# klasmodin/quflow

Hardware: AMD Instinct MI355X
Metric: isospectral timesteps/sec at N=1024 (1 GPU) + ensemble steps/sec at 1/2/4/8 GPUs (higher is better)
Workload: dtype f64

## Files before the change

### include/quflow_hip.h

```cpp
#ifndef QUFLOW_HIP_H
#define QUFLOW_HIP_H

#ifdef __cplusplus
extern "C" {
#endif

#define QF_OK 0
#define QF_ERR_INVALID 1
#define QF_ERR_NO_DEVICE 2
#define QF_ERR_HIP 3
#define QF_ERR_STATE 4
#define QF_ERR_CALLBACK 5
#define QF_ERR_UNSUPPORTED 6
#define QF_ERR_NONFINITE 7
#define QF_ERR_NOCONVERGE 8

#define QF_VERSION 100

typedef struct qf_ctx qf_ctx;

int qf_version(void);
const char *qf_last_error(void);
int qf_device_count(void);

int qf_ctx_create(int N, int device, qf_ctx **out);
int qf_ctx_destroy(qf_ctx *ctx);
int qf_ctx_size(const qf_ctx *ctx);
int qf_sync(qf_ctx *ctx);

double qf_hbar(int N);


int qf_laplacian_table(qf_ctx *ctx, int bc, double *lap_host);

int qf_solve_poisson(qf_ctx *ctx, const void *W_host, void *P_host, int skewh);

int qf_laplace(qf_ctx *ctx, const void *P_host, void *W_host);

int qf_solve_tridiagonal(qf_ctx *ctx, const double *lap_host, unsigned long long table_key,
                         const void *W_host, void *P_host, int skewh);
int qf_factor_cache_stats(qf_ctx *ctx, int *entries, unsigned long long *device_bytes);

int qf_set_hamiltonian(qf_ctx *ctx, const double *table_host, unsigned long long table_key, const void *offset_host,
                       unsigned long long offset_key);
int qf_clear_hamiltonian(qf_ctx *ctx);
int qf_hamiltonian(qf_ctx *ctx, const void *W_host, void *P_host);
int qf_hamiltonian_energy(qf_ctx *ctx, double *H);

int qf_set_forcing(qf_ctx *ctx, const void *F0_host, unsigned long long F0_key, double a_W, double a_P, double a_lap);
int qf_clear_forcing(qf_ctx *ctx);
int qf_forcing(qf_ctx *ctx, const void *P_host, const void *W_host, void *F_host);

int qf_set_stochastic_forcing(qf_ctx *ctx, int l_min, int l_max, const double *sigma, unsigned long long seed,
                              unsigned long long step, double a_W, double a_P, double a_lap, long long band_bytes_max);
int qf_stochastic_tell(qf_ctx *ctx, unsigned long long *step);
int qf_stochastic_seek(qf_ctx *ctx, unsigned long long step);
int qf_stochastic_pattern(qf_ctx *ctx, unsigned long long step, double dt, double *omega_host, void *F0_host);

int qf_upload_W(qf_ctx *ctx, const void *W_host);
int qf_download_W(qf_ctx *ctx, void *W_host);

typedef struct qf_isomp_stats {
    long long total_iterations;
    long long number_of_maxit;
    double tol_used;
    double last_resnorm;
} qf_isomp_stats;

int qf_isomp(qf_ctx *ctx, double dt, int steps, double tol, int minit, int maxit,
             int compsum, int reinitialize, qf_isomp_stats *stats_out);
int qf_isomp_continue(qf_ctx *ctx, double dt, int steps, double tol, int minit, int maxit,
                      int compsum, int reinitialize, qf_isomp_stats *stats_out);

int qf_isomp_multi(qf_ctx **ctxs, int k, double dt, int steps, double tol, int minit, int maxit,
                   qf_isomp_stats *stats_out);
int qf_c64_isomp_multi(qf_ctx **ctxs, int k, double dt, int steps, double tol, int minit, int maxit, qf_isomp_stats *stats_out);

#define QF_ERK_EULER 0
#define QF_ERK_HEUN 1
#define QF_ERK_RK4 2
int qf_erk(qf_ctx *ctx, int method, double dt, int steps, int skewh);
int qf_erk_states(qf_ctx *ctx, void *states_host, int k, int method, double dt, int steps, int skewh);

int qf_isomp_simple(qf_ctx *ctx, double dt, int steps);
int qf_isomp_quasinewton(qf_ctx *ctx, double dt, int steps, double tol, int maxit, qf_isomp_stats *stats_out);
struct qf_isomp_hooks;
int qf_isomp_simple_hooked(qf_ctx *ctx, double dt, int steps, const struct qf_isomp_hooks *hooks);
int qf_isomp_quasinewton_hooked(qf_ctx *ctx, double dt, int steps, double tol, int maxit, qf_isomp_stats *stats_out,
                                const struct qf_isomp_hooks *hooks);

int qf_isomp_states(qf_ctx *ctx, void *states_host, int k, double dt, int steps, double tol, int minit, int maxit,
                    int reinitialize, int magnetic, qf_isomp_stats *stats_out);

int qf_states_upload(qf_ctx *ctx, const void *states_host, int k);
int qf_states_download(qf_ctx *ctx, void *states_host, int k);
int qf_states_advance(qf_ctx *ctx, double dt, int steps, double tol, int minit, int maxit, int reinitialize, int magnetic,
                      qf_isomp_stats *stats_out);
int qf_states_select(qf_ctx *ctx, int j);
int qf_states_store(qf_ctx *ctx, int j);
int qf_states_inner(qf_ctx *ctx, double *out);
int qf_mhd_diagnostics(qf_ctx *ctx, double out[5]);
int qf_states_advance_diag(qf_ctx *ctx, double dt, int steps, double tol, int minit, int maxit, int reinitialize, int magnetic,
                           qf_isomp_stats *stats_out, double *mhd_out);

typedef struct qf_isomp_hooks {
    void *user;
    int (*hamiltonian)(void *user, const void *Whalf, void *P, double time);
    int (*forcing)(void *user, const void *P, const void *Whalf, void *F, double time);
    int (*strang)(void *user, double h, void *W);
    int (*callback)(void *user, const void *W, const void *dW2);
    int hamiltonian_takes_time, forcing_takes_time;
    int has_time;
    double time;
    int skewh;
    int solve_skewh;
    const double *strang_table;
    unsigned long long strang_key;
    int magnetic;
    int states_p;
} qf_isomp_hooks;
int qf_isomp_hooked(qf_ctx *ctx, void *states_host, int k, double dt, int steps, double tol, int minit, int maxit,
                    int compsum, int reinitialize, const qf_isomp_hooks *hooks, qf_isomp_stats *stats_out);
int qf_isomp_forced(qf_ctx *ctx, double dt, int steps, double tol, int minit, int maxit, int reinitialize,
                    const double *strang_table, unsigned long long strang_key, qf_isomp_stats *stats_out);
int qf_erk_hooked(qf_ctx *ctx, void *W_host, int method, double dt, int steps, const qf_isomp_hooks *hooks);
int qf_erk_states_hooked(qf_ctx *ctx, void *states_host, int k, int method, double dt, int steps, const qf_isomp_hooks *hooks);

int qf_basis_upload(qf_ctx *ctx, const double *basis_host, long long count);
int qf_basis_compute(qf_ctx *ctx);
int qf_basis_download(qf_ctx *ctx, double *basis_host, long long count);
int qf_basis_stream(qf_ctx *ctx, long long slab_bytes);
int qf_basis_slab_plan(int N, int Nmax, long long slab_bytes, int *first_block, int capacity);
int qf_shr2mat(qf_ctx *ctx, const double *omega_host, long long n_omega, void *W_host);
int qf_mat2shr(qf_ctx *ctx, const void *W_host, double *omega_host, long long n_omega);
int qf_shc2mat(qf_ctx *ctx, const void *omega_host, void *W_host);
int qf_mat2shc(qf_ctx *ctx, const void *W_host, void *omega_host);
int qf_shr2fun(qf_ctx *ctx, const double *omega_host, long long n_omega, int L, int berezin, double *f_host);
int qf_shc2fun(qf_ctx *ctx, const void *omega_host, long long n_omega, int L, int berezin, int isreal, void *f_host);
int qf_fun2shc(qf_ctx *ctx, const void *f_host, int L, int isreal, void *omega_host);
int qf_fun2shr(qf_ctx *ctx, const void *f_host, int L, int isreal, double *omega_host);

int qf_diagnostics(qf_ctx *ctx, double *energy_euler, double *enstrophy);
int qf_isomp_diag(qf_ctx *ctx, double dt, int steps, double tol, int minit, int maxit, int compsum,
                  int reinitialize, qf_isomp_stats *stats, double *energy_euler, double *enstrophy);
int qf_norm_inf_W(qf_ctx *ctx, double *out);

typedef struct qf_eigh_stats {
    int sweeps;
    long long rotations;
    double off;
} qf_eigh_stats;
int qf_eigh(qf_ctx *ctx, const void *H_host, double *lambda_host, void *V_host, qf_eigh_stats *stats);
int qf_eigh_skew(qf_ctx *ctx, const void *W_host, double *lambda_host, void *V_host, qf_eigh_stats *stats);
int qf_eigh_state(qf_ctx *ctx, double *lambda_host, qf_eigh_stats *stats);
int qf_scale_decomposition(qf_ctx *ctx, const void *W_host, const void *P_host, void *Ws_host, void *Wr_host);

int qf_so3_exp_plan(int N, const double xi[3], int *squarings, int *degree);
int qf_so3_exp(qf_ctx *ctx, const double xi[3], void *R_host);
// ... 68 lines not shown
```

### quflow_amd/_lib.py

```python
import ctypes
import os

_HERE = os.path.dirname(os.path.abspath(__file__))
LIB_PATH = os.environ.get("QUFLOW_HIP_LIB") or os.path.join(_HERE, "libquflow_hip.so")

QF_OK = 0
QF_ERR_NONFINITE = 7
QF_ERR_NOCONVERGE = 8
ERR_NAMES = {1: "QF_ERR_INVALID", 2: "QF_ERR_NO_DEVICE", 3: "QF_ERR_HIP", 4: "QF_ERR_STATE", 5: "QF_ERR_CALLBACK",
             6: "QF_ERR_UNSUPPORTED", 7: "QF_ERR_NONFINITE", 8: "QF_ERR_NOCONVERGE"}

KERNEL_IDS = {"poisson": 0, "gemm1": 1, "gemm2": 2, "norm": 3, "update": 4, "slice": 5}
ERK_METHODS = {"euler": 0, "heun": 1, "rk4": 2}
BUFFER_IDS = {"W": 0, "dW": 1, "Whalf": 2, "Phalf": 3, "PW": 4}


class QuflowHipError(RuntimeError):
    pass


HAMILTONIAN_CB = ctypes.CFUNCTYPE(ctypes.c_int, ctypes.c_void_p, ctypes.c_void_p, ctypes.c_void_p, ctypes.c_double)
FORCING_CB = ctypes.CFUNCTYPE(ctypes.c_int, ctypes.c_void_p, ctypes.c_void_p, ctypes.c_void_p, ctypes.c_void_p, ctypes.c_double)
STRANG_CB = ctypes.CFUNCTYPE(ctypes.c_int, ctypes.c_void_p, ctypes.c_double, ctypes.c_void_p)
CALLBACK_CB = ctypes.CFUNCTYPE(ctypes.c_int, ctypes.c_void_p, ctypes.c_void_p, ctypes.c_void_p)


class IsompHooks(ctypes.Structure):
    _fields_ = [("user", ctypes.c_void_p),
                ("hamiltonian", HAMILTONIAN_CB),
                ("forcing", FORCING_CB),
                ("strang", STRANG_CB),
                ("callback", CALLBACK_CB),
                ("hamiltonian_takes_time", ctypes.c_int),
                ("forcing_takes_time", ctypes.c_int),
                ("has_time", ctypes.c_int),
                ("time", ctypes.c_double),
                ("skewh", ctypes.c_int),
                ("solve_skewh", ctypes.c_int),
                ("strang_table", ctypes.c_void_p),
                ("strang_key", ctypes.c_ulonglong),
                ("magnetic", ctypes.c_int),
                ("states_p", ctypes.c_int)]


class IsompStats(ctypes.Structure):
    _fields_ = [("total_iterations", ctypes.c_longlong),
                ("number_of_maxit", ctypes.c_longlong),
                ("tol_used", ctypes.c_double),
                ("last_resnorm", ctypes.c_double)]


class EighStats(ctypes.Structure):
    _fields_ = [("sweeps", ctypes.c_int),
                ("rotations", ctypes.c_longlong),
                ("off", ctypes.c_double)]


_vp = ctypes.c_void_p
_dp = ctypes.POINTER(ctypes.c_double)
SIGNATURES = {
    "qf_version": (ctypes.c_int, []),
    "qf_last_error": (ctypes.c_char_p, []),
    "qf_device_count": (ctypes.c_int, []),
    "qf_ctx_create": (ctypes.c_int, [ctypes.c_int, ctypes.c_int, ctypes.POINTER(_vp)]),
    "qf_ctx_destroy": (ctypes.c_int, [_vp]),
    "qf_ctx_size": (ctypes.c_int, [_vp]),
    "qf_sync": (ctypes.c_int, [_vp]),
    "qf_hbar": (ctypes.c_double, [ctypes.c_int]),
    "qf_laplacian_table": (ctypes.c_int, [_vp, ctypes.c_int, _vp]),
    "qf_solve_poisson": (ctypes.c_int, [_vp, _vp, _vp, ctypes.c_int]),
    "qf_laplace": (ctypes.c_int, [_vp, _vp, _vp]),
    "qf_solve_tridiagonal": (ctypes.c_int, [_vp, _vp, ctypes.c_ulonglong, _vp, _vp, ctypes.c_int]),
    "qf_set_hamiltonian": (ctypes.c_int, [_vp, _vp, ctypes.c_ulonglong, _vp, ctypes.c_ulonglong]),
    "qf_clear_hamiltonian": (ctypes.c_int, [_vp]),
    "qf_hamiltonian": (ctypes.c_int, [_vp, _vp, _vp]),
    "qf_hamiltonian_energy": (ctypes.c_int, [_vp, _dp]),
    "qf_set_forcing": (ctypes.c_int, [_vp, _vp, ctypes.c_ulonglong, ctypes.c_double, ctypes.c_double, ctypes.c_double]),
    "qf_clear_forcing": (ctypes.c_int, [_vp]),
    "qf_forcing": (ctypes.c_int, [_vp, _vp, _vp, _vp]),
    "qf_set_stochastic_forcing": (ctypes.c_int, [_vp, ctypes.c_int, ctypes.c_int, _vp, ctypes.c_ulonglong, ctypes.c_ulonglong,
                                                 ctypes.c_double, ctypes.c_double, ctypes.c_double, ctypes.c_longlong]),
    "qf_stochastic_tell": (ctypes.c_int, [_vp, ctypes.POINTER(ctypes.c_ulonglong)]),
    "qf_stochastic_seek": (ctypes.c_int, [_vp, ctypes.c_ulonglong]),
    "qf_stochastic_pattern": (ctypes.c_int, [_vp, ctypes.c_ulonglong, ctypes.c_double, _vp, _vp]),
    "qf_isomp_forced": (ctypes.c_int, [_vp, ctypes.c_double, ctypes.c_int, ctypes.c_double, ctypes.c_int, ctypes.c_int,
                                       ctypes.c_int, _vp, ctypes.c_ulonglong, ctypes.POINTER(IsompStats)]),
    "qf_factor_cache_stats": (ctypes.c_int, [_vp, ctypes.POINTER(ctypes.c_int), ctypes.POINTER(ctypes.c_ulonglong)]),
    "qf_comm_unique_id": (ctypes.c_int, [_vp]),
    "qf_comm_create": (ctypes.c_int, [ctypes.POINTER(_vp), ctypes.c_int, ctypes.c_int, ctypes.c_int, _vp]),
    "qf_comm_allgather_f64": (ctypes.c_int, [_vp, _vp, ctypes.c_int, _vp]),
    "qf_comm_barrier": (ctypes.c_int, [_vp]),
    "qf_comm_destroy": (ctypes.c_int, [_vp]),
    "qf_upload_W": (ctypes.c_int, [_vp, _vp]),
    "qf_download_W": (ctypes.c_int, [_vp, _vp]),
    "qf_isomp": (ctypes.c_int, [_vp, ctypes.c_double, ctypes.c_int, ctypes.c_double, ctypes.c_int,
                                ctypes.c_int, ctypes.c_int, ctypes.c_int, ctypes.POINTER(IsompStats)]),
    "qf_isomp_diag": (ctypes.c_int, [_vp, ctypes.c_double, ctypes.c_int, ctypes.c_double, ctypes.c_int,
                                     ctypes.c_int, ctypes.c_int, ctypes.c_int, ctypes.POINTER(IsompStats),
                                     ctypes.POINTER(ctypes.c_double), ctypes.POINTER(ctypes.c_double)]),
    "qf_isomp_continue": (ctypes.c_int, [_vp, ctypes.c_double, ctypes.c_int, ctypes.c_double, ctypes.c_int,
                                         ctypes.c_int, ctypes.c_int, ctypes.c_int, ctypes.POINTER(IsompStats)]),
    "qf_isomp_multi": (ctypes.c_int, [ctypes.POINTER(_vp), ctypes.c_int, ctypes.c_double, ctypes.c_int, ctypes.c_double,
                                      ctypes.c_int, ctypes.c_int, ctypes.POINTER(IsompStats)]),
    "qf_c64_isomp_multi": (ctypes.c_int, [ctypes.POINTER(_vp), ctypes.c_int, ctypes.c_double, ctypes.c_int, ctypes.c_double,
                                          ctypes.c_int, ctypes.c_int, ctypes.POINTER(IsompStats)]),
    "qf_erk": (ctypes.c_int, [_vp, ctypes.c_int, ctypes.c_double, ctypes.c_int, ctypes.c_int]),
    "qf_erk_states": (ctypes.c_int, [_vp, _vp, ctypes.c_int, ctypes.c_int, ctypes.c_double, ctypes.c_int, ctypes.c_int]),
    "qf_isomp_simple_hooked": (ctypes.c_int, [_vp, ctypes.c_double, ctypes.c_int, ctypes.POINTER(IsompHooks)]),
    "qf_isomp_quasinewton_hooked": (ctypes.c_int, [_vp, ctypes.c_double, ctypes.c_int, ctypes.c_double, ctypes.c_int,
                                                   ctypes.POINTER(IsompStats), ctypes.POINTER(IsompHooks)]),
    "qf_isomp_simple": (ctypes.c_int, [_vp, ctypes.c_double, ctypes.c_int]),
    "qf_isomp_quasinewton": (ctypes.c_int, [_vp, ctypes.c_double, ctypes.c_int, ctypes.c_double, ctypes.c_int,
                                            ctypes.POINTER(IsompStats)]),
    "qf_isomp_states": (ctypes.c_int, [_vp, _vp, ctypes.c_int, ctypes.c_double, ctypes.c_int, ctypes.c_double,
                                       ctypes.c_int, ctypes.c_int, ctypes.c_int, ctypes.c_int,
                                       ctypes.POINTER(IsompStats)]),
    "qf_states_upload": (ctypes.c_int, [_vp, _vp, ctypes.c_int]),
    "qf_states_download": (ctypes.c_int, [_vp, _vp, ctypes.c_int]),
    "qf_states_advance": (ctypes.c_int, [_vp, ctypes.c_double, ctypes.c_int, ctypes.c_double, ctypes.c_int, ctypes.c_int,
                                         ctypes.c_int, ctypes.c_int, ctypes.POINTER(IsompStats)]),
    "qf_states_advance_diag": (ctypes.c_int, [_vp, ctypes.c_double, ctypes.c_int, ctypes.c_double, ctypes.c_int, ctypes.c_int,
                                              ctypes.c_int, ctypes.c_int, ctypes.POINTER(IsompStats), _dp]),
    "qf_states_select": (ctypes.c_int, [_vp, ctypes.c_int]),
    "qf_states_store": (ctypes.c_int, [_vp, ctypes.c_int]),
    "qf_mhd_diagnostics": (ctypes.c_int, [_vp, _dp]),
    "qf_states_inner": (ctypes.c_int, [_vp, _dp]),
    "qf_isomp_hooked": (ctypes.c_int, [_vp, _vp, ctypes.c_int, ctypes.c_double, ctypes.c_int, ctypes.c_double, ctypes.c_int,
                                       ctypes.c_int, ctypes.c_int, ctypes.c_int, ctypes.POINTER(IsompHooks),
                                       ctypes.POINTER(IsompStats)]),
    "qf_erk_hooked": (ctypes.c_int, [_vp, _vp, ctypes.c_int, ctypes.c_double, ctypes.c_int, ctypes.POINTER(IsompHooks)]),
    "qf_erk_states_hooked": (ctypes.c_int, [_vp, _vp, ctypes.c_int, ctypes.c_int, ctypes.c_double, ctypes.c_int,
                                            ctypes.POINTER(IsompHooks)]),
    "qf_basis_upload": (ctypes.c_int, [_vp, _vp, ctypes.c_longlong]),
    "qf_basis_compute": (ctypes.c_int, [_vp]),
    "qf_basis_download": (ctypes.c_int, [_vp, _vp, ctypes.c_longlong]),
    "qf_basis_stream": (ctypes.c_int, [_vp, ctypes.c_longlong]),
    "qf_basis_slab_plan": (ctypes.c_int, [ctypes.c_int, ctypes.c_int, ctypes.c_longlong, ctypes.POINTER(ctypes.c_int),
                                          ctypes.c_int]),
    "qf_shr2mat": (ctypes.c_int, [_vp, _vp, ctypes.c_longlong, _vp]),
    "qf_mat2shr": (ctypes.c_int, [_vp, _vp, _vp, ctypes.c_longlong]),
    "qf_shc2mat": (ctypes.c_int, [_vp, _vp, _vp]),
    "qf_mat2shc": (ctypes.c_int, [_vp, _vp, _vp]),
    "qf_shr2fun": (ctypes.c_int, [_vp, _vp, ctypes.c_longlong, ctypes.c_int, ctypes.c_int, _vp]),
    "qf_shc2fun": (ctypes.c_int, [_vp, _vp, ctypes.c_longlong, ctypes.c_int, ctypes.c_int, ctypes.c_int, _vp]),
    "qf_fun2shc": (ctypes.c_int, [_vp, _vp, ctypes.c_int, ctypes.c_int, _vp]),
    "qf_fun2shr": (ctypes.c_int, [_vp, _vp, ctypes.c_int, ctypes.c_int, _vp]),
    "qf_diagnostics": (ctypes.c_int, [_vp, _dp, _dp]),
    "qf_norm_inf_W": (ctypes.c_int, [_vp, _dp]),
    "qf_eigh": (ctypes.c_int, [_vp, _vp, _vp, _vp, ctypes.POINTER(EighStats)]),
    "qf_eigh_skew": (ctypes.c_int, [_vp, _vp, _vp, _vp, ctypes.POINTER(EighStats)]),
    "qf_eigh_state": (ctypes.c_int, [_vp, _vp, ctypes.POINTER(EighStats)]),
    "qf_scale_decomposition": (ctypes.c_int, [_vp, _vp, _vp, _vp, _vp]),
    "qf_so3_exp_plan": (ctypes.c_int, [ctypes.c_int, _dp, ctypes.POINTER(ctypes.c_int), ctypes.POINTER(ctypes.c_int)]),
    "qf_so3_exp": (ctypes.c_int, [_vp, _dp, _vp]),
    "qf_so3_exp_times": (ctypes.c_int, [_vp, _dp, _dp]),
    "qf_rotate": (ctypes.c_int, [_vp, _dp, _vp, _vp]),
    "qf_grad": (ctypes.c_int, [_vp, _vp, _vp]),
    "qf_profile_enable": (ctypes.c_int, [_vp, ctypes.c_int]),
    "qf_profile_reset": (ctypes.c_int, [_vp]),
    "qf_profile_read": (ctypes.c_int, [_vp, ctypes.c_int, ctypes.POINTER(ctypes.c_longlong), _dp]),
    "qf_plan_describe": (ctypes.c_int, [_vp, ctypes.c_char_p, ctypes.c_int]),
    "qf_device_info": (ctypes.c_int, [ctypes.c_int, ctypes.c_char_p, ctypes.c_int]),
    "qf_debug_modulus": (ctypes.c_int, [_vp, ctypes.c_int, _dp, _dp, _dp, _dp]),
    "qf_profile_stride": (ctypes.c_int, [_vp, ctypes.c_int]),
    "qf_profile_seen": (ctypes.c_int, [_vp, ctypes.c_int, ctypes.POINTER(ctypes.c_longlong)]),
    "qf_timer_start": (ctypes.c_int, [_vp]),
    "qf_timer_stop": (ctypes.c_int, [_vp, _dp]),
    "qf_download_buffer": (ctypes.c_int, [_vp, ctypes.c_int, _vp]),
    "qf_debug_guard_check": (ctypes.c_int, [ctypes.POINTER(ctypes.c_longlong), ctypes.POINTER(ctypes.c_longlong), ctypes.c_char_p, ctypes.c_int]),
    "qf_zgemm": (ctypes.c_int, [_vp, _vp, _vp, _vp]),
    "qf_commutator": (ctypes.c_int, [_vp, _vp, _vp, _vp, ctypes.c_int]),
    "qf_zgemm_i8": (ctypes.c_int, [_vp, _vp, _vp, _vp]),
    "qf_fixedpoint_products": (ctypes.c_int, [_vp, _vp, _vp, _vp, _vp, ctypes.c_int, _vp, _vp, _vp]),
    "qf_c64_laplacian_table": (ctypes.c_int, [_vp, ctypes.c_int, _vp]),
    "qf_c64_solve_poisson": (ctypes.c_int, [_vp, _vp, _vp, ctypes.c_int]),
    "qf_c64_laplace": (ctypes.c_int, [_vp, _vp, _vp]),
    "qf_c64_solve_tridiagonal": (ctypes.c_int, [_vp, _vp, _vp, _vp, ctypes.c_int]),
    "qf_c64_upload_W": (ctypes.c_int, [_vp, _vp]),
    "qf_c64_download_W": (ctypes.c_int, [_vp, _vp]),
    "qf_c64_isomp": (ctypes.c_int, [_vp, ctypes.c_double, ctypes.c_int, ctypes.c_double, ctypes.c_int,
                                    ctypes.c_int, ctypes.c_int, ctypes.c_int, ctypes.POINTER(IsompStats)]),
    "qf_c64_isomp_continue": (ctypes.c_int, [_vp, ctypes.c_double, ctypes.c_int, ctypes.c_double, ctypes.c_int,
                                             ctypes.c_int, ctypes.c_int, ctypes.c_int, ctypes.POINTER(IsompStats)]),
    "qf_c64_diagnostics": (ctypes.c_int, [_vp, _dp, _dp]),
    "qf_cgemm": (ctypes.c_int, [_vp, _vp, _vp, _vp]),
    "qf_c64_fixedpoint_products": (ctypes.c_int, [_vp, _vp, _vp, _vp, _vp, _vp, _vp, _vp]),
    "qf_c64_fixedpoint_products_tri": (ctypes.c_int, [_vp, _vp, _vp, _vp, _vp, _vp, _vp, _vp]),
}
# ... 50 lines not shown
```

### quflow_amd/csrc/api_context.hip

```cpp
#include <cmath>
#include <cstdarg>
#include <cstdio>
#include <cstdlib>
#include <cstring>
#include <limits>
#include <chrono>

#include "qf_api.h"

static thread_local char g_err[512] = "";

void qf_set_error(const char *fmt, ...)
{
    va_list ap;
    va_start(ap, fmt);
    vsnprintf(g_err, sizeof(g_err), fmt, ap);
    va_end(ap);
}

extern "C" {

int qf_version(void) { return QF_VERSION; }

int qf_device_info(int device, char *buf, int n)
// ... 35 lines not shown
        return -QF_ERR_INVALID;
    }
    static const char *const role[QF_KERNEL_COUNT] = {"laplacian_inverse", "first_product", "second_product", "residual_norm",
                                                      "step_update", "slicing"};
    std::string out = "{\"N\": " + std::to_string(ctx->N);
    for (int r = 0; r < QF_KERNEL_COUNT; ++r) {
        out += ", \"";
        out += role[r];
        out += "\": ";
        out += ctx->plan[r].text[0] ? ctx->plan[r].text : "null";
    }
    if (ctx->ham_table || ctx->ham_offset_on) {
        char h[160];
        if (ctx->ham_table) snprintf(h, sizeof(h), ", \"hamiltonian\": {\"table_key\": %llu, \"offset\": %s}", ctx->ham_key, ctx->ham_offset_on ? "true" : "false");
        else snprintf(h, sizeof(h), ", \"hamiltonian\": {\"table_key\": null, \"offset\": true}");
        out += h;
    } else {
        out += ", \"hamiltonian\": \"poisson\"";
    }
    out += "}";
    if (n > 0) {
        const size_t m = out.size() < (size_t)(n - 1) ? out.size() : (size_t)(n - 1);
        memcpy(buf, out.data(), m);
        buf[m] = 0;
    }
    return (int)out.size();
}

const char *qf_last_error(void) { return g_err; }

int qf_device_count(void)
{
    int n = 0;
    if (hipGetDeviceCount(&n) != hipSuccess) return 0;
    return n;
}

double qf_hbar(int N) { return 2.0 / std::sqrt((double)N * (double)N - 1.0); }

int qf_ctx_create(int N, int device, qf_ctx **out)
{
    if (!out) {
        qf_set_error("qf_ctx_create: out is null");
        return QF_ERR_INVALID;
    }
    *out = nullptr;
    if (N < 2 || N > 8192) {
        qf_set_error("qf_ctx_create: N=%d out of range [2, 8192]", N);
        return QF_ERR_INVALID;
    }
    int ndev = qf_device_count();
    if (ndev <= 0) {
        qf_set_error("qf_ctx_create: no HIP device visible (this library has no CPU fallback)");
        return QF_ERR_NO_DEVICE;
    }
    if (device < 0 || device >= ndev) {
        qf_set_error("qf_ctx_create: device %d out of range (0..%d)", device, ndev - 1);
        return QF_ERR_NO_DEVICE;
    }
    QF_HIP(hipSetDevice(device));
    qf_ctx *ctx = new qf_ctx();
    ctx->N = N;
    ctx->device = device;
    if (const char *g = getenv("QUFLOW_HIP_GEMM")) {
        ctx->gemm_i8_allowed = (g[0] == 'i');
        if (g[0] == 'i' && strstr(g, "x6")) ctx->oz_digits = 6;
        if (g[0] == 'i' && strstr(g, "x65")) ctx->oz_digits2 = 5;
        if (g[0] == 'i' && strchr(g, 'h')) ctx->gemm_i8_hybrid = true;
        if (g[0] == 'i' && strchr(g, 'f') && !ctx->gemm_i8_hybrid) ctx->gemm_i8_first = true;
        if (g[0] == 'a') {
            ctx->gemm_i8_allowed = true;
            ctx->oz_digits = 6;
            ctx->oz_digits2 = 5;
            ctx->gemm_i8_min_n = 1024;
        }
    }
    if (const char *g = getenv("QUFLOW_HIP_GEMM2")) ctx->gemm_tri_allowed = !(g[0] == 'f');
    if (const char *g = getenv("QUFLOW_HIP_FUSED")) ctx->fused_allowed = !(g[0] == '0');
    if (const char *g = getenv("QUFLOW_HIP_I8_MIN_N")) ctx->gemm_i8_min_n = atoi(g);
    if (const char *g = getenv("QUFLOW_HIP_TRI_MIN_N")) ctx->gemm_tri_min_n = atoi(g);
    if (const char *g = getenv("QUFLOW_HIP_DEFER")) ctx->defer_allowed = !(g[0] == '0');
    if (getenv("QUFLOW_HIP_DEBUG"))
        if (const char *g = getenv("QUFLOW_HIP_DEBUG_DROP_FLAG")) ctx->debug_drop = atoi(g);
    if (const char *g = getenv("QUFLOW_HIP_FACTOR_CACHE_MB")) ctx->factor_budget_bytes = (size_t)(atoi(g) > 0 ? atoi(g) : 1) << 20;
    const size_t NN = (size_t)N * N;
    const size_t mbytes = NN * sizeof(cplx);
    int rc = QF_OK;
    auto fail = [&](int code) {
        qf_ctx_destroy(ctx);
        return code;
    };
#define QF_CREATE_HIP(call)                                                                   \
    do {                                                                                      \
        hipError_t _e = (call);                                                               \
        if (_e != hipSuccess) {                                                               \
            qf_set_error("%s failed: %s", #call, hipGetErrorString(_e));                     \
            return fail(QF_ERR_HIP);                                                          \
        }                                                                                     \
    } while (0)
    QF_CREATE_HIP(hipStreamCreateWithFlags(&ctx->stream, hipStreamNonBlocking));
    cplx **mats[] = {&ctx->W, &ctx->dW[0], &ctx->dW[1], &ctx->Whalf, &ctx->Phalf, &ctx->PW, &ctx->stage};
    for (cplx **m : mats) {
        QF_CREATE_HIP(hipMalloc((void **)m, mbytes));
        QF_CREATE_HIP(hipMemsetAsync(*m, 0, mbytes, ctx->stream));
    }
    QF_CREATE_HIP(hipMalloc((void **)&ctx->lap, 2 * NN * sizeof(double)));
    ctx->rowpart_tiles = qf_gemm_tiles_n(N);
    {
        const int slots32 = (N + 31) / 32;
        QF_CREATE_HIP(hipMalloc((void **)&ctx->rowpart, (size_t)(ctx->rowpart_tiles > slots32 ? ctx->rowpart_tiles : slots32) * N * sizeof(double)));
    }
    QF_CREATE_HIP(hipMalloc((void **)&ctx->rowsum, (size_t)N * sizeof(double)));
    QF_CREATE_HIP(hipMalloc((void **)&ctx->scalars, 4096 * sizeof(double)));
    QF_CREATE_HIP(hipHostMalloc((void **)&ctx->host_scalars, 64 * sizeof(double), hipHostMallocDefault));
    QF_CREATE_HIP(hipMalloc((void **)&ctx->state, sizeof(qf_dev_state)));
    QF_CREATE_HIP(hipMemsetAsync(ctx->state, 0, sizeof(qf_dev_state), ctx->stream));
    QF_CREATE_HIP(hipMalloc((void **)&ctx->ticket, 704 * sizeof(unsigned)));
    QF_CREATE_HIP(hipMemsetAsync(ctx->ticket, 0, 704 * sizeof(unsigned), ctx->stream));
    QF_CREATE_HIP(hipHostMalloc((void **)&ctx->host_rec, sizeof(qf_host_record), hipHostMallocCoherent));
    memset(ctx->host_rec, 0, sizeof(qf_host_record));
    {
        hipDeviceProp_t prop;
        QF_CREATE_HIP(hipGetDeviceProperties(&prop, device));
        ctx->num_cus = prop.multiProcessorCount;
        if (N % 64 == 0 && ctx->num_cus > 0) {
            ctx->sk_slots = ctx->num_cus;
            QF_CREATE_HIP(hipMalloc((void **)&ctx->sk_partial, (size_t)ctx->sk_slots * 64 * 64 * sizeof(cplx)));
            QF_CREATE_HIP(hipMalloc((void **)&ctx->sk_flags, (size_t)(ctx->sk_slots + 16) * sizeof(unsigned)));
            QF_CREATE_HIP(hipMemsetAsync(ctx->sk_flags, 0, (size_t)(ctx->sk_slots + 16) * sizeof(unsigned), ctx->stream));
        }
    }
    QF_CREATE_HIP(hipEventCreate(&ctx->timer_start));
    QF_CREATE_HIP(hipEventCreate(&ctx->timer_stop));
#undef QF_CREATE_HIP
    if ((rc = alloc_factors(ctx, &ctx->poisson)) != QF_OK) return fail(rc);
    if ((rc = qf_launch_lap_table(ctx, 1, ctx->lap)) != QF_OK) return fail(rc);
    if ((rc = qf_launch_build_factors(ctx, ctx->lap, ctx->poisson)) != QF_OK) return fail(rc);
    if (hipStreamSynchronize(ctx->stream) != hipSuccess) {
        qf_set_error("qf_ctx_create: table construction failed");
        return fail(QF_ERR_HIP);
    }
    *out = ctx;
    return QF_OK;
}

int qf_ctx_destroy(qf_ctx *ctx)
{
    if (!ctx) return QF_OK;
    (void)hipSetDevice(ctx->device);
    if (ctx->stream) (void)hipStreamSynchronize(ctx->stream);
    void *ptrs[] = {ctx->W, ctx->dW[0], ctx->dW[1], ctx->Whalf, ctx->Phalf, ctx->PW, ctx->kahan_c, ctx->stage,
                    ctx->lap, ctx->lap_user, ctx->poisson.tab, ctx->ham.tab, ctx->ham_offset, ctx->forcing_f0, ctx->stoch.basis, ctx->stoch.omega,
                    ctx->stoch.stage, ctx->stoch.sigma, ctx->rowpart, ctx->rowsum,
                    ctx->t32_partial, ctx->t32_arrive, ctx->W2, ctx->Whalf2, ctx->ns_inv, ctx->ns_tmp, ctx->multi_rowpart, ctx->scalars, ctx->sk_partial, ctx->sk_flags, ctx->basis, ctx->sh_stage, ctx->sh_omega, ctx->slab};
    for (void *p : ptrs)
        if (p) (void)hipFree(p);
    void *sht[] = {ctx->sht.omega, ctx->sht.tab, ctx->sht.col, ctx->sht.At, ctx->sht.tw, ctx->sht.f, ctx->sht.H, ctx->sht.Q};
    for (void *p : sht)
        if (p) (void)hipFree(p);
    void *eigh[] = {ctx->eigh.H, ctx->eigh.G, ctx->eigh.V, ctx->eigh.ray, ctx->eigh.sig, ctx->eigh.perm, ctx->eigh.word};
    for (void *p : eigh)
        if (p) (void)hipFree(p);
    void *geom[] = {ctx->geom.R[0], ctx->geom.R[1], ctx->geom.grad};
    for (void *p : geom)
        if (p) (void)hipFree(p);
    for (hipEvent_t e : ctx->geom.ev)
        if (e) (void)hipEventDestroy(e);
    for (cplx *p : ctx->multi)
        if (p) (void)hipFree(p);
    for (cplx *p : ctx->stack)
        if (p) (void)hipFree(p);
    if (ctx->mhd_part) (void)hipFree(ctx->mhd_part);
    for (int q = 0; q < 4; ++q) {
        if (ctx->oz_planes[q]) (void)hipFree(ctx->oz_planes[q]);
        if (ctx->oz_scale[q]) (void)hipFree(ctx->oz_scale[q]);
        if (q == 0 && ctx->oz_tbuf) (void)hipFree(ctx->oz_tbuf);
        if (q == 0 && ctx->oz_tflags) (void)hipFree(ctx->oz_tflags);
        if (q == 0 && ctx->oz_diag) (void)hipFree(ctx->oz_diag);
    }
    for (auto &kv : ctx->user_factors) {
        if (kv.second.f.tab) (void)hipFree(kv.second.f.tab);
    }
    for (int q = 0; q < 3; ++q)
        if (ctx->hook_host[q]) (void)hipHostFree(ctx->hook_host[q]);
    qf_c64_free(ctx->c64);
    ctx->c64 = nullptr;
    if (ctx->host_scalars) (void)hipHostFree(ctx->host_scalars);
    if (ctx->host_rec) (void)hipHostFree(ctx->host_rec);
    if (ctx->state) (void)hipFree(ctx->state);
    if (ctx->ticket) (void)hipFree(ctx->ticket);
    for (auto &ev : ctx->events_busy) {
        (void)hipEventDestroy(ev.start);
        (void)hipEventDestroy(ev.stop);
    }
    for (auto &ev : ctx->events_free) {
        (void)hipEventDestroy(ev.start);
        (void)hipEventDestroy(ev.stop);
    }
    if (ctx->timer_start) (void)hipEventDestroy(ctx->timer_start);
    if (ctx->timer_stop) (void)hipEventDestroy(ctx->timer_stop);
    if (ctx->stream) (void)hipStreamDestroy(ctx->stream);
    delete ctx;
    return QF_OK;
}

int qf_ctx_size(const qf_ctx *ctx) { return ctx ? ctx->N : -1; }

int qf_sync(qf_ctx *ctx)
{
    QF_TRY(check_ctx(ctx));
    QF_HIP(hipStreamSynchronize(ctx->stream));
    return QF_OK;
}


int qf_upload_W(qf_ctx *ctx, const void *W_host)
{
    QF_TRY(check_ctx(ctx));
    if (!W_host) {
        qf_set_error("qf_upload_W: null buffer");
        return QF_ERR_INVALID;
    }
    QF_HIP(hipMemcpyAsync(ctx->W, W_host, (size_t)ctx->N * ctx->N * sizeof(cplx), hipMemcpyHostToDevice, ctx->stream));
    QF_HIP(hipStreamSynchronize(ctx->stream));
    ctx->w_skew_known = false;
    return QF_OK;
}

int qf_download_W(qf_ctx *ctx, void *W_host)
{
    QF_TRY(check_ctx(ctx));
    if (!W_host) {
        qf_set_error("qf_download_W: null buffer");
        return QF_ERR_INVALID;
    }
    QF_HIP(hipMemcpyAsync(W_host, ctx->W, (size_t)ctx->N * ctx->N * sizeof(cplx), hipMemcpyDeviceToHost, ctx->stream));
    QF_HIP(hipStreamSynchronize(ctx->stream));
    return QF_OK;
}

int qf_norm_inf_W(qf_ctx *ctx, double *out)
{
    QF_TRY(check_ctx(ctx));
    QF_TRY(qf_launch_norm_inf(ctx, ctx->W, ctx->scalars));
    return read_scalar(ctx, ctx->scalars, out);
}


int qf_c64_upload_W(qf_ctx *ctx, const void *W_host)
{
    QF_TRY(qf_need_c64(ctx));
    if (!W_host) {
        qf_set_error("qf_c64_upload_W: null buffer");
        return QF_ERR_INVALID;
    }
    QF_HIP(hipMemcpyAsync(ctx->c64->W, W_host, (size_t)ctx->N * ctx->N * sizeof(float2), hipMemcpyHostToDevice, ctx->stream));
    QF_HIP(hipStreamSynchronize(ctx->stream));
    ctx->c64->increment_valid = false;
    ctx->c64->w_skew_known = false;
    return QF_OK;
}

int qf_c64_download_W(qf_ctx *ctx, void *W_host)
{
    QF_TRY(qf_need_c64(ctx));
    if (!W_host) {
        qf_set_error("qf_c64_download_W: null buffer");
        return QF_ERR_INVALID;
    }
    QF_HIP(hipMemcpyAsync(W_host, ctx->c64->W, (size_t)ctx->N * ctx->N * sizeof(float2), hipMemcpyDeviceToHost, ctx->stream));
    QF_HIP(hipStreamSynchronize(ctx->stream));
    return QF_OK;
}


int qf_profile_enable(qf_ctx *ctx, int mask)
{
    QF_TRY(check_ctx(ctx));
    if (!mask) QF_TRY(drain_events(ctx));
    ctx->profile_mask = mask;
    return QF_OK;
}

// ... 109 lines not shown
```

### quflow_amd/csrc/api_isomp.hip

```cpp
#include <cmath>
#include <cstdarg>
#include <cstdio>
#include <cstdlib>
#include <cstring>
#include <limits>
#include <chrono>
#include <type_traits>
#include <utility>

#include "qf_api.h"

namespace {

#ifndef QF_RUN_AHEAD
#define QF_RUN_AHEAD 3
#endif

template <class S> constexpr bool is_c64 = std::is_same<S, qf_c64>::value;

template <class S> S *ws(qf_ctx *ctx)
{
    if constexpr (is_c64<S>) return ctx->c64;
    else return ctx;
}

template <class S> double mach_eps(bool root)
{
    using R = std::conditional_t<is_c64<S>, float, double>;
    const R e = std::numeric_limits<R>::epsilon();
    return root ? std::sqrt(e) : e;
}

int launch_solve(qf_ctx *ctx, const cplx *W, cplx *P, double vareps, qf_guard g, const qf_decide *dec = nullptr)
{
    return qf_launch_hamiltonian(ctx, W, P, vareps, g, dec);
}
int launch_solve(qf_ctx *ctx, const float2 *W, float2 *P, double vareps, qf_guard g)
{
    return qf_launch_solve(ctx, ctx->c64->tab, W, P, (float)vareps, 1, g);
}
int launch_gemm(qf_ctx *ctx, const cplx *A, const cplx *B, cplx *C, const qf_epilogue *ep, qf_guard g)
{
    return qf_launch_zgemm(ctx, A, B, C, ep, g);
}
int launch_gemm(qf_ctx *ctx, const float2 *A, const float2 *B, float2 *C, const qf_epilogue_f *ep, qf_guard g)
{
    return qf_launch_cgemm(ctx, A, B, C, ep, g);
}

template <class S> auto epilogue_of(S *w, bool fused)
{
    std::conditional_t<is_c64<S>, qf_epilogue_f, qf_epilogue> ep;
    ep.PW = w->PW;
    ep.W = w->W;
    ep.dW[0] = w->dW[0];
    ep.dW[1] = w->dW[1];
    ep.Whalf = w->Whalf;
    ep.rowpart = w->rowpart;
    if (fused) {
        ep.fused = 1;
        ep.Wpair[0] = w->W;
        ep.Wpair[1] = w->W2;
        ep.Whalf_step = w->Whalf2;
    }
    return ep;
}

template <class S> int check_skew(qf_ctx *ctx, S *w)
{
    if (w->w_skew_known) return QF_OK;
    double defect = 0.0;
    QF_TRY(qf_launch_skew_defect(ctx, w->W, ctx->scalars + 4));
    QF_TRY(read_scalar(ctx, ctx->scalars + 4, &defect));
    w->w_skew_known = (defect == 0.0);
    return QF_OK;
}

int tri32_alloc(qf_ctx *ctx)
{
    const int nt = (ctx->N + 31) / 32;
    const int n_tiles = nt * (nt + 1) / 2;
    if (!ctx->t32_partial) {
        QF_HIP(hipMalloc((void **)&ctx->t32_partial, (size_t)n_tiles * 4 * 32 * 32 * sizeof(cplx)));
        QF_HIP(hipMalloc((void **)&ctx->t32_arrive, (size_t)n_tiles * sizeof(unsigned)));
        QF_HIP(hipMemsetAsync(ctx->t32_arrive, 0, (size_t)n_tiles * sizeof(unsigned), ctx->stream));
        int so = 2, sd = 1;
        {
            const int cus = ctx->num_cus > 0 ? ctx->num_cus : 256;
            if (nt * (nt - 1) + 2 * nt <= cus) sd = 2;
            else if (nt * (nt - 1) + nt > cus) so = 1;
        }
        ctx->tri32_split = so;
        ctx->tri32_split_diag = sd;
    }
    return QF_OK;
}

int select_second_product(qf_ctx *ctx)
{
// ... 6 lines not shown
    const bool want_tri32 = ctx->gemm_tri_allowed && !want_tri && ctx->N >= 64 && tri32_fits;
    const bool want_i8 = ctx->gemm_i8_allowed && ctx->N % 64 == 0 && ctx->N >= ctx->gemm_i8_min_n && ctx->N <= 4096;
    if (!want_tri && !want_i8 && !want_tri32) return QF_OK;
    QF_TRY(check_skew(ctx, ctx));
    const bool skew = ctx->w_skew_known;
    ctx->gemm_tri = want_tri && skew;
    ctx->gemm_i8 = want_i8 && skew;
    ctx->gemm_tri32 = want_tri32 && skew && (!ctx->gemm_i8 || ctx->gemm_i8_first);
    if (ctx->gemm_tri32) QF_TRY(tri32_alloc(ctx));
    return QF_OK;
}

int select_second_product_c64(qf_ctx *ctx)
{
    qf_c64 *f = ctx->c64;
    f->tri = false;
    if (f->tri_allowed && ctx->gemm_tri_allowed && (qf_c64_tile(ctx) == 32 || ctx->N % 64 == 0) && ctx->N >= 64) {
        QF_TRY(check_skew(ctx, f));
        if (f->w_skew_known) {
            QF_TRY(qf_c64_tri_alloc(ctx));
            f->tri = true;
        }
    }
    return QF_OK;
}

bool triangle_product(const qf_ctx *ctx) { return (ctx->gemm_tri || ctx->gemm_tri32) && (!ctx->gemm_i8 || ctx->gemm_i8_first); }
bool triangle_product(const qf_c64 *f) { return f->tri; }

template <class S> int begin_increment(qf_ctx *ctx, S *w, bool carry)
{
    const size_t mbytes = (size_t)ctx->N * ctx->N * sizeof(*w->W);
    if (carry) {
        if (w->dw_cur != 0)
            QF_HIP(hipMemcpyAsync(w->dW[0], w->dW[w->dw_cur], mbytes, hipMemcpyDeviceToDevice, ctx->stream));
        QF_TRY(qf_launch_lincomb(ctx, 1, w->W, 1, w->dW[0], 0, w->Whalf));
    } else {
        QF_HIP(hipMemsetAsync(w->dW[0], 0, mbytes, ctx->stream));
        QF_HIP(hipMemcpyAsync(w->Whalf, w->W, mbytes, hipMemcpyDeviceToDevice, ctx->stream));
    }
    return QF_OK;
}

template <class S> int enqueue_iterations(qf_ctx *ctx, int step, int first, int count, double vareps)
{
    S *w = ws<S>(ctx);
    for (int i = first; i < first + count; ++i) {
        qf_guard g;
        g.state = ctx->state;
        g.step = step;
        g.iter = i;
        {
            prof_scope p(ctx, QF_KERNEL_POISSON);
            QF_TRY(launch_solve(ctx, w->Whalf, w->Phalf, vareps, g));
        }
        {
            prof_scope p(ctx, QF_KERNEL_GEMM1);
            QF_TRY(launch_gemm(ctx, w->Phalf, w->Whalf, w->PW, nullptr, g));
        }
        {
            prof_scope p(ctx, QF_KERNEL_GEMM2);
            const auto ep = epilogue_of(w, false);
            QF_TRY(launch_gemm(ctx, w->PW, w->Phalf, nullptr, &ep, g));
        }
        {
            prof_scope p(ctx, QF_KERNEL_NORM);
            QF_TRY(qf_launch_norm_decide(ctx, w->rowpart, is_c64<S> ? w->rowpart_tiles : qf_rowpart_slots(ctx), g));
        }
    }
    return QF_OK;
}

qf_decide deferred_decision(qf_ctx *ctx)
{
    qf_decide d;
    d.rowpart = ctx->rowpart;
    d.slots = ctx->gemm_tri32 ? (ctx->N + 31) / 32 : ctx->N / 64;
    d.state_rw = ctx->state;
    d.rec = ctx->host_rec;
    d.ticket = ctx->ticket + 402;
    return d;
}

template <class S> int enqueue_iterations_fused(qf_ctx *ctx, int step, int first, int count, double vareps, bool last_step)
{
    S *w = ws<S>(ctx);
    const bool defer = !is_c64<S> && ctx->defer;
    const qf_decide dec = defer ? deferred_decision(ctx) : qf_decide();
    for (int i = first; i < first + count; ++i) {
        qf_guard g;
        g.state = ctx->state;
        g.step = step;
        g.iter = i;
        g.alt = w->Whalf2;
        {
            prof_scope p(ctx, QF_KERNEL_POISSON);
            if constexpr (is_c64<S>) QF_TRY(launch_solve(ctx, w->Whalf, w->Phalf, vareps, g));
            else QF_TRY(launch_solve(ctx, w->Whalf, w->Phalf, vareps, g, defer ? &dec : nullptr));
        }
        {
            prof_scope p(ctx, QF_KERNEL_GEMM1);
            QF_TRY(launch_gemm(ctx, w->Phalf, w->Whalf, w->PW, nullptr, g));
        }
        {
            prof_scope p(ctx, QF_KERNEL_GEMM2);
            const auto ep = epilogue_of(w, true);
            g.alt = nullptr;
            if constexpr (is_c64<S>) {
                if (w->tri) QF_TRY(qf_launch_cgemm_tri(ctx, w->PW, w->Phalf, &ep, g));
                else QF_TRY(qf_launch_cgemm(ctx, w->PW, w->Phalf, nullptr, &ep, g));
            } else {
                QF_TRY(qf_launch_zgemm(ctx, w->PW, w->Phalf, nullptr, &ep, g));
            }
        }
    }
    if (defer && last_step && count > 0) QF_TRY(qf_launch_decide(ctx, dec));
    return QF_OK;
}

int enqueue_iterations_fused_i8(qf_ctx *ctx, int step, int first, int count, double vareps)
{
    for (int i = first; i < first + count; ++i) {
        qf_guard g;
        g.state = ctx->state;
        g.step = step;
        g.iter = i;
        g.alt = ctx->Whalf2;
        {
            prof_scope p(ctx, QF_KERNEL_POISSON);
            QF_TRY(qf_launch_hamiltonian(ctx, ctx->Whalf, ctx->Phalf, vareps, g));
        }
        if (ctx->gemm_i8_hybrid) {
            {
                prof_scope p(ctx, QF_KERNEL_GEMM1);
                QF_TRY(qf_launch_zgemm(ctx, ctx->Phalf, ctx->Whalf, ctx->PW, nullptr, g));
            }
            g.alt = nullptr;
            {
                prof_scope p(ctx, QF_KERNEL_SLICE);
                qf_oz_jobs jobs;
                jobs.n = 2;
                jobs.j[0].X = ctx->PW;
                jobs.j[0].planes = ctx->oz_planes[3];
                jobs.j[0].scale = ctx->oz_scale[3];
                jobs.j[1].X = ctx->Phalf;
                jobs.j[1].planes = ctx->oz_planes[0];
                jobs.j[1].scale = ctx->oz_scale[0];
                QF_TRY(qf_launch_oz_slice(ctx, jobs, g));
            }
            {
                prof_scope p(ctx, QF_KERNEL_GEMM2);
                const qf_epilogue ep = epilogue_of(ctx, true);
                QF_TRY(qf_launch_oz_gemm(ctx, ctx->oz_planes[3], ctx->oz_scale[3], ctx->oz_planes[0], ctx->oz_scale[0], nullptr,
                                         &ep, g));
            }
            continue;
        }
        g.alt = nullptr;
        {
            prof_scope p(ctx, QF_KERNEL_SLICE);
            qf_oz_jobs jobs;
            jobs.n = 2;
            jobs.j[0].X = ctx->Phalf;
            jobs.j[0].planes = ctx->oz_planes[0];
            jobs.j[0].scale = ctx->oz_scale[0];
            jobs.j[1].X = ctx->Whalf;
            jobs.j[1].X_alt = ctx->Whalf2;
            jobs.j[1].planes = ctx->oz_planes[2];
            jobs.j[1].scale = ctx->oz_scale[2];
            jobs.diag = ctx->oz_diag;
            QF_TRY(qf_launch_oz_slice(ctx, jobs, g));
        }
        {
            prof_scope p(ctx, QF_KERNEL_GEMM1);
            QF_TRY(qf_launch_oz_gemm(ctx, ctx->oz_planes[0], ctx->oz_scale[0], ctx->oz_planes[2], ctx->oz_scale[2],
                                     ctx->PW, nullptr, g, 0, 0, ctx->oz_diag));
        }
        if (ctx->gemm_i8_first) {
            prof_scope p(ctx, QF_KERNEL_GEMM2);
            const qf_epilogue ep = epilogue_of(ctx, true);
            QF_TRY(qf_launch_zgemm(ctx, ctx->PW, ctx->Phalf, nullptr, &ep, g));
            continue;
        }
        {
            prof_scope p(ctx, QF_KERNEL_SLICE);
            qf_oz_jobs jobs;
            jobs.n = 1;
            jobs.j[0].X = ctx->PW;
            jobs.j[0].planes = ctx->oz_planes[3];
            jobs.j[0].scale = ctx->oz_scale[3];
            QF_TRY(qf_launch_oz_slice(ctx, jobs, g, ctx->oz_digits2));
        }
        {
            prof_scope p(ctx, QF_KERNEL_GEMM2);
            const qf_epilogue ep = epilogue_of(ctx, true);
            QF_TRY(qf_launch_oz_gemm(ctx, ctx->oz_planes[3], ctx->oz_scale[3], ctx->oz_planes[0], ctx->oz_scale[0], nullptr,
                                     &ep, g, ctx->oz_digits2, ctx->oz_digits2 ? ctx->oz_digits : 0));
        }
    }
    return QF_OK;
}

template <class S> struct fused_run {
    qf_ctx *ctx = nullptr;
    int steps = 0, minit = 1, maxit = 1;
    double vareps = 0.0;
    int pred = 1, pred0 = 1;
    std::vector<int> enq_iters;
    int known = 0, enq = 0;
    bool first_seen = false;
    bool aborted = false;
    unsigned long long idle_polls = 0;

    int enqueue(int step, int first, int count)
    {
        if constexpr (!is_c64<S>)
            if (ctx->gemm_i8) return enqueue_iterations_fused_i8(ctx, step, first, count, vareps);
        return enqueue_iterations_fused<S>(ctx, step, first, count, vareps, step == steps - 1);
    }
    bool cold_start = true;
    void begin(qf_ctx *c, int steps_, int minit_, int maxit_, double vareps_)
    {
        ctx = c;
        cold_start = ws<S>(c)->increment_is_zero;
        steps = steps_;
        minit = minit_;
        maxit = maxit_;
        vareps = vareps_;
        pred = ctx->pred_iters;
        if (pred < minit) pred = minit;
        if (pred > maxit) pred = maxit;
        pred0 = ctx->pred_first_iters > 0 ? ctx->pred_first_iters : pred + 1;
        if (pred0 < pred) pred0 = pred;
        if (pred0 > maxit) pred0 = maxit;
        enq_iters.assign((size_t)steps + 1, 0);
        known = enq = 0;
        first_seen = false;
        aborted = false;
        idle_polls = 0;
    }
    bool done() const { return known >= steps; }
    int pump()
    {
        if (done()) return QF_OK;
        while (enq < steps && enq - known < QF_RUN_AHEAD) {
            const int n = (enq == 0 && cold_start) ? pred0 : pred;
            QF_TRY(enqueue(enq, 0, n));
            enq_iters[enq] = n;
            ++enq;
        }
        volatile qf_host_record *rec = ctx->host_rec;
        unsigned long long p = __atomic_load_n(&rec->progress, __ATOMIC_ACQUIRE);
        int ps = (int)(p >> 32), pi = (int)(p & 0xffffffffull);
        if (ps >= QF_STEP_ABORTED) {
            aborted = true;
            known = steps;
            return QF_OK;
        }
        if (!(ps > known || (ps == known && pi >= enq_iters[known]))) {
            if (++idle_polls > (1ull << 22)) {
                QF_HIP(hipStreamSynchronize(ctx->stream));
                p = __atomic_load_n(&rec->progress, __ATOMIC_ACQUIRE);
                ps = (int)(p >> 32);
                pi = (int)(p & 0xffffffffull);
                if (ps >= QF_STEP_ABORTED) {
                    aborted = true;
                    known = steps;
                    return QF_OK;
                }
                if (!(ps > known || (ps == known && pi >= enq_iters[known]))) {
                    qf_set_error("qf_isomp: device progress stuck at step %d iteration %d (waiting for step %d)", ps, pi, known);
                    return QF_ERR_STATE;
                }
            } else {
                return QF_OK;
            }
        }
        idle_polls = 0;
        if (ps > known) {
            const int it = rec->last_step_iters;
            if (known == 0 && ps == 1 && !first_seen && cold_start) {
                first_seen = true;
                if (it >= minit && it <= maxit) ctx->pred_first_iters = it;
            } else if (it >= minit && it <= maxit) {
                pred = it;
            }
            known = ps < enq ? ps : enq;
            if (done()) ctx->pred_iters = pred;
            return QF_OK;
        }
        const int have = enq_iters[known];
        if (have >= maxit) {
            qf_set_error("qf_isomp: step %d did not close after maxit=%d iterations (internal error)", known, maxit);
            return QF_ERR_STATE;
        }
        QF_TRY(enqueue(known, have, maxit - have));
        enq_iters[known] = maxit;
        enq = known + 1;
        if (pred < maxit) pred += 1;
        return QF_OK;
    }
};

bool poll_yields()
{
    static const int mode = [] {
        const char *e = getenv("QUFLOW_HIP_POLL");
        return (e && strcmp(e, "yield") == 0) ? 1 : 0;
    }();
    return mode == 1;
}

inline void poll_relax()
{
    if (poll_yields()) {
        sched_yield();
        return;
    }
#if defined(__x86_64__)
    __builtin_ia32_pause();
#endif
}

template <class S> int run_fused(qf_ctx *ctx, int steps, int minit, int maxit, double vareps)
{
    fused_run<S> run;
    run.begin(ctx, steps, minit, maxit, vareps);
    while (!run.done()) {
        QF_TRY(run.pump());
        poll_relax();
    }
    ctx->pred_iters = run.pred;
    return QF_OK;
}

template <class S> int enqueue_step_end(qf_ctx *ctx, int step, int compsum, int reinitialize)
{
    S *w = ws<S>(ctx);
    qf_guard g;
    g.state = ctx->state;
    g.step = step;
    prof_scope p(ctx, QF_KERNEL_UPDATE);
    return qf_launch_update(ctx, w->PW, w->W, w->dW[0], w->dW[1], w->Whalf, compsum ? w->kahan_c : nullptr, reinitialize, g);
}

int wait_for_advance(qf_ctx *ctx, unsigned long long seq)
{
    volatile qf_host_record *rec = ctx->host_rec;
    unsigned long long spins = 0;
    while (__atomic_load_n(&rec->seq, __ATOMIC_ACQUIRE) < seq) {
        if (++spins > (1ull << 22)) {
            const unsigned long long before = __atomic_load_n(&rec->seq, __ATOMIC_ACQUIRE);
            const hipError_t q = hipStreamQuery(ctx->stream);
            QF_HIP(hipStreamSynchronize(ctx->stream));
            if (getenv("QUFLOW_HIP_DEBUG"))
                fprintf(stderr, "[quflow_hip] wait_for_advance: spin limit; want seq %llu, saw %llu before sync (stream %s), %llu after; step_index %d incomplete %d\n",
                        seq, before, q == hipSuccess ? "idle" : "busy", (unsigned long long)rec->seq, rec->step_index, rec->incomplete);
            if (__atomic_load_n(&rec->seq, __ATOMIC_ACQUIRE) < seq) {
                qf_set_error("qf_isomp: device progress record stuck at %llu (< %llu)",
                             (unsigned long long)rec->seq, seq);
                return QF_ERR_STATE;
            }
            break;
        }
#if defined(__x86_64__)
        __builtin_ia32_pause();
#endif
    }
    return QF_OK;
}

int reset_after_abort(qf_ctx *ctx)
{
    if (!ctx->needs_reset) return QF_OK;
    QF_HIP(hipMemsetAsync(ctx->ticket, 0, 704 * sizeof(unsigned), ctx->stream));
    if (ctx->sk_flags) QF_HIP(hipMemsetAsync(ctx->sk_flags + (ctx->sk_slots > 0 ? ctx->sk_slots : ctx->num_cus), 0, 16 * sizeof(unsigned), ctx->stream));
    if (ctx->t32_arrive) {
        const size_t nt = (size_t)(ctx->N + 31) / 32;
        QF_HIP(hipMemsetAsync(ctx->t32_arrive, 0, nt * (nt + 1) / 2 * sizeof(unsigned), ctx->stream));
    }
    if (ctx->c64 && ctx->c64->tri_arrive)
        QF_HIP(hipMemsetAsync(ctx->c64->tri_arrive, 0, ctx->c64->tri_arrive_count * sizeof(unsigned), ctx->stream));
    ctx->needs_reset = false;
    return QF_OK;
}

template <class S> int fused_enter(qf_ctx *ctx, double dt, double tol, int minit, int maxit, bool carry)
{
    S *w = ws<S>(ctx);
    const size_t mbytes = (size_t)ctx->N * ctx->N * sizeof(*w->W);
    const bool tol_on_device = tol < 0;
    const double tol_factor = tol_on_device ? mach_eps<S>(true) * dt / qf_hbar(ctx->N) : 0.0;
    QF_TRY(reset_after_abort(ctx));
    if constexpr (is_c64<S>) {
        QF_TRY(select_second_product_c64(ctx));
    } else {
        QF_TRY(select_second_product(ctx));
        ctx->defer = ctx->defer_allowed && !ctx->gemm_i8 && ctx->gemm_tri32 && ctx->N <= 512;
    }
    w->increment_is_zero = !carry;
    w->increment_valid = true;
    volatile qf_host_record *rec = ctx->host_rec;
    rec->progress = 0ull;
    rec->step_index = 0;
    rec->fault = 0;
    rec->nonfinite = 0;
    __atomic_thread_fence(__ATOMIC_SEQ_CST);
    if (is_c64<S> || carry) {
        if (tol_on_device) QF_TRY(qf_launch_norm_inf(ctx, w->W, ctx->scalars));
        QF_TRY(begin_increment(ctx, w, carry));
        QF_TRY(qf_launch_state_init(ctx, tol, minit, maxit, tol_on_device ? ctx->scalars : nullptr, tol_factor));
    } else {
        QF_TRY(qf_launch_call_begin(ctx, tol, minit, maxit, tol_on_device ? 1 : 0, tol_factor));
    }
    if (!w->W2) QF_HIP(hipMalloc((void **)&w->W2, mbytes));
    if (!w->Whalf2) QF_HIP(hipMalloc((void **)&w->Whalf2, mbytes));
    if constexpr (!is_c64<S>)
        if (ctx->gemm_i8) QF_TRY(qf_oz_alloc(ctx));
    return QF_OK;
}

template <class S> int fused_leave(qf_ctx *ctx, int steps, qf_isomp_stats *stats_out)
{
    S *w = ws<S>(ctx);
    volatile qf_host_record *rec = ctx->host_rec;
    const int w_parity = steps > 0 ? rec->w_parity : 0, wh_sel = steps > 0 ? rec->wh_sel : 0;
    w->dw_cur = steps > 0 ? rec->dw_parity : 0;
    if (w_parity) std::swap(w->W, w->W2);
    if (wh_sel) std::swap(w->Whalf, w->Whalf2);
    if (triangle_product(w) && steps > 0) {
        QF_TRY(qf_launch_mirror_lower(ctx, w->W));
        QF_TRY(qf_launch_mirror_lower(ctx, w->dW[w->dw_cur]));
    }
    if constexpr (!is_c64<S>)
        if (ctx->diag_at_exit) {
            QF_TRY(qf_enqueue_diagnostics(ctx));
            ctx->diag_valid = true;
        }
    QF_HIP(hipStreamSynchronize(ctx->stream));
    if (rec->nonfinite) {
        qf_set_error("array must not contain infs or NaNs");
        ctx->needs_reset = true;
        w->increment_valid = false;
        ctx->diag_valid = false;
        rec->nonfinite = 0;
        return QF_ERR_NONFINITE;
    }
    if (steps > 0 && rec->step_index != steps) {
        qf_set_error("qf_isomp: device completed %d of %d steps (internal error)", rec->step_index, steps);
        return QF_ERR_STATE;
    }
    if (rec->fault) {
        qf_set_error("qf_isomp: a device-side wait of the second product ran out (a parked partial tile or a mirrored result tile was never published)");
        return QF_ERR_STATE;
    }
    if (stats_out) {
        stats_out->total_iterations = steps > 0 ? rec->total_iterations : 0;
        stats_out->number_of_maxit = steps > 0 ? rec->number_of_maxit : 0;
        stats_out->tol_used = rec->tol;
        stats_out->last_resnorm = rec->resnorm;
    }
    return QF_OK;
}

void fused_abort(qf_ctx *ctx)
{
    (void)hipStreamSynchronize(ctx->stream);
// ... 142 lines not shown
                steps, t_tol, t_sel, t_init, t_loop, t_sync, ms_since(t_entry), t_waitmax, waitstep, t_waitat, t_enqmax, enqstep, t_enqat);
    if (st.fault == QF_FAULT_NONFINITE || rec->nonfinite) {
        qf_set_error("array must not contain infs or NaNs");
        ctx->needs_reset = true;
        w->increment_valid = false;
        rec->nonfinite = 0;
        return QF_ERR_NONFINITE;
    }
    if (st.step_index != steps) {
        qf_set_error("qf_isomp: device completed %d of %d steps (internal error)", st.step_index, steps);
        return QF_ERR_STATE;
    }
    w->dw_cur = st.dw_parity;
    if (rec->fault) {
        qf_set_error("qf_isomp: a device-side wait of the second product ran out (a parked partial tile or a mirrored result tile was never published)");
        return QF_ERR_STATE;
    }
    if (stats_out) {
        stats_out->total_iterations = st.total_iterations;
        stats_out->number_of_maxit = st.number_of_maxit;
        stats_out->tol_used = tol;
        stats_out->last_resnorm = rec->resnorm;
    }
    return QF_OK;
}

template <class S>
int isomp_multi(qf_ctx **ctxs, int k, double dt, int steps, double tol, int minit, int maxit, qf_isomp_stats *stats_out)
{
    const char *name = is_c64<S> ? "qf_c64_isomp_multi" : "qf_isomp_multi";
    if (!ctxs || k < 1) {
        qf_set_error("%s: bad arguments (k=%d)", name, k);
        return QF_ERR_INVALID;
    }
    if (minit < 1) {
        qf_set_error("minit must be at least 1.");
        return QF_ERR_INVALID;
    }
    if (maxit < minit) {
        qf_set_error("maxit must be at minit.");
        return QF_ERR_INVALID;
    }
    if (steps < 0) {
        qf_set_error("%s: steps must be >= 0", name);
        return QF_ERR_INVALID;
    }
    bool together = true;
    for (int r = 0; r < k; ++r) {
        QF_TRY(check_ctx(ctxs[r]));
        QF_TRY(qf_refuse_forcing(ctxs[r], name));
        if (is_c64<S> && !ctxs[r]->c64) {
            qf_set_error("%s: context %d holds no complex64 state (qf_c64_upload_W)", name, r);
            return QF_ERR_STATE;
        }
        for (int q = 0; q < r; ++q)
            if (ctxs[q] == ctxs[r]) {
                qf_set_error("%s: context %d is listed twice", name, r);
                return QF_ERR_INVALID;
            }
        if (ctxs[r]->device != ctxs[0]->device) {
            qf_set_error("%s: the contexts live on different devices", name);
            return QF_ERR_INVALID;
        }
        together = together && ctxs[r]->fused_allowed;
    }
    auto mark_failed = [&](int r) {
        if (!stats_out) return;
        stats_out[r].total_iterations = -1;
        stats_out[r].number_of_maxit = -1;
        stats_out[r].last_resnorm = std::numeric_limits<double>::quiet_NaN();
    };
    if (!together) {
        int first_rc = QF_OK;
        for (int q = 0; q < k; ++q) {
            const int rc = isomp_impl<S>(ctxs[q], dt, steps, tol, minit, maxit, 0, 0, stats_out ? stats_out + q : nullptr, false);
            if (rc != QF_OK) {
                mark_failed(q);
                if (first_rc == QF_OK) first_rc = rc;
            }
        }
        return first_rc;
    }
    auto abort_all = [&](int rc) {
        for (int q = 0; q < k; ++q) fused_abort(ctxs[q]);
        return rc;
    };
    std::vector<fused_run<S>> runs((size_t)k);
    for (int r = 0; r < k; ++r) {
        const int rc = fused_enter<S>(ctxs[r], dt, tol, minit, maxit, false);
        if (rc != QF_OK) return abort_all(rc);
        runs[r].begin(ctxs[r], steps, minit, maxit, dt / (2 * qf_hbar(ctxs[r]->N)));
    }
    for (;;) {
        bool all = true;
        for (int r = 0; r < k; ++r) {
            if (runs[r].done()) continue;
            const int rc = runs[r].pump();
            if (rc != QF_OK) return abort_all(rc);
            all = all && runs[r].done();
        }
        if (all) break;
        poll_relax();
    }
    int first_rc = QF_OK;
    for (int r = 0; r < k; ++r) {
        ctxs[r]->pred_iters = runs[r].pred;
        const int rc = fused_leave<S>(ctxs[r], steps, stats_out ? stats_out + r : nullptr);
        if (rc != QF_OK) {
            mark_failed(r);
            if (first_rc == QF_OK) first_rc = rc;
        }
    }
    return first_rc == QF_OK ? QF_OK : abort_all(first_rc);
}

int c64_fixedpoint_products(const char *name, bool tri, qf_ctx *ctx, const void *Phalf_host, const void *Whalf_host,
                            const void *W_host, const void *dW_old_host, void *dW_new_host, void *Whalf_new_host,
                            double *rowsum_host)
{
    QF_TRY(qf_need_c64(ctx));
    if (!Phalf_host || !Whalf_host || !W_host || !dW_old_host || !dW_new_host || !Whalf_new_host || !rowsum_host) {
        qf_set_error("%s: null buffer", name);
        return QF_ERR_INVALID;
    }
    if (tri) QF_TRY(qf_c64_tri_alloc(ctx));
    qf_c64 *f = ctx->c64;
    const int N = ctx->N;
    const size_t bytes = (size_t)N * N * sizeof(float2);
    QF_HIP(hipMemcpyAsync(f->Phalf, Phalf_host, bytes, hipMemcpyHostToDevice, ctx->stream));
    QF_HIP(hipMemcpyAsync(f->Whalf, Whalf_host, bytes, hipMemcpyHostToDevice, ctx->stream));
    QF_HIP(hipMemcpyAsync(f->stage, W_host, bytes, hipMemcpyHostToDevice, ctx->stream));
    QF_HIP(hipMemcpyAsync(f->dW[0], dW_old_host, bytes, hipMemcpyHostToDevice, ctx->stream));
    QF_TRY(qf_launch_cgemm(ctx, f->Phalf, f->Whalf, f->PW, nullptr));
    qf_epilogue_f ep = epilogue_of(f, false);
    ep.W = f->stage;
    if (tri) {
        QF_TRY(qf_launch_cgemm_tri(ctx, f->PW, f->Phalf, &ep));
        QF_TRY(qf_launch_mirror_lower(ctx, f->dW[1]));
        QF_TRY(qf_launch_sum_rowpart(ctx, f->rowpart, (N + qf_c64_tile(ctx) - 1) / qf_c64_tile(ctx), ctx->rowsum));
    } else {
        QF_TRY(qf_launch_cgemm(ctx, f->PW, f->Phalf, nullptr, &ep));
        QF_TRY(qf_launch_sum_rowpart(ctx, f->rowpart, f->rowpart_tiles, ctx->rowsum));
    }
    QF_HIP(hipMemcpyAsync(dW_new_host, f->dW[1], bytes, hipMemcpyDeviceToHost, ctx->stream));
    QF_HIP(hipMemcpyAsync(Whalf_new_host, f->Whalf, bytes, hipMemcpyDeviceToHost, ctx->stream));
    QF_HIP(hipMemcpyAsync(rowsum_host, ctx->rowsum, (size_t)N * sizeof(double), hipMemcpyDeviceToHost, ctx->stream));
    QF_HIP(hipStreamSynchronize(ctx->stream));
    return QF_OK;
}

}

int qf_rowpart_slots(const qf_ctx *ctx) { return ctx->gemm_tri ? ctx->N / 64 : ctx->gemm_tri32 ? (ctx->N + 31) / 32 : ctx->rowpart_tiles; }

int qf_enqueue_diagnostics(qf_ctx *ctx)
{
    QF_TRY(qf_launch_solve(ctx, ctx->poisson, ctx->W, ctx->stage, 1.0, 1));
    QF_TRY(qf_launch_inner2(ctx, ctx->W, ctx->stage, ctx->scalars + 2));
    QF_HIP(hipMemcpyAsync(ctx->host_scalars, ctx->scalars + 2, 2 * sizeof(double), hipMemcpyDeviceToHost, ctx->stream));
    return QF_OK;
}

int qf_isomp_multi(qf_ctx **ctxs, int k, double dt, int steps, double tol, int minit, int maxit, qf_isomp_stats *stats_out)
{
    return isomp_multi<qf_ctx>(ctxs, k, dt, steps, tol, minit, maxit, stats_out);
}

int qf_c64_isomp_multi(qf_ctx **ctxs, int k, double dt, int steps, double tol, int minit, int maxit, qf_isomp_stats *stats_out)
{
    return isomp_multi<qf_c64>(ctxs, k, dt, steps, tol, minit, maxit, stats_out);
}

int qf_isomp(qf_ctx *ctx, double dt, int steps, double tol, int minit, int maxit, int compsum,
             int reinitialize, qf_isomp_stats *stats_out)
{
    return isomp_impl<qf_ctx>(ctx, dt, steps, tol, minit, maxit, compsum, reinitialize, stats_out, false);
}

int qf_isomp_continue(qf_ctx *ctx, double dt, int steps, double tol, int minit, int maxit, int compsum,
                      int reinitialize, qf_isomp_stats *stats_out)
{
    return isomp_impl<qf_ctx>(ctx, dt, steps, tol, minit, maxit, compsum, reinitialize, stats_out, true);
}

int qf_isomp_diag(qf_ctx *ctx, double dt, int steps, double tol, int minit, int maxit, int compsum, int reinitialize,
                  qf_isomp_stats *stats_out, double *energy_euler, double *enstrophy)
{
    QF_TRY(check_ctx(ctx));
    ctx->diag_at_exit = true;
    ctx->diag_valid = false;
    const int rc = isomp_impl<qf_ctx>(ctx, dt, steps, tol, minit, maxit, compsum, reinitialize, stats_out, false);
    ctx->diag_at_exit = false;
    if (rc != QF_OK) return rc;
    if (!ctx->diag_valid) return qf_diagnostics(ctx, energy_euler, enstrophy);
    ctx->diag_valid = false;
    const double wp = ctx->host_scalars[0], ww = ctx->host_scalars[1];
    if (energy_euler) *energy_euler = -(wp / ctx->N) / 2.0;
    if (enstrophy) *enstrophy = (ww / ctx->N) / 2.0;
    return QF_OK;
}


int qf_fixedpoint_products(qf_ctx *ctx, const void *Phalf_host, const void *Whalf_host, const void *W_host,
                           const void *dW_old_host, int variant, void *dW_new_host, void *Whalf_new_host,
                           double *rowsum_host)
{
    QF_TRY(check_ctx(ctx));
    if (!Phalf_host || !Whalf_host || !W_host || !dW_old_host || !dW_new_host || !Whalf_new_host || !rowsum_host) {
        qf_set_error("qf_fixedpoint_products: null buffer");
        return QF_ERR_INVALID;
    }
    const int variant_arg = variant;
    variant &= 15;
    if (variant == 1 && !ctx->sk_partial) {
        qf_set_error("qf_fixedpoint_products: the upper-triangle product needs N %% 64 == 0 (N=%d)", ctx->N);
        return QF_ERR_INVALID;
    }
    if (variant == 2) {
        if (ctx->N < 64) {
            qf_set_error("qf_fixedpoint_products: the 32x32 upper-triangle product needs N >= 64 (N=%d)", ctx->N);
            return QF_ERR_INVALID;
        }
        QF_TRY(tri32_alloc(ctx));
    }
    const int N = ctx->N;
    const size_t bytes = (size_t)N * N * sizeof(cplx);
    QF_HIP(hipMemcpyAsync(ctx->Phalf, Phalf_host, bytes, hipMemcpyHostToDevice, ctx->stream));
    QF_HIP(hipMemcpyAsync(ctx->Whalf, Whalf_host, bytes, hipMemcpyHostToDevice, ctx->stream));
    QF_HIP(hipMemcpyAsync(ctx->stage, W_host, bytes, hipMemcpyHostToDevice, ctx->stream));
    QF_HIP(hipMemcpyAsync(ctx->dW[0], dW_old_host, bytes, hipMemcpyHostToDevice, ctx->stream));
    QF_TRY(qf_launch_zgemm(ctx, ctx->Phalf, ctx->Whalf, ctx->PW, nullptr));
    qf_epilogue ep = epilogue_of(ctx, false);
    ep.W = ctx->stage;
    const bool saved = ctx->gemm_tri, saved32 = ctx->gemm_tri32;
    const int s_min = ctx->sk_min_units, s_epi = ctx->sk_epi_units, s_so = ctx->tri32_split, s_sd = ctx->tri32_split_diag;
    ctx->gemm_tri = (variant == 1);
    ctx->gemm_tri32 = (variant == 2);
    if (variant == 1) {
        if ((variant_arg >> 8) & 0xff) ctx->sk_min_units = (variant_arg >> 8) & 0xff;
        if ((variant_arg >> 16) & 0xff) ctx->sk_epi_units = ((variant_arg >> 16) & 0xff) - 64;
    } else if (variant == 2) {
        const int so = (variant_arg >> 8) & 15, sd = (variant_arg >> 12) & 15;
        if (so == 1 || so == 2 || so == 4) ctx->tri32_split = so;
// ... 65 lines not shown
```

### quflow_amd/csrc/poisson.hip

```cpp
#include "qf_internal.h"
#include "qf_step_end.h"

#pragma clang fp contract(off)

#ifdef QF_PROBE
__device__ int qf_probe_flags = 0;
__device__ unsigned long long *qf_probe_stamps = nullptr;
#define QF_PROBE_SKIP(bit_) (qf_probe_flags & (1 << (bit_)))
#define QF_PROBE_STAMP(slot_)                                                                     \
    if (qf_probe_stamps && (threadIdx.x & 63) == 0)                                               \
        qf_probe_stamps[((size_t)blockIdx.x * (blockDim.x >> 6) + (threadIdx.x >> 6)) * 16 + (slot_)] = __builtin_amdgcn_s_memtime();
#else
#define QF_PROBE_SKIP(bit_) 0
#define QF_PROBE_STAMP(slot_)
#endif

namespace {

template <typename R>
__global__ void k_lap_table(int N, int bc, R *__restrict__ lap)
{
    size_t e = (size_t)blockIdx.x * blockDim.x + threadIdx.x;
    if (e >= (size_t)N * N) return;
    int i = (int)(e / N), j = (int)(e % N);
// ... 126 lines not shown
    const int l = lane & (width - 1);
#define QF_SCAN_STEP(D_)                                                               \
    if (width > (D_)) {                                                                \
        const R ap = dpp_mov<0x110 + (D_), 0xf>(a);                                    \
        const R bx = dpp_mov<0x110 + (D_), 0xf>(b.x);                                  \
        const R by = dpp_mov<0x110 + (D_), 0xf>(b.y);                                  \
        if (l >= (D_) && (lane & 15) >= (D_)) {                                        \
            b.x = fma_r(a, bx, b.x);                                                   \
            b.y = fma_r(a, by, b.y);                                                   \
            a *= ap;                                                                   \
        }                                                                              \
    }
    QF_SCAN_STEP(1)
    QF_SCAN_STEP(2)
    QF_SCAN_STEP(4)
    QF_SCAN_STEP(8)
#undef QF_SCAN_STEP
    if (width > 16) {
        const R ap = dpp_mov<0x142, 0xa>(a);
        const R bx = dpp_mov<0x142, 0xa>(b.x);
        const R by = dpp_mov<0x142, 0xa>(b.y);
        if (lane & 16) {
            b.x = fma_r(a, bx, b.x);
            b.y = fma_r(a, by, b.y);
            a *= ap;
        }
    }
    if (width > 32) {
        const R ap = dpp_mov<0x143, 0xc>(a);
        const R bx = dpp_mov<0x143, 0xc>(b.x);
        const R by = dpp_mov<0x143, 0xc>(b.y);
        if (lane & 32) {
            b.x = fma_r(a, bx, b.x);
            b.y = fma_r(a, by, b.y);
            a *= ap;
        }
    }
}

template <typename R> __device__ __forceinline__ R lane_before(R v) { return dpp_mov<0x138, 0xf>(v); }

template <typename R, int CPW, bool REVERSE>
__device__ __forceinline__ void scan_chunks(int C, int G, int CE, int CR, int GP, const R *endc, const typename rt<R>::C *endv,
                                            typename rt<R>::C *carry, int lane, int wave, int nwaves)
{
    typedef typename rt<R>::C cplx;
    int Cp = CPW;
    if (!CPW) {
        Cp = 1;
        while (Cp < C) Cp <<= 1;
    }
    const int dpw = 64 / Cp;
    const int l = lane & (Cp - 1);
    const int q = REVERSE ? C - 1 - l : l;
    for (int gd = wave * dpw + (CPW == 64 ? 0 : lane / Cp); gd < G; gd += nwaves * dpw) {
        R a = R(0);
        cplx b = mkc<R>(R(0), R(0));
        if (l < C) {
            a = endc[gd * CR + q];
            b = endv[gd * CE + q];
        }
        scan_affine(a, b, lane, Cp);
        const R cx = lane_before(b.x), cy = lane_before(b.y);
        if (l < C) carry[q * GP + gd] = (l == 0) ? mkc<R>(R(0), R(0)) : mkc<R>(cx, cy);
    }
}

template <typename R, int L, int SKEWH, int FOLD = 0>
__global__ __launch_bounds__(L <= 17 ? 512 : 256) void k_solve(int N, int G, int C, const typename rt<R>::C *__restrict__ W,
                        typename rt<R>::C *__restrict__ P, const typename rt<R>::C *__restrict__ tab, R scale,
                        qf_guard guard, qf_decide dec, int tail_off)
#define QF_SOLVE_OFFSET 0
#include "poisson_solve_body.h"
#undef QF_SOLVE_OFFSET

template <int L, int FOLD>
__global__ __launch_bounds__(L <= 17 ? 512 : 256) void k_solve_off(int N, int G, int C, const double2 *__restrict__ W,
                        double2 *__restrict__ P, const double2 *__restrict__ tab, const double2 *__restrict__ F, double scale,
                        qf_guard guard, qf_decide dec, int tail_off)
#define QF_SOLVE_OFFSET 1
#include "poisson_solve_body.h"
#undef QF_SOLVE_OFFSET

__global__ __launch_bounds__(256) void k_decide(int N, qf_decide dec)
{
    __shared__ double scratch[40];
    if (!dec.state_rw->pending) return;
    const qf_new_state ns = qf_decide_compute(N, dec.slots, dec.rowpart, dec.state_rw, scratch);
    if (threadIdx.x == 0) qf_decide_apply(dec.state_rw, dec.rec, dec.ticket, ns);
}

struct solve_cfg {
    int L, G, C, threads, fold, T;
    size_t smem;
};

bool fold_wanted(int N, int skewh)
{
    const char *e = getenv("QUFLOW_HIP_SOLVE_FOLD");
    const int forced = e ? atoi(e) : -1;
    if (!skewh || N + 1 > 17 * 128) return false;
    if (forced == 0) return false;
    if (forced == 1) return N >= 256;
    return N >= 768;
}

solve_cfg pick_cfg(int N, size_t csize = sizeof(cplx), bool fold = false)
{
    solve_cfg c;
    c.fold = fold ? 1 : 0;
    c.T = N;
    if (fold) {
        c.L = (N + 1 <= 9 * 128) ? 9 : 17;
        c.C = (N + 1 + c.L - 1) / c.L;
        c.T = (N + 1) / 2;
        int G = 64;
        while (G > 1 && G * c.C > 512) G >>= 1;
        while (G > 2 && (c.T + G - 1) / G < 256) G >>= 1;
        c.G = G;
        c.threads = ((G * c.C + 63) / 64) * 64;
        const size_t scan_bytes = (size_t)(c.C + 2) * G * csize + (size_t)c.C * (G + 1) * csize + (size_t)c.threads * csize +
                                  (size_t)(c.C + 4) * G * (csize / 2);
        const size_t tile_bytes = (size_t)c.C * c.L * G * csize;
        c.smem = (((scan_bytes > tile_bytes ? scan_bytes : tile_bytes) + 15) & ~(size_t)15) + 8 * csize;
        return c;
    }
    c.L = 16;
    c.C = (N + c.L - 1) / c.L;
    if (c.C > 64) {
        c.L = 32;
        c.C = (N + c.L - 1) / c.L;
    } else if ((N + 3) / 4 <= 64) {
        c.L = 4;
        c.C = (N + 3) / 4;
    } else if ((N + 7) / 8 <= 64) {
        c.L = 8;
        c.C = (N + 7) / 8;
    }
    const int max_threads = c.L <= 16 ? 512 : 256;
    int G = 64;
    while (G > 1 && G * c.C > max_threads) G >>= 1;
    while (G > 4 && (N + G - 1) / G < 256) G >>= 1;
    c.G = G;
    c.threads = ((G * c.C + 63) / 64) * 64;
    const size_t scan_bytes = (size_t)(c.C + 2) * G * csize + (size_t)c.C * (G + 1) * csize + (size_t)c.threads * csize +
                              (size_t)(c.C + 4) * G * (csize / 2);
    const size_t tile_bytes = (size_t)c.C * (c.L + 1) * G * csize;
    c.smem = (((scan_bytes > tile_bytes ? scan_bytes : tile_bytes) + 15) & ~(size_t)15) + 8 * csize;
    return c;
}

template <typename R>
int launch_solve(qf_ctx *ctx, const typename rt<R>::C *tab, const typename rt<R>::C *W, typename rt<R>::C *P, R scale, int skewh,
                 const qf_guard &guard, const qf_decide *decp = nullptr, const typename rt<R>::C *F = nullptr)
{
    if (F && (sizeof(R) != sizeof(double) || !skewh)) {
        qf_set_error("qf_launch_solve: the offset form exists for the double-precision skew-Hermitian solve only");
        return QF_ERR_UNSUPPORTED;
    }
    qf_decide dec;
    if (decp) dec = *decp;
    const int N = ctx->N;
    solve_cfg c = pick_cfg(N, sizeof(typename rt<R>::C), fold_wanted(N, skewh));
    if (c.G * c.C > (c.L <= 17 ? 512 : 256)) {
        qf_set_error("qf_launch_solve: N=%d too large for the chunked solver", N);
        return QF_ERR_INVALID;
    }
    const int T = c.fold ? c.T : (skewh ? N : N + 1);
    unsigned blocks = (unsigned)((T + c.G - 1) / c.G);
    dim3 grid(blocks), block(c.threads);
    if (c.smem > 160 * 1024) {
        qf_set_error("qf_launch_solve: N=%d needs %zu bytes of LDS", N, c.smem);
// ... 9 lines not shown
#define QF_SOLVE(LL, SK) QF_SOLVE_F(LL, SK, 0)
    qf_plan_note(ctx, 0x4000000ull | (unsigned long long)(c.L << 16 | c.G << 8 | (F ? 8 : 0) | c.fold << 2 | (skewh ? 2 : 0) | (sizeof(R) == 4 ? 1 : 0)),
                 "{\"kernel\": \"k_solve%s<%s, L=%d, %s%s>\", \"chunk\": %d, \"chunks_per_walk\": %d, \"walks_per_workgroup\": %d, "
                 "\"workgroups\": %u, \"threads\": %d, \"lds_bytes\": %zu, \"step_end\": \"%s\"}",
                 F ? "_off" : "", sizeof(R) == 4 ? "float" : "double", c.L, skewh ? "skew-Hermitian" : "general", c.fold ? ", folded walk slots" : "", c.L, c.C,
                 c.G, blocks, c.threads, c.smem, dec.state_rw ? "takes the deferred decision of the previous iteration" : "none");
    if constexpr (sizeof(R) == sizeof(double)) {
        if (F) {
#define QF_SOLVE_OFF(LL, FO)                                                                        \
    {                                                                                               \
        static qf_smem_attr attr;                                                                   \
        QF_TRY(qf_smem_attr_set(attr, (const void *)k_solve_off<LL, FO>, ctx->device, c.smem));     \
        hipLaunchKernelGGL((k_solve_off<LL, FO>), grid, block, c.smem, ctx->stream, N, c.G, c.C, W, P, tab, F,  \
                           scale, guard, dec, (int)c.smem - 8 * (int)sizeof(typename rt<R>::C)); \
    }
            if (c.fold) {
                if (c.L == 9) QF_SOLVE_OFF(9, 1) else QF_SOLVE_OFF(17, 1)
            } else if (c.L == 4) QF_SOLVE_OFF(4, 0)
            else if (c.L == 8) QF_SOLVE_OFF(8, 0)
            else if (c.L == 16) QF_SOLVE_OFF(16, 0)
            else QF_SOLVE_OFF(32, 0)
#undef QF_SOLVE_OFF
            QF_HIP(hipGetLastError());
            return QF_OK;
        }
    }
    if (c.fold) {
        if (c.L == 9) QF_SOLVE_F(9, 1, 1) else QF_SOLVE_F(17, 1, 1)
    } else if (c.L == 4) {
        if (skewh) QF_SOLVE(4, 1) else QF_SOLVE(4, 0)
    } else if (c.L == 8) {
        if (skewh) QF_SOLVE(8, 1) else QF_SOLVE(8, 0)
    } else if (c.L == 16) {
        if (skewh) QF_SOLVE(16, 1) else QF_SOLVE(16, 0)
    } else {
        if (skewh) QF_SOLVE(32, 1) else QF_SOLVE(32, 0)
    }
#undef QF_SOLVE
#undef QF_SOLVE_F
    QF_HIP(hipGetLastError());
    return QF_OK;
}

}

int qf_launch_lap_table(qf_ctx *ctx, int bc, double *lap_dev)
{
    size_t NN = (size_t)ctx->N * ctx->N;
    int threads = 256;
    unsigned blocks = (unsigned)((NN + threads - 1) / threads);
    hipLaunchKernelGGL(k_lap_table<double>, dim3(blocks), dim3(threads), 0, ctx->stream, ctx->N, bc, lap_dev);
    QF_HIP(hipGetLastError());
    return QF_OK;
}

int qf_launch_build_factors(qf_ctx *ctx, const double *lap_dev, qf_factors f)
{
    int threads = 64;
    unsigned blocks = (unsigned)((ctx->N + 1 + threads - 1) / threads);
    hipLaunchKernelGGL((k_build_factors<double, double2>), dim3(blocks), dim3(threads), 0, ctx->stream, ctx->N, lap_dev, f.tab);
    QF_HIP(hipGetLastError());
    return QF_OK;
}

int qf_launch_solve(qf_ctx *ctx, const qf_factors &f, const cplx *W, cplx *P, double scale, int skewh,
                    qf_guard guard, const qf_decide *dec)
{
    return launch_solve<double>(ctx, f.tab, W, P, scale, skewh, guard, dec);
}

int qf_launch_hamiltonian(qf_ctx *ctx, const cplx *W, cplx *P, double scale, qf_guard guard, const qf_decide *dec)
{
    const qf_factors &f = ctx->ham_table ? ctx->ham : ctx->poisson;
    return launch_solve<double>(ctx, f.tab, W, P, scale, 1, guard, dec, ctx->ham_offset_on ? ctx->ham_offset : nullptr);
}

int qf_launch_decide(qf_ctx *ctx, const qf_decide &dec)
{
    hipLaunchKernelGGL(k_decide, dim3(1), dim3(256), 0, ctx->stream, ctx->N, dec);
    QF_HIP(hipGetLastError());
    return QF_OK;
}

int qf_launch_laplace(qf_ctx *ctx, const cplx *P, cplx *W)
{
    const int N = ctx->N;
    dim3 block(256), grid((N + 255) / 256, N);
    hipLaunchKernelGGL((k_laplace<double, double2>), grid, block, 0, ctx->stream, N, P, W);
    QF_HIP(hipGetLastError());
    return QF_OK;
}

int qf_launch_laplace_scaled(qf_ctx *ctx, const cplx *P, cplx *W, double scale)
{
    const int N = ctx->N;
    dim3 block(256), grid((N + 255) / 256, N);
    hipLaunchKernelGGL(k_laplace_scaled, grid, block, 0, ctx->stream, N, P, W, scale);
    QF_HIP(hipGetLastError());
    return QF_OK;
}

int qf_launch_lap_table(qf_ctx *ctx, int bc, float *lap_dev)
{
    size_t NN = (size_t)ctx->N * ctx->N;
    int threads = 256;
    unsigned blocks = (unsigned)((NN + threads - 1) / threads);
    hipLaunchKernelGGL(k_lap_table<float>, dim3(blocks), dim3(threads), 0, ctx->stream, ctx->N, bc, lap_dev);
    QF_HIP(hipGetLastError());
    return QF_OK;
}

int qf_launch_build_factors(qf_ctx *ctx, const float *lap_dev, float2 *tab)
{
    int threads = 64;
    unsigned blocks = (unsigned)((ctx->N + 1 + threads - 1) / threads);
    hipLaunchKernelGGL((k_build_factors<float, float2>), dim3(blocks), dim3(threads), 0, ctx->stream, ctx->N, lap_dev, tab);
    QF_HIP(hipGetLastError());
    return QF_OK;
}

int qf_launch_solve(qf_ctx *ctx, const float2 *tab, const float2 *W, float2 *P, float scale, int skewh, qf_guard guard)
{
    return launch_solve<float>(ctx, tab, W, P, scale, skewh, guard, nullptr);
}

int qf_launch_laplace(qf_ctx *ctx, const float2 *P, float2 *W)
{
    const int N = ctx->N;
    dim3 block(256), grid((N + 255) / 256, N);
    hipLaunchKernelGGL((k_laplace<float, float2>), grid, block, 0, ctx->stream, N, P, W);
    QF_HIP(hipGetLastError());
    return QF_OK;
}
```

### quflow_amd/csrc/qf_internal.h

```cpp
#pragma once

#include <hip/hip_runtime.h>

#include <atomic>
#include <cstdarg>
#include <cstdio>
#include <map>
#include <mutex>
#include <string>
#include <vector>

#include "../../include/quflow_hip.h"

typedef double2 cplx;

hipError_t qf_guard_malloc(void **p, size_t bytes);
hipError_t qf_guard_free(void *p);
#define hipMalloc(p, n) qf_guard_malloc((void **)(p), (n))
#define hipFree(p) qf_guard_free((void *)(p))

void qf_set_error(const char *fmt, ...);
struct qf_ctx;
inline void qf_plan_note(qf_ctx *ctx, unsigned long long key, const char *fmt, ...) __attribute__((format(printf, 3, 4)));

#define QF_HIP(call)                                                                   \
    do {                                                                               \
        hipError_t _e = (call);                                                        \
        if (_e != hipSuccess) {                                                        \
            qf_set_error("%s failed: %s (%s:%d)", #call, hipGetErrorString(_e), __FILE__, __LINE__); \
            return QF_ERR_HIP;                                                         \
        }                                                                              \
    } while (0)

#define QF_TRY(call)              \
    do {                          \
        int _r = (call);          \
        if (_r != QF_OK) return _r; \
    } while (0)

struct qf_factors {
    double2 *tab = nullptr;
};

#define QF_FAULT_WAIT 1
#define QF_FAULT_NONFINITE 2
#define QF_STEP_ABORTED 0x40000000
#define QF_FINITE(x_) ((x_) <= 1.7976931348623157e308 && (x_) >= -1.7976931348623157e308)

struct qf_dev_state {
    double resnorm;
    double tol;
    long long total_iterations;
    long long number_of_maxit;
    int step_index;
    int iters_this_step;
    int step_done;
    int minit, maxit;
    int dw_parity;
    int fault;
    int w_parity;
    int wh_sel;
    int pending;
    int pending_iter;
};


struct qf_host_record {
    unsigned long long seq;
    long long total_iterations;
    long long number_of_maxit;
    double resnorm;
    int step_index;
    int last_step_iters;
    int incomplete;
    int nonfinite;
    unsigned long long progress;
    double tol;
    int w_parity, wh_sel, dw_parity;
    int fault;
};

struct qf_decide {
    const double *rowpart = nullptr;
    int slots = 0;
    qf_dev_state *state_rw = nullptr;
    qf_host_record *rec = nullptr;
    unsigned *ticket = nullptr;
};

struct qf_guard {
    const qf_dev_state *state = nullptr;
    int step = 0;
    int iter = 0;
    const void *alt = nullptr;
};

#ifdef __HIPCC__
__device__ __forceinline__ bool qf_guard_iter(const qf_guard &g)
{
    if (!g.state) return true;
    return g.state->step_index == g.step && g.state->step_done == 0 && g.state->iters_this_step == g.iter;
}
__device__ __forceinline__ bool qf_guard_step_end(const qf_guard &g)
{
    if (!g.state) return true;
    return g.state->step_index == g.step && (g.state->step_done != 0 || g.state->iters_this_step >= g.state->maxit);
}
template <int CTRL> __device__ __forceinline__ double qf_dpp_f64(double v)
{
    const int lo = __builtin_amdgcn_update_dpp(0, __double2loint(v), CTRL, 0xf, 0xf, true);
    const int hi = __builtin_amdgcn_update_dpp(0, __double2hiint(v), CTRL, 0xf, 0xf, true);
    return __hiloint2double(hi, lo);
}
__device__ __forceinline__ double qf_row16_sum(double v)
{
    v += qf_dpp_f64<0xB1>(v);
    v += qf_dpp_f64<0x4E>(v);
    v += qf_dpp_f64<0x141>(v);
    v += qf_dpp_f64<0x140>(v);
    return v;
}

__device__ __forceinline__ double qf_modulus(double er, double ei)
{
    const double x = er * er + ei * ei;
    const double y = __builtin_amdgcn_rsq(x);
    double g = x * y, h = 0.5 * y;
    const double r = __builtin_fma(-h, g, 0.5);
    g = __builtin_fma(g, r, g);
    h = __builtin_fma(h, r, h);
    double d = __builtin_fma(-g, g, x);
    g = __builtin_fma(d, h, g);
    d = __builtin_fma(-g, g, x);
    g = __builtin_fma(d, h, g);
    return (x > 0.0 && x < __builtin_inf()) ? g : x;
}

__device__ __forceinline__ double qf_lap_b(int N, int i, int j)
{
    long long k = i < j ? i : j;
    long long am = i < j ? j - i : i - j;
    long long NN = N;
    return -(double)((NN - 1) * (2 * k + 1 + am) - 2 * k * (k + am));
}
__device__ __forceinline__ double qf_lap_a(int N, int i, int j)
{
    long long k = i < j ? i : j;
    long long am = i < j ? j - i : i - j;
    long long NN = N;
    return sqrt((double)(((k + am) * (NN - k - am)) * (k * (NN - k))));
}
template <typename R, typename C2>
__device__ __forceinline__ C2 qf_laplace_entry(int N, const C2 *__restrict__ P, int i, int j)
{
#pragma clang fp contract(off)
    const size_t e = (size_t)i * N + j;
    R b = (R)qf_lap_b(N, i, j);
    C2 p = P[e];
    R wr = b * p.x, wi = b * p.y;
    if (i < N - 1 && j < N - 1) {
        R a = (R)qf_lap_a(N, i + 1, j + 1);
        C2 q = P[e + N + 1];
        wr += a * q.x;
        wi += a * q.y;
    }
    if (i > 0 && j > 0) {
        R a = (R)qf_lap_a(N, i, j);
        C2 q = P[e - N - 1];
        wr += a * q.x;
        wi += a * q.y;
    }
// ... 127 lines not shown
    cplx *W2 = nullptr;
    cplx *Whalf2 = nullptr;
    bool fused_allowed = true;
    cplx *Whalf = nullptr;
    cplx *Phalf = nullptr;
    cplx *PW = nullptr;
    cplx *kahan_c = nullptr;
    cplx *stage = nullptr;
    signed char *oz_planes[4] = {nullptr, nullptr, nullptr, nullptr};
    double *oz_scale[4] = {nullptr, nullptr, nullptr, nullptr};
    bool gemm_i8 = false;
    bool gemm_i8_allowed = false;
    bool gemm_i8_hybrid = false;
    bool gemm_i8_first = false;
    int gemm_i8_min_n = 768;
    int oz_digits = 5;
    int oz_digits2 = 0;
    cplx *oz_tbuf = nullptr;
    unsigned *oz_tflags = nullptr;
    unsigned oz_epoch = 0;
    double *oz_diag = nullptr;
    std::vector<cplx *> multi;
    double *multi_rowpart = nullptr;
    std::vector<cplx *> stack;
    int stack_k = 0;
    double *mhd_part = nullptr;
    cplx *hook_host[3] = {nullptr, nullptr, nullptr};
    size_t hook_host_bytes = 0;
    cplx *ns_inv = nullptr;
    cplx *ns_tmp = nullptr;

    double *lap = nullptr;
    qf_factors poisson;
    struct factor_entry {
        qf_factors f;
        unsigned long long fingerprint = 0;
        unsigned long long last_used = 0;
    };
    std::map<unsigned long long, factor_entry> user_factors;
    unsigned long long factor_clock = 0;
    size_t factor_budget_bytes = (size_t)512 << 20;
    double *lap_user = nullptr;
    qf_factors ham;
    unsigned long long ham_key = 0, ham_fp = 0;
    cplx *ham_offset = nullptr;
    unsigned long long ham_offset_key = 0, ham_offset_fp = 0;
    bool ham_table = false, ham_offset_on = false;
    cplx *forcing_f0 = nullptr;
    unsigned long long forcing_key = 0, forcing_fp = 0;
    bool forcing_on = false, forcing_f0_on = false;
    double forcing_aW = 0.0, forcing_aP = 0.0, forcing_alap = 0.0;
    qf_stoch stoch;

    double *basis = nullptr;
    cplx *sh_stage = nullptr;
    double *sh_omega = nullptr;
    long long sh_shr_count = 0;
    long long slab_budget = 0;
    double *slab = nullptr;
    size_t slab_cap = 0;
    qf_sht sht;
    qf_eigh_ws eigh;
    qf_geom_ws geom;

    double *rowpart = nullptr;
    int rowpart_tiles = 0;
    double *rowsum = nullptr;
    double *scalars = nullptr;
    double *host_scalars = nullptr;
    qf_dev_state *state = nullptr;
    qf_host_record *host_rec = nullptr;
    bool diag_at_exit = false, diag_valid = false;
    unsigned *ticket = nullptr;
    int pred_iters = 3;
    bool gemm_tri_allowed = true;
    bool gemm_tri = false;
    int gemm_tri_min_n = 960;
    bool gemm_tri32 = false;
    int tri32_split = 2, tri32_split_diag = 1;
    cplx *t32_partial = nullptr;
    unsigned *t32_arrive = nullptr;
    bool defer_allowed = true;
    bool defer = false;
    int num_cus = 0;
    cplx *sk_partial = nullptr;
    unsigned *sk_flags = nullptr;
    int sk_slots = 0;
    unsigned sk_epoch = 0;
    int sk_epi_units = 0;
    int sk_epi_units_fused = 2;
    int sk_min_units = 8;
    int debug_drop = 0;
    bool needs_reset = false;

    qf_c64 *c64 = nullptr;

    int profile_mask = 0;
    std::vector<qf_event_pair> events_busy;
    std::vector<qf_event_pair> events_free;
    int profile_stride = 1;
    struct plan_slot {
        unsigned long long key = 0;
        char text[384] = {0};
    } plan[QF_KERNEL_COUNT];
    int plan_role = -1;
    long long prof_seen[QF_KERNEL_COUNT] = {0};
    long long prof_launches[QF_KERNEL_COUNT] = {0};
    double prof_ms[QF_KERNEL_COUNT] = {0};
    hipEvent_t timer_start = nullptr, timer_stop = nullptr;
};

inline void qf_plan_note(qf_ctx *ctx, unsigned long long key, const char *fmt, ...)
{
    if (!ctx || ctx->plan_role < 0 || ctx->plan_role >= QF_KERNEL_COUNT) return;
    qf_ctx::plan_slot &s = ctx->plan[ctx->plan_role];
    if (key != 0 && s.key == key) return;
    va_list ap;
    va_start(ap, fmt);
    vsnprintf(s.text, sizeof(s.text), fmt, ap);
    va_end(ap);
    s.key = key;
}

inline int qf_refuse_forcing(const qf_ctx *ctx, const char *who)
{
    if (ctx && ctx->forcing_on) {
        qf_set_error("%s: a forcing is installed on this context (qf_set_forcing) and this entry point cannot apply it; "
                     "qf_isomp_forced, qf_isomp_hooked (k = 1) and qf_erk_hooked follow an installed forcing", who);
        return QF_ERR_UNSUPPORTED;
    }
    return QF_OK;
}

int qf_launch_forcing_affine(qf_ctx *ctx, const cplx *Ph, const cplx *X, cplx *out, double pscale, double s);

int qf_launch_stoch_pattern(qf_ctx *ctx, unsigned long long step, double dt);

int qf_launch_lap_table(qf_ctx *ctx, int bc, double *lap_dev);
int qf_launch_build_factors(qf_ctx *ctx, const double *lap_dev, qf_factors f);
int qf_launch_solve(qf_ctx *ctx, const qf_factors &f, const cplx *W, cplx *P, double scale, int skewh,
                    qf_guard guard = qf_guard(), const qf_decide *dec = nullptr);
int qf_launch_decide(qf_ctx *ctx, const qf_decide &dec);
int qf_launch_hamiltonian(qf_ctx *ctx, const cplx *W, cplx *P, double scale, qf_guard guard = qf_guard(),
                          const qf_decide *dec = nullptr);
int qf_launch_laplace(qf_ctx *ctx, const cplx *P, cplx *W);
int qf_launch_laplace_scaled(qf_ctx *ctx, const cplx *P, cplx *W, double scale);

int qf_launch_lap_table(qf_ctx *ctx, int bc, float *lap_dev);
int qf_launch_build_factors(qf_ctx *ctx, const float *lap_dev, float2 *tab);
int qf_launch_solve(qf_ctx *ctx, const float2 *tab, const float2 *W, float2 *P, float scale, int skewh,
                    qf_guard guard = qf_guard());
int qf_launch_laplace(qf_ctx *ctx, const float2 *P, float2 *W);

int qf_c64_alloc(qf_ctx *ctx);
void qf_c64_free(qf_c64 *f);
int qf_launch_cgemm(qf_ctx *ctx, const float2 *A, const float2 *B, float2 *C, const qf_epilogue_f *ep, qf_guard guard = qf_guard());
int qf_c64_tile(const qf_ctx *ctx);
int qf_c64_tile_first(const qf_ctx *ctx);
int qf_c64_tri_alloc(qf_ctx *ctx);
int qf_launch_cgemm_tri(qf_ctx *ctx, const float2 *A, const float2 *B, const qf_epilogue_f *ep, qf_guard guard = qf_guard());

struct qf_epilogue {
    const cplx *PW = nullptr;
    const cplx *W = nullptr;
    cplx *dW[2] = {nullptr, nullptr};
    cplx *Whalf = nullptr;
    double *rowpart = nullptr;
    int fused = 0;
    cplx *Wpair[2] = {nullptr, nullptr};
    cplx *Whalf_step = nullptr;
    unsigned *ticket = nullptr;
    int n_tiles = 0;
    qf_dev_state *state_rw = nullptr;
    qf_host_record *rec = nullptr;
    int debug_drop = 0;
};
struct qf_streamk {
    cplx *partial = nullptr;
    unsigned *flags = nullptr;
    unsigned epoch = 0;
    int *fault = nullptr;
    unsigned *ticket = nullptr;
    int n_tiles = 0;
    qf_dev_state *state_rw = nullptr;
    qf_host_record *rec = nullptr;
    unsigned spin_limit = 1u << 22;
    int debug_drop = 0;
    int slots = 0;
};
struct qf_tri32 {
    cplx *partial = nullptr;
    unsigned *arrive = nullptr;
    int split = 1;
    int split_diag = 1;
    unsigned *ticket = nullptr;
    int n_tiles = 0;
    qf_dev_state *state_rw = nullptr;
    qf_host_record *rec = nullptr;
    int debug_drop = 0;
    int deferred = 0;
};
int qf_gemm_tiles_n(int N);
int qf_launch_zgemm_tri32(qf_ctx *ctx, const cplx *A, const cplx *B, const qf_epilogue *ep, qf_guard guard = qf_guard());
int qf_launch_zgemm_tri(qf_ctx *ctx, const cplx *A, const cplx *B, const qf_epilogue *ep, qf_guard guard = qf_guard());
int qf_launch_zgemm(qf_ctx *ctx, const cplx *A, const cplx *B, cplx *C, const qf_epilogue *ep,
                    qf_guard guard = qf_guard());

int qf_launch_basis(qf_ctx *ctx, double *basis_dev);
__host__ __device__ inline long long qf_slab_prefix(int N, int Nmax, int m)
{
    const long long a = m, n = N, k = Nmax;
    return a * n * k - (n + k) * (a * (a - 1) / 2) + (a - 1) * a * (2 * a - 1) / 6;
}
int qf_slab_plan(int N, int Nmax, long long slab_bytes, std::vector<int> &first, long long *max_bytes);
int qf_launch_shr2mat(qf_ctx *ctx, int Nmax, const double *omega_dev, cplx *W_dev);
int qf_launch_band_basis(qf_ctx *ctx, int Nmax, double *band_dev);
int qf_launch_band_shr2mat(qf_ctx *ctx, int Nmax, const double *band_dev, const double *omega_dev, cplx *stage, cplx *W_dev);
int qf_launch_mat2shr(qf_ctx *ctx, int Nmax, const cplx *W_dev, double *omega_dev);
int qf_launch_shc2mat(qf_ctx *ctx, const double *omega_dev, cplx *W_dev);
int qf_launch_mat2shc(qf_ctx *ctx, const cplx *W_dev, double *omega_dev);

int qf_launch_sht_synth(qf_ctx *ctx, int L, int shr, int isreal, const double *omega_dev, long long n_valid);
void qf_sht_sizes(int L, int isreal, size_t bytes[6]);
int qf_launch_sht_analysis(qf_ctx *ctx, int L, int shr, int isreal, double *omega_dev);
int qf_launch_sht_qbuild(qf_ctx *ctx, int L);
void qf_sht_analysis_sizes(int L, int isreal, size_t bytes[8]);

int qf_launch_eigh_round(qf_ctx *ctx, cplx *G, int round, double tol, unsigned long long *word);
int qf_launch_eigh_normalise(qf_ctx *ctx, cplx *G, double *sig);
int qf_launch_eigh_rowdot(qf_ctx *ctx, const cplx *T, const cplx *U, cplx *out);
int qf_launch_eigh_conj_transpose(qf_ctx *ctx, const cplx *U, const int *perm, const cplx *scale, cplx *out);
int qf_launch_eigh_neg_i(qf_ctx *ctx, const cplx *X, cplx *out);

#define QF_SO3_STRIP 32
#define QF_SO3_MAX_DEGREE 16
int qf_so3_plan(int N, const double xi[3], int *squarings, int *degree, double *b_scaled);
int qf_launch_so3_taylor(qf_ctx *ctx, const double xi[3], int squarings, int degree, cplx *T);
int qf_launch_so3_grad(qf_ctx *ctx, const cplx *P, cplx *out);

struct qf_oz_job {
    const cplx *X = nullptr;
    const cplx *X_alt = nullptr;
    signed char *planes = nullptr;
    double *scale = nullptr;
};
struct qf_oz_mirror {
    cplx *tbuf = nullptr;
    unsigned *flags = nullptr;
    unsigned epoch = 0;
    int *fault = nullptr;
    const double *diag = nullptr;
    int debug_drop = 0;
};
struct qf_oz_jobs {
    qf_oz_job j[3];
    int n = 0;
    double *diag = nullptr;
};
size_t qf_oz_operand_bytes(int N, int digits);
size_t qf_oz_record_bytes(int N, int digits);
int qf_launch_oz_slice(qf_ctx *ctx, const qf_oz_jobs &jobs, qf_guard guard = qf_guard(), int digits = 0);
int qf_launch_oz_gemm(qf_ctx *ctx, const signed char *pa, const double *sa, const signed char *pm, const double *sm,
                      cplx *C, const qf_epilogue *ep = nullptr, qf_guard guard = qf_guard(), int digits = 0, int digits_m = 0,
                      const double *diag = nullptr);

template <class T> struct qf_same_type { typedef T type; };
template <class T> using qf_same = typename qf_same_type<T>::type;
template <class C>
int qf_launch_update(qf_ctx *ctx, const C *PW, C *W, const C *dW_a, const C *dW_b, C *Whalf, qf_same<C> *kahan_c,
                     int reinitialize, qf_guard guard = qf_guard());
int qf_launch_debug_modulus(qf_ctx *ctx, int n, const double *er, const double *ei, double *out_mod, double *out_sqrt);
int qf_launch_norm_from_rowpart(qf_ctx *ctx, const double *rowpart, int tiles, double *out_dev);
int qf_launch_fold_nonfinite(qf_ctx *ctx, const double *in_dev, double *acc_dev);
int qf_launch_norm_decide(qf_ctx *ctx, const double *rowpart, int tiles, qf_guard guard);
int qf_launch_state_init(qf_ctx *ctx, double tol, int minit, int maxit, const double *norm_dev = nullptr, double tol_factor = 0.0);
template <class C> int qf_launch_norm_inf(qf_ctx *ctx, const C *A, double *out_dev);
int qf_launch_call_begin(qf_ctx *ctx, double tol, int minit, int maxit, int auto_tol, double tol_factor);
template <class C> int qf_launch_inner2(qf_ctx *ctx, const C *A, const C *B, double *out_dev);
int qf_launch_inner(qf_ctx *ctx, const cplx *A, const cplx *B, double *out_dev);
int qf_launch_mhd_sums(qf_ctx *ctx, const cplx *W, const cplx *P, const cplx *Theta, double *part, double *out_dev);
int qf_launch_erk_stage(qf_ctx *ctx, const cplx *A, const cplx *B, double inv_hb, const cplx *W, cplx *acc,
                        double c_acc, cplx *Wp, double c_wp, cplx *Wout, double c_fin);
int qf_launch_magnetic_fix(qf_ctx *ctx, const cplx *BTP, const cplx *BT, cplx *dW, const cplx *dW_old, const cplx *W,
                           cplx *Whalf, double *rowpart);
int qf_launch_magnetic_update(qf_ctx *ctx, const cplx *BT, cplx *W, const cplx *dW, cplx *Whalf);
template <class C>
int qf_launch_lincomb(qf_ctx *ctx, double a, const C *X, double b, const qf_same<C> *Y, double c, C *out);
int qf_launch_neg_conj_transpose(qf_ctx *ctx, const cplx *X, cplx *out);
template <class C> int qf_launch_mirror_lower(qf_ctx *ctx, C *X);
// ... 3 lines not shown
```

### quflow_amd/csrc/zgemm.hip

```cpp
#include "qf_internal.h"
#include "qf_step_end.h"

#include <cstring>

typedef double v4d __attribute__((ext_vector_type(4)));

#ifdef QF_STAMP
__device__ unsigned long long *qf_stamp_buf = nullptr;
#define QF_STAMP_SLOTS 80
#ifdef QF_STAMP_LIGHT
#define QF_STAMP_AT(slot_)
#define QF_STAMP_PH(kt_, ph_)
__device__ unsigned long long *qf_phase_buf = nullptr;
#else
#define QF_STAMP_AT(slot_)                                                              \
    if (qf_stamp_buf && lane == 0 && (slot_) < QF_STAMP_SLOTS)                          \
        qf_stamp_buf[((size_t)blockIdx.x * (T / 64) + wave) * QF_STAMP_SLOTS + (slot_)] = __builtin_amdgcn_s_memtime();
__device__ unsigned long long *qf_phase_buf = nullptr;
#define QF_STAMP_PH(kt_, ph_)                                                           \
    if (qf_phase_buf && tid == 0 && (kt_) >= 20 && (kt_) < 28)                          \
        qf_phase_buf[((size_t)blockIdx.x * 8 + ((kt_) - 20)) * 5 + (ph_)] = __builtin_amdgcn_s_memtime();
#endif
__device__ unsigned long long *qf_tri_buf = nullptr;
#define QF_TRI_STAMP(seg_, k_)                                                          \
    if (qf_tri_buf && tid == 0 && (seg_) < 4)                                           \
        qf_tri_buf[((size_t)blockIdx.x * 4 + (seg_)) * 8 + (k_)] = __builtin_amdgcn_s_memtime();
#define QF_TRI_NOTE(seg_, k_, v_)                                                       \
    if (qf_tri_buf && tid == 0 && (seg_) < 4) qf_tri_buf[((size_t)blockIdx.x * 4 + (seg_)) * 8 + (k_)] = (unsigned long long)(v_);
#else
#define QF_STAMP_AT(slot_)
#define QF_STAMP_PH(kt_, ph_)
#define QF_TRI_STAMP(seg_, k_)
#define QF_TRI_NOTE(seg_, k_, v_)
#endif
#ifndef QF_ABL_NOSTORE
#define QF_ABL_NOSTORE 0
#endif
#ifndef QF_ABL_NOSUMS
#define QF_ABL_NOSUMS 0
#endif
#ifndef QF_ABL_NOADD
#define QF_ABL_NOADD 0
#endif
#define QF_SUM3M(c_) (QF_ABL_NOADD ? (c_).x : (c_).x + (c_).y)
#ifndef QF_ABL_NOGLOAD
#define QF_ABL_NOGLOAD 0
#endif
#ifndef QF_ABL_NOBARRIER
#define QF_ABL_NOBARRIER 0
#endif
#ifndef QF_SK_AUX_ST
#define QF_SK_AUX_ST 16
#endif
#ifndef QF_SK_AUX_LD
#define QF_SK_AUX_LD 16
#endif
#ifndef QF_XCD_BLOCK
#define QF_XCD_BLOCK 1
#endif
#ifndef QF_POLL_SLEEP
#define QF_POLL_SLEEP 8
#endif
#ifndef QF_TAIL_LITERAL
#define QF_TAIL_LITERAL 1
#endif
#ifndef QF_TAIL_LITERAL32
#define QF_TAIL_LITERAL32 1
#endif
#ifndef QF_STAGE_SPREAD
#define QF_STAGE_SPREAD 1
#endif

#ifndef QF_WT_PW
#define QF_WT_PW 1
#endif

namespace {

constexpr int BK = 16;

template <int BM, int BN, bool PAIR = false>
struct tile_smem {
    static constexpr int A_STRIDE = BM;
    static constexpr int B_STRIDE = BN;
    static constexpr int A_BUF_BYTES = BK * A_STRIDE * (int)sizeof(cplx);
    static constexpr int B_BUF_BYTES = BK * B_STRIDE * (int)sizeof(cplx);
    static constexpr int B_OFFSET = 2 * A_BUF_BYTES;
    static constexpr int A3_STRIDE = PAIR ? BM : BM + 2;
    static constexpr int B3_STRIDE = BN;
    static constexpr int A3_BUF_BYTES = BK * A3_STRIDE * (int)sizeof(double);
    static constexpr int B3_BUF_BYTES = BK * B3_STRIDE * (int)sizeof(double);
    static constexpr int A3_OFFSET = 2 * (A_BUF_BYTES + B_BUF_BYTES);
    static constexpr int B3_OFFSET = A3_OFFSET + 2 * A3_BUF_BYTES;
    static constexpr size_t main_bytes = (size_t)2 * (A_BUF_BYTES + B_BUF_BYTES) + (size_t)2 * (A3_BUF_BYTES + B3_BUF_BYTES);
    static constexpr size_t epi_bytes = (size_t)4 * BM * sizeof(double);
    static constexpr size_t bytes = main_bytes > epi_bytes ? main_bytes : epi_bytes;
};

__device__ __forceinline__ int xcd_remap(int bid, int nwg)
{
    const int q = nwg / 8, r = nwg % 8, xcd = bid % 8;
    return (xcd < r ? xcd * (q + 1) : r * (q + 1) + (xcd - r) * q) + bid / 8;
}

template <int BM, int BN, int WM, int WN, bool EPI, bool EXACT, bool FUSED = false>
__global__ __launch_bounds__(WM *WN * 64) void k_zgemm(int N, int tiles_m, int tiles_n,
                                                        const cplx *__restrict__ A,
                                                        const cplx *__restrict__ B, cplx *__restrict__ C,
                                                        qf_epilogue ep, qf_guard guard)
{
    constexpr int T = WM * WN * 64;
    constexpr bool FAST = EXACT && BM == 64 && BN == 64 && T == 256;
    using SM = tile_smem<BM, BN, FAST>;
    constexpr int WTM = BM / WM, WTN = BN / WN;
    constexpr int MT = WTM / 16, NT = WTN / 16;
    constexpr int A_STRIDE = SM::A_STRIDE, B_STRIDE = SM::B_STRIDE;
    constexpr int A_PER = (BM * BK) / T;
    constexpr int B_PER = (BN * BK) / T;
    constexpr int A_ROWS_PER = T / BK;
    constexpr int B_ROWS_PER = T / BN;
    static_assert((BM * BK) % T == 0 && (BN * BK) % T == 0 && T % BK == 0 && T % BN == 0, "tile/threads mismatch");
    constexpr int A3_STRIDE = SM::A3_STRIDE, B3_STRIDE = SM::B3_STRIDE;

    extern __shared__ __attribute__((aligned(16))) unsigned char smem_raw[];

    const int tid = (int)threadIdx.x;
    const int lane = tid & 63, wave = tid >> 6;
    const int wm = wave / WN, wn = wave % WN;
    const int r16 = lane & 15, q4 = lane >> 4;

    int tm, tn;
    if (QF_XCD_BLOCK && tiles_m % 4 == 0 && tiles_n % 2 == 0) {
        const int x = blockIdx.x & 7, l = blockIdx.x >> 3;
        const int R = tiles_m / 4, C = tiles_n / 2;
        int lr, lc;
        if (R % 4 == 0 && C % 8 == 0) {
            const int blk = l >> 5, in = l & 31;
            const int bpr = C / 8;
            lr = (blk / bpr) * 4 + (in >> 3);
            lc = (blk % bpr) * 8 + (in & 7);
        } else {
            lr = l / C;
            lc = l % C;
        }
        tm = (x >> 1) * R + lr;
        tn = (x & 1) * C + lc;
    } else {
        const int lid0 = xcd_remap(blockIdx.x, tiles_m * tiles_n);
        tm = lid0 / tiles_n;
        tn = lid0 % tiles_n;
    }
    const int lid = tm * tiles_n + tn;
    const int i0 = tm * BM, j0 = tn * BN;
    const cplx zero = make_double2(0.0, 0.0);
    const int parity = (EPI && guard.state) ? guard.state->dw_parity : 0;
    const cplx *__restrict__ ep_dW_old = ep.dW[parity];
    cplx *__restrict__ ep_dW_new = ep.dW[parity ^ 1];
    const int wpar = (FUSED && guard.state) ? guard.state->w_parity : 0;
    const cplx *__restrict__ ep_W = FUSED ? (wpar ? ep.Wpair[1] : ep.Wpair[0]) : ep.W;
    cplx *__restrict__ ep_Wnext = FUSED ? (wpar ? ep.Wpair[0] : ep.Wpair[1]) : nullptr;

    const unsigned char *lds_fa[2] = {
        smem_raw + (size_t)(q4 * A_STRIDE + wm * WTM + (r16 ^ q4)) * sizeof(cplx),
        smem_raw + (size_t)(q4 * A_STRIDE + wm * WTM + (r16 ^ q4 ^ 4)) * sizeof(cplx)};
    const unsigned char *lds_fb = smem_raw + SM::B_OFFSET + (size_t)(q4 * B_STRIDE + wn * WTN + r16) * sizeof(cplx);
    unsigned char *lds_sa = smem_raw + (size_t)((tid % BK) * A_STRIDE + ((tid / BK) ^ (tid % BK & 7))) * sizeof(cplx);
    unsigned char *lds_sb = smem_raw + SM::B_OFFSET + (size_t)tid * sizeof(cplx);
    const unsigned char *lds_fa3[2] = {
        smem_raw + SM::A3_OFFSET + (size_t)(q4 * A3_STRIDE + (FAST ? wm * WTM + 2 * (r16 ^ q4) : wm * WTM + r16)) * sizeof(double),
        smem_raw + SM::A3_OFFSET + (size_t)(q4 * A3_STRIDE + (FAST ? wm * WTM + 2 * (r16 ^ q4 ^ 4) : wm * WTM + r16)) * sizeof(double)};
    const unsigned char *lds_fb3 = smem_raw + SM::B3_OFFSET +
        (size_t)(q4 * B3_STRIDE + (FAST ? wn * WTN + 2 * r16 : wn * WTN + r16)) * sizeof(double);
    unsigned char *lds_sa3 = smem_raw + SM::A3_OFFSET +
        (size_t)((tid % BK) * A3_STRIDE + (FAST ? 2 * ((tid / BK) ^ (tid % BK & 7)) : tid / BK)) * sizeof(double);
    const int b_jA = ((tid % 32) / 16) * 32 + (tid % 16);
    unsigned char *lds_sb3 = smem_raw + SM::B3_OFFSET +
        (size_t)(FAST ? (tid / 32) * B3_STRIDE + 32 * ((tid % 32) / 16) + 2 * (tid % 16) : tid) * sizeof(double);
    if (FAST) lds_sb = smem_raw + SM::B_OFFSET + (size_t)((tid / 32) * B_STRIDE + b_jA) * sizeof(cplx);

    const unsigned a_voff = (unsigned)(((size_t)(tid / BK) * N + (tid % BK)) * sizeof(cplx));
    const unsigned b_voff = (unsigned)(((size_t)(tid / BN) * N + (tid % BN)) * sizeof(cplx));
    const int kt_off = 0;
    const unsigned char *a_row = reinterpret_cast<const unsigned char *>(A) + (size_t)i0 * N * sizeof(cplx);
    const size_t a_pass = (size_t)A_ROWS_PER * N * sizeof(cplx);
    const size_t b_pass = (size_t)B_ROWS_PER * N * sizeof(cplx);
    const size_t b_ktile = (size_t)BK * N * sizeof(cplx);
    const __amdgpu_buffer_rsrc_t rsrcA = __builtin_amdgcn_make_buffer_rsrc(
        const_cast<cplx *>(A), 0, FAST ? (int)((size_t)N * N * sizeof(cplx)) : 0, 0x00020000);
    const unsigned fa_voff = (unsigned)(((size_t)(tid / BK) * N + (tid % BK)) * sizeof(cplx));
    const unsigned fb_voff = (unsigned)(((size_t)(tid / 32) * N + b_jA) * sizeof(cplx));
    const unsigned fa_soff0 = (unsigned)((size_t)i0 * N * sizeof(cplx));
    const unsigned fb_soff0 = (unsigned)((size_t)j0 * sizeof(cplx));
// ... 352 lines not shown
#pragma unroll
        for (int mi = 0; mi < MT; ++mi)
#pragma unroll
            for (int ni = 0; ni < NT; ++ni)
#pragma unroll
                for (int reg = 0; reg < 4; ++reg) {
                    int gi = i0 + wm * WTM + mi * 16 + q4 + 4 * reg;
                    int gj = j0 + wn * WTN + ni * 16 + r16;
                    const double cre = accR[mi][ni][reg] - accI[mi][ni][reg];
                    const double cim = (accS[mi][ni][reg] - accR[mi][ni][reg]) - accI[mi][ni][reg];
                    if (EXACT || (gi < N && gj < N)) {
#if QF_WT_PW
                        const cplx v = make_double2(cre, cim);
                        __builtin_amdgcn_raw_buffer_store_b128(*reinterpret_cast<const v4u *>(&v), rsrcC,
                                                               (unsigned)(((size_t)gi * N + gj) * sizeof(cplx)), 0, 16);
#else
                        C[(size_t)gi * N + gj] = make_double2(cre, cim);
#endif
                    }
                }
    } else {
        double *rs = reinterpret_cast<double *>(smem_raw);
        __syncthreads();
#pragma unroll
        for (int mi = 0; mi < MT; ++mi) {
#pragma unroll
            for (int reg = 0; reg < 4; ++reg) {
                const int li = wm * WTM + mi * 16 + q4 + 4 * reg;
                const int gi = i0 + li;
                double rsum = 0.0;
#pragma unroll
                for (int ni = 0; ni < NT; ++ni) {
                    const int gj = j0 + wn * WTN + ni * 16 + r16;
                    if (EXACT || (gi < N && gj < N)) {
                        const size_t e = (size_t)gi * N + gj;
                        const double cr = e_c[mi][ni][reg].x;
                        const double ci = e_c[mi][ni][reg].y;
                        const double tre = accR[mi][ni][reg] - accI[mi][ni][reg];
                        const double tim = (accS[mi][ni][reg] - accR[mi][ni][reg]) - accI[mi][ni][reg];
                        const double dr = tre + cr;
                        const double di = tim + ci;
                        ep_dW_new[e] = make_double2(dr, di);
                        const cplx w = e_w[mi][ni][reg];
                        ep.Whalf[e] = make_double2(w.x + dr, w.y + di);
                        if (FUSED) {
                            const double wr = w.x + 2.0 * cr, wi = w.y + 2.0 * ci;
                            ep_Wnext[e] = make_double2(wr, wi);
                            ep.Whalf_step[e] = make_double2(wr + dr, wi + di);
                        }
                        const cplx o = e_old[mi][ni][reg];
                        const double er = o.x - dr, ei = o.y - di;
                        rsum += qf_modulus(er, ei);
                    }
                }
                rsum = qf_row16_sum(rsum);
                if (r16 == 0) rs[wn * BM + li] = rsum;
            }
        }
        __syncthreads();
        for (int li = tid; li < BM; li += T) {
            double s = 0.0;
#pragma unroll
            for (int c = 0; c < WN; ++c) s += rs[c * BM + li];
            if (EXACT || i0 + li < N) {
                if (FUSED) __hip_atomic_store(ep.rowpart + (size_t)tn * N + i0 + li, s, __ATOMIC_RELAXED, __HIP_MEMORY_SCOPE_AGENT);
                else ep.rowpart[(size_t)tn * N + i0 + li] = s;
            }
        }
        if (FUSED) {
            asm volatile("s_waitcnt vmcnt(0)" ::: "memory");
            __syncthreads();
            unsigned *last_flag = reinterpret_cast<unsigned *>(rs + WN * BM);
            if (tid == 0) {
                unsigned old = 0u;
                if (!((ep.debug_drop & 2) && lid == 0)) old = __hip_atomic_fetch_add(ep.ticket, 1u, __ATOMIC_RELAXED, __HIP_MEMORY_SCOPE_AGENT);
                *last_flag = (old == (unsigned)(ep.n_tiles - 1)) ? 1u : 0u;
            }
            __syncthreads();
            if (*last_flag != 0u)
                qf_fused_step_end(N, tiles_n, ep.rowpart, ep.ticket, ep.state_rw, ep.rec, guard.iter, tid, rs + WN * BM + 2);
        }
    }
    QF_STAMP_AT(KT + 2)
}

constexpr size_t TRI_SMEM_BYTES = 2 * 64 * 65 * sizeof(cplx) + 4 * 64 * sizeof(double) + 64;

__global__ __launch_bounds__(256) void k_zgemm_tri(int N, int nt, int U, int E, const cplx *__restrict__ A,
                                                    const cplx *__restrict__ B, qf_epilogue ep, qf_guard guard,
                                                    qf_streamk sk)
{
    constexpr int BM = 64, BN = 64, WM = 2, WN = 2;
    constexpr bool EPI = true, EXACT = true, FAST = true;
    using SM = tile_smem<BM, BN, true>;
    constexpr int T = WM * WN * 64;
    constexpr int WTM = BM / WM, WTN = BN / WN;
    constexpr int MT = WTM / 16, NT = WTN / 16;
    constexpr int A_STRIDE = SM::A_STRIDE, B_STRIDE = SM::B_STRIDE;
    constexpr int A_PER = (BM * BK) / T, B_PER = (BN * BK) / T;
    constexpr int A_ROWS_PER = T / BK, B_ROWS_PER = T / BN;
    constexpr int A3_STRIDE = SM::A3_STRIDE, B3_STRIDE = SM::B3_STRIDE;
    constexpr int TS = BN + 1;
    constexpr int TT_BYTES = BM * TS * (int)sizeof(cplx);
    static_assert((size_t)2 * TT_BYTES + (WN * BM + WM * BN) * sizeof(double) + 16 <= TRI_SMEM_BYTES, "epilogue scratch exceeds the LDS request");
    static_assert(TRI_SMEM_BYTES >= SM::main_bytes, "K-loop buffers exceed the LDS request");
    typedef unsigned v4u __attribute__((ext_vector_type(4)));
    constexpr int SG_MFMA = 0x008, SG_VMEM_RD = 0x020, SG_DS_WR = 0x200;

    extern __shared__ __attribute__((aligned(16))) unsigned char smem_raw[];

    const int tid = threadIdx.x;
    const int lane = tid & 63, wave = tid >> 6;
    const int wm = wave / WN, wn = wave % WN;
    const int r16_c = lane & 15, q4_c = lane >> 4;
    const int G = gridDim.x;
    const int c = xcd_remap(blockIdx.x, G);
    const int KTN = N / BK;
    const int S = KTN + E;
    int u = (int)((long long)c * U / G);
    const int u_end = (int)((long long)(c + 1) * U / G);
    const cplx zero = make_double2(0.0, 0.0);

    const unsigned char *lds_fa[2] = {
        smem_raw + (size_t)(q4_c * A_STRIDE + wm * WTM + (r16_c ^ q4_c)) * sizeof(cplx),
        smem_raw + (size_t)(q4_c * A_STRIDE + wm * WTM + (r16_c ^ q4_c ^ 4)) * sizeof(cplx)};
    const unsigned char *lds_fb = smem_raw + SM::B_OFFSET + (size_t)(q4_c * B_STRIDE + wn * WTN + r16_c) * sizeof(cplx);
    unsigned char *lds_sa = smem_raw + (size_t)((tid % BK) * A_STRIDE + ((tid / BK) ^ (tid % BK & 7))) * sizeof(cplx);
    const unsigned char *lds_fa3[2] = {
        smem_raw + SM::A3_OFFSET + (size_t)(q4_c * A3_STRIDE + wm * WTM + 2 * (r16_c ^ q4_c)) * sizeof(double),
        smem_raw + SM::A3_OFFSET + (size_t)(q4_c * A3_STRIDE + wm * WTM + 2 * (r16_c ^ q4_c ^ 4)) * sizeof(double)};
    const unsigned char *lds_fb3 = smem_raw + SM::B3_OFFSET + (size_t)(q4_c * B3_STRIDE + wn * WTN + 2 * r16_c) * sizeof(double);
    unsigned char *lds_sa3 = smem_raw + SM::A3_OFFSET + (size_t)((tid % BK) * A3_STRIDE + 2 * ((tid / BK) ^ (tid % BK & 7))) * sizeof(double);
    const int b_jA = ((tid % 32) / 16) * 32 + (tid % 16);
    unsigned char *lds_sb3 = smem_raw + SM::B3_OFFSET + (size_t)((tid / 32) * B3_STRIDE + 32 * ((tid % 32) / 16) + 2 * (tid % 16)) * sizeof(double);
    unsigned char *lds_sb = smem_raw + SM::B_OFFSET + (size_t)((tid / 32) * B_STRIDE + b_jA) * sizeof(cplx);
    const __amdgpu_buffer_rsrc_t rsrcA = __builtin_amdgcn_make_buffer_rsrc(const_cast<cplx *>(A), 0, (int)((size_t)N * N * sizeof(cplx)), 0x00020000);
    const __amdgpu_buffer_rsrc_t rsrcB = __builtin_amdgcn_make_buffer_rsrc(const_cast<cplx *>(B), 0, (int)((size_t)N * N * sizeof(cplx)), 0x00020000);
    const unsigned fa_voff = (unsigned)(((size_t)(tid / BK) * N + (tid % BK)) * sizeof(cplx));
    const unsigned fb_voff = (unsigned)(((size_t)(tid / 32) * N + b_jA) * sizeof(cplx));
    const unsigned f_rows16 = (unsigned)((size_t)16 * N * sizeof(cplx));
    const __amdgpu_buffer_rsrc_t rsrcP = __builtin_amdgcn_make_buffer_rsrc(sk.partial, 0, (int)((size_t)sk.slots * (BM * BN) * sizeof(cplx)), 0x00020000);
    const unsigned p_voff = (unsigned)(tid * sizeof(cplx));
    const unsigned char *a_row = nullptr, *b_col = nullptr;
    const size_t a_pass = 0, b_pass = 0, b_ktile = 0;
    const unsigned a_voff = 0, b_voff = 0;
    const int kt_off = 0;
    const int i0 = 0, j0 = 0;

    cplx e_c[MT][NT][4], e_t[MT][NT][4], e_w[MT][NT][4], e_old[MT][NT][4];
    v4d accR[MT][NT], accI[MT][NT], accS[MT][NT];
    cplx ra[2][A_PER], rb[2][B_PER];
    cplx fa[2][MT], fb[2][NT];
    double fas[2][MT], fbs[2][NT];
#pragma unroll
    for (int r = 0; r < A_PER; ++r) ra[1][r] = rb[1][r] = zero;

#define QF_TRI_KOF(p_) ((p_) <= 0 ? 0 : ((p_) <= E + 1 ? 1 : ((p_) - E > KTN ? KTN : (int)((p_) - E))))
#define QF_TRI_NEXT(u_, found_, t_, k0_, KT_, tm_, tn_)                                \
    {                                                                                  \
        found_ = false;                                                                \
        while (!(found_) && (u_) < u_end) {                                            \
            t_ = (int)((u_) / S);                                                      \
            const int pa_ = (u_) - (t_) * S;                                           \
            int pb_ = u_end - (t_) * S;                                                \
            if (pb_ > S) pb_ = S;                                                      \
            const int klo_ = QF_TRI_KOF(pa_), khi_ = QF_TRI_KOF(pb_);                  \
// ... 220 lines not shown
                for (int cc = 0; cc < WN; ++cc) s2 += rs[cc * BM + tid];
                __hip_atomic_store(ep.rowpart + (size_t)tn * N + i0 + tid, s2, __ATOMIC_RELAXED, __HIP_MEMORY_SCOPE_AGENT);
                if (open_if_large && s2 > tol_now) *open_flag = 1u;
            } else if (offdiag && tid < BM + BN) {
                const int lj = tid - BM;
                double s2 = 0.0;
#pragma unroll
                for (int cc = 0; cc < WM; ++cc) s2 += cs[cc * BN + lj];
                __hip_atomic_store(ep.rowpart + (size_t)tm * N + j0 + lj, s2, __ATOMIC_RELAXED, __HIP_MEMORY_SCOPE_AGENT);
                if (open_if_large && s2 > tol_now) *open_flag = 1u;
            }
            unsigned ticket_old = 0u;
            if (ep.fused) {
                asm volatile("s_waitcnt vmcnt(0) lgkmcnt(0)\n\ts_barrier" ::: "memory");
                if (tid == 0 && !((sk.debug_drop & 2) && t == 0))
                    ticket_old = __hip_atomic_fetch_add(sk.ticket, 1u, __ATOMIC_RELAXED, __HIP_MEMORY_SCOPE_AGENT);
            } else {
                asm volatile("s_waitcnt lgkmcnt(0)\n\ts_barrier" ::: "memory");
            }
            QF_TRI_STAMP(seg, 7)
            const bool speculate = ep.fused && !(open_for_sure || (open_if_large && *open_flag != 0u));

            if (speculate) {
#pragma unroll
                for (int mi = 0; mi < MT; ++mi)
#pragma unroll
                    for (int reg = 0; reg < 4; ++reg) {
                        const int li = wm * WTM + mi * 16 + q4 + 4 * reg;
#pragma unroll
                        for (int ni = 0; ni < NT; ++ni) {
                            const int lj = wn * WTN + ni * 16 + r16;
                            const size_t e = (size_t)(i0 + li) * N + (j0 + lj);
                            const cplx w = e_w[mi][ni][reg];
                            const cplx wc = make_double2(w.x + 2.0 * e_c[mi][ni][reg].x, w.y + 2.0 * e_c[mi][ni][reg].y);
                            const cplx whs = make_double2(wc.x + tre[mi][ni][reg], wc.y + tim[mi][ni][reg]);
                            ep_Wnext[e] = wc;
                            ep.Whalf_step[e] = whs;
                            Ts[li * TS + lj] = whs;
                        }
                    }
            }
            asm volatile("s_waitcnt lgkmcnt(0)\n\ts_barrier" ::: "memory");
            if (offdiag) {
#pragma unroll
                for (int r = 0; r < 16; ++r) {
                    const int jl = wave * 16 + r;
                    const cplx wv = Th[lane_v * TS + jl];
                    const size_t e2 = (size_t)(j0 + jl) * N + (i0 + lane_v);
                    ep.Whalf[e2] = make_double2(-wv.x, wv.y);
                    if (speculate || !ep.fused) {
                        const cplx ws = Ts[lane_v * TS + jl];
                        if (ep.fused) ep.Whalf_step[e2] = make_double2(-ws.x, ws.y);
                        else ep_dW_new[e2] = make_double2(-ws.x, ws.y);
                    }
                }
            }
            if (have_next) QF_TRI_START_LOADS(n_k0, n_KT, n_tm, n_tn)
            if (ep.fused) {
                unsigned *last_flag = reinterpret_cast<unsigned *>(rs);
                if (tid == 0) *last_flag = (ticket_old == (unsigned)(sk.n_tiles - 1)) ? 1u : 0u;
                asm volatile("s_waitcnt lgkmcnt(0)\n\ts_barrier" ::: "memory");
                if (*last_flag != 0u) run_finale = true;
            }
        }
        QF_TRI_STAMP(seg, 3)
        ++seg;
        have = have_next;
        t = n_t;
        k0 = n_k0;
        KT = n_KT;
        tm = n_tm;
        tn = n_tn;
        asm volatile("s_waitcnt lgkmcnt(0)\n\ts_barrier" ::: "memory");
    }
    if (run_finale)
        qf_fused_step_end(N, nt, ep.rowpart, sk.ticket, sk.state_rw, sk.rec, guard.iter, tid, reinterpret_cast<double *>(smem_raw));
#undef QF_TRI_NEXT
#undef QF_TRI_KOF
#undef QF_TRI_HAS_PIECE
#undef QF_TRI_START_LOADS
}

template <bool EXACT>
__global__ __launch_bounds__(256) void k_zgemm_tri32(int N, int nt, const cplx *__restrict__ A, const cplx *__restrict__ B,
                                                      qf_epilogue ep, qf_guard guard, qf_tri32 sx)
{
    if (!qf_guard_iter(guard)) return;
    constexpr int BM = 32, BN = 32, WM = 2, WN = 2;
    constexpr bool EPI = true, FAST = false;
    using SM = tile_smem<BM, BN, false>;
    constexpr int T = WM * WN * 64;
    constexpr int WTM = BM / WM, WTN = BN / WN;
    constexpr int MT = WTM / 16, NT = WTN / 16;
    static_assert(MT == 1 && NT == 1, "one MFMA tile per wave");
    constexpr int A_STRIDE = SM::A_STRIDE, B_STRIDE = SM::B_STRIDE;
    constexpr int A_PER = (BM * BK) / T, B_PER = (BN * BK) / T;
    constexpr int A_ROWS_PER = T / BK, B_ROWS_PER = T / BN;
    constexpr int A3_STRIDE = SM::A3_STRIDE, B3_STRIDE = SM::B3_STRIDE;
    constexpr int TS = BN + 1;
    constexpr int TT_BYTES = BM * TS * (int)sizeof(cplx);
    static_assert((size_t)2 * TT_BYTES + (WN * BM + WM * BN) * sizeof(double) + 16 <= SM::bytes, "epilogue scratch exceeds the K-loop buffers");
    typedef unsigned v4u __attribute__((ext_vector_type(4)));
    constexpr int SG_MFMA = 0x008, SG_VMEM_RD = 0x020, SG_DS_WR = 0x200;

    extern __shared__ __attribute__((aligned(16))) unsigned char smem_raw[];

    const int tid = threadIdx.x;
    const int lane = tid & 63, wave = tid >> 6;
    const int wm = wave / WN, wn = wave % WN;
    const int r16 = lane & 15, q4 = lane >> 4;

    const int n_diag_w = nt * sx.split_diag;
    const int n_off = nt * (nt - 1) / 2;
    int tm, tn, h, nh, t;
    if ((int)blockIdx.x < n_diag_w) {
        nh = sx.split_diag;
        tm = tn = (int)blockIdx.x % nt;
        h = (int)blockIdx.x / nt;
        t = tm;
    } else {
        const int nw = (int)gridDim.x - n_diag_w;
        const int w = (n_diag_w % 8 == 0) ? xcd_remap((int)blockIdx.x - n_diag_w, nw) : (int)blockIdx.x - n_diag_w;
        nh = sx.split;
        const int o = w % n_off;
        h = w / n_off;
        tm = 0;
        int rem = o;
        while (rem >= nt - 1 - tm) {
            rem -= nt - 1 - tm;
            ++tm;
        }
        tn = tm + 1 + rem;
        t = nt + o;
    }
    const int i0 = tm * BM, j0 = tn * BN;
    const int KTN = (N + BK - 1) / BK;
    const int kt_begin = (int)((long long)h * KTN / nh);
    const int KT = (int)((long long)(h + 1) * KTN / nh) - kt_begin;

    const cplx zero = make_double2(0.0, 0.0);
    const int parity = guard.state ? guard.state->dw_parity : 0;
    const cplx *__restrict__ ep_dW_old = ep.dW[parity];
    cplx *__restrict__ ep_dW_new = ep.dW[parity ^ 1];
    const int wpar = (ep.fused && guard.state) ? guard.state->w_parity : 0;
    const cplx *__restrict__ ep_W = ep.fused ? ep.Wpair[wpar] : ep.W;
    cplx *__restrict__ ep_Wnext = ep.fused ? ep.Wpair[wpar ^ 1] : nullptr;
    const bool below_maxit = ep.fused && sx.state_rw && (guard.iter + 1 < sx.state_rw->maxit);
    const bool open_for_sure = below_maxit && (guard.iter + 1 < sx.state_rw->minit);
    const bool open_if_large = below_maxit && guard.iter == 0;
    const double tol_now = (ep.fused && sx.state_rw) ? sx.state_rw->tol : 0.0;

    const unsigned char *lds_fa[2] = {
        smem_raw + (size_t)(q4 * A_STRIDE + wm * WTM + (r16 ^ q4)) * sizeof(cplx),
        smem_raw + (size_t)(q4 * A_STRIDE + wm * WTM + (r16 ^ q4 ^ 4)) * sizeof(cplx)};
    const unsigned char *lds_fb = smem_raw + SM::B_OFFSET + (size_t)(q4 * B_STRIDE + wn * WTN + r16) * sizeof(cplx);
    unsigned char *lds_sa = smem_raw + (size_t)((tid % BK) * A_STRIDE + ((tid / BK) ^ (tid % BK & 7))) * sizeof(cplx);
    unsigned char *lds_sb = smem_raw + SM::B_OFFSET + (size_t)tid * sizeof(cplx);
    const unsigned char *lds_fa3[2] = {
        smem_raw + SM::A3_OFFSET + (size_t)(q4 * A3_STRIDE + wm * WTM + r16) * sizeof(double),
        smem_raw + SM::A3_OFFSET + (size_t)(q4 * A3_STRIDE + wm * WTM + r16) * sizeof(double)};
    const unsigned char *lds_fb3 = smem_raw + SM::B3_OFFSET + (size_t)(q4 * B3_STRIDE + wn * WTN + r16) * sizeof(double);
    unsigned char *lds_sa3 = smem_raw + SM::A3_OFFSET + (size_t)((tid % BK) * A3_STRIDE + tid / BK) * sizeof(double);
    unsigned char *lds_sb3 = smem_raw + SM::B3_OFFSET + (size_t)tid * sizeof(double);
    const unsigned a_voff = (unsigned)(((size_t)(tid / BK) * N + (tid % BK)) * sizeof(cplx));
    const unsigned b_voff = (unsigned)(((size_t)(tid / BN) * N + (tid % BN)) * sizeof(cplx));
    const int kt_off = kt_begin;
    const unsigned char *a_row = reinterpret_cast<const unsigned char *>(A) + ((size_t)i0 * N + (size_t)kt_begin * BK) * sizeof(cplx);
    const unsigned char *b_col = reinterpret_cast<const unsigned char *>(B) + ((size_t)kt_begin * BK * N + (size_t)j0) * sizeof(cplx);
// ... 122 lines not shown
    if (tid < BM) {
        double s2 = 0.0;
#pragma unroll
        for (int cc = 0; cc < WN; ++cc) s2 += rs[cc * BM + tid];
        if (EXACT || i0 + tid < N)
            __hip_atomic_store(ep.rowpart + (size_t)tn * N + i0 + tid, s2, __ATOMIC_RELAXED, __HIP_MEMORY_SCOPE_AGENT);
        if (open_if_large && s2 > tol_now) *open_flag = 1u;
    } else if (offdiag && tid >= 64 && tid < 64 + BN) {
        const int lj = tid - 64;
        double s2 = 0.0;
#pragma unroll
        for (int cc = 0; cc < WM; ++cc) s2 += cs[cc * BN + lj];
        if (EXACT || j0 + lj < N)
            __hip_atomic_store(ep.rowpart + (size_t)tm * N + j0 + lj, s2, __ATOMIC_RELAXED, __HIP_MEMORY_SCOPE_AGENT);
        if (open_if_large && s2 > tol_now) *open_flag = 1u;
    }
    unsigned ticket_old = 0u;
    if (ep.fused && sx.deferred) {
        if (tid == 0 && t == 0 && !(sx.debug_drop & 2)) {
            sx.state_rw->pending_iter = guard.iter;
            sx.state_rw->pending = 1;
        }
        asm volatile("s_waitcnt lgkmcnt(0)\n\ts_barrier" ::: "memory");
    } else if (ep.fused) {
        asm volatile("s_waitcnt vmcnt(0) lgkmcnt(0)\n\ts_barrier" ::: "memory");
        if (tid == 0 && !((sx.debug_drop & 2) && t == 0))
            ticket_old = __hip_atomic_fetch_add(sx.ticket, 1u, __ATOMIC_RELAXED, __HIP_MEMORY_SCOPE_AGENT);
    } else {
        asm volatile("s_waitcnt lgkmcnt(0)\n\ts_barrier" ::: "memory");
    }
    const bool speculate = ep.fused && !(open_for_sure || (open_if_large && *open_flag != 0u));
#pragma unroll
    for (int reg = 0; reg < 4; ++reg) {
        const int li = wm * WTM + q4 + 4 * reg;
        const int lj = wn * WTN + r16;
        const size_t e = (size_t)(i0 + li) * N + (j0 + lj);
        const cplx d = make_double2(tre[reg], tim[reg]);
        const cplx w = e_w[0][0][reg];
        const cplx wh = make_double2(w.x + d.x, w.y + d.y);
        const bool in = EXACT || (i0 + li < N && j0 + lj < N);
        if (in) {
            ep_dW_new[e] = d;
            ep.Whalf[e] = wh;
        }
        Th[li * TS + lj] = wh;
        if (speculate) {
            const cplx wc = make_double2(w.x + 2.0 * e_c[0][0][reg].x, w.y + 2.0 * e_c[0][0][reg].y);
            const cplx whs = make_double2(wc.x + d.x, wc.y + d.y);
            if (in) {
                ep_Wnext[e] = wc;
                ep.Whalf_step[e] = whs;
            }
            Ts[li * TS + lj] = whs;
        } else if (!ep.fused) {
            Ts[li * TS + lj] = d;
        }
    }
    asm volatile("s_waitcnt lgkmcnt(0)\n\ts_barrier" ::: "memory");
    if (offdiag) {
        const int il = lane & 31;
#pragma unroll
        for (int r = 0; r < 4; ++r) {
            const int jl = wave * 8 + r * 2 + (lane >> 5);
            if (!EXACT && (j0 + jl >= N || i0 + il >= N)) continue;
            const cplx wv = Th[il * TS + jl];
            const size_t e2 = (size_t)(j0 + jl) * N + (i0 + il);
            ep.Whalf[e2] = make_double2(-wv.x, wv.y);
            if (speculate || !ep.fused) {
                const cplx ws = Ts[il * TS + jl];
                if (ep.fused) ep.Whalf_step[e2] = make_double2(-ws.x, ws.y);
                else ep_dW_new[e2] = make_double2(-ws.x, ws.y);
            }
        }
    }
    if (ep.fused && !sx.deferred) {
        unsigned *last_flag = reinterpret_cast<unsigned *>(rs);
        if (tid == 0) *last_flag = (ticket_old == (unsigned)(sx.n_tiles - 1)) ? 1u : 0u;
        asm volatile("s_waitcnt lgkmcnt(0)\n\ts_barrier" ::: "memory");
        if (*last_flag != 0u)
            qf_fused_step_end(N, nt, ep.rowpart, sx.ticket, sx.state_rw, sx.rec, guard.iter, tid, reinterpret_cast<double *>(smem_raw));
    }
}

#undef QF_KTILE_STEADY
#undef QF_KTILE_TAIL
#undef QF_KTILE_LAST
#undef QF_KTILE
#undef QF_KTILE_SPREAD
#undef QF_KTILE_PHASE1
#undef QF_STORE_A
#undef QF_STORE_B
#undef QF_EPI_FETCH
#undef QF_EPI_COMM
#undef QF_LOAD_TILE
#undef QF_STORE_TILE
#undef QF_READ_FRAGS
#undef QF_MFMA

struct gemm_cfg {
    int BM, BN;
};

gemm_cfg pick_gemm(int N)
{
    gemm_cfg c;
    bool big;
    if (N % 32 != 0) {
        big = false;
    } else if (N % 64 != 0 || N < 896) {
        big = false;
    } else {
        const long long tiles = (long long)(N / 64) * (N / 64), rounds = (tiles + 255) / 256;
        big = tiles * 100 >= rounds * 256 * 85;
    }
    if (big) { c.BM = 64; c.BN = 64; }
    else { c.BM = 32; c.BN = 32; }
    return c;
}

template <int BM, int BN, int WM, int WN, bool EPI, bool EXACT, bool FUSED>
int launch4(qf_ctx *ctx, const cplx *A, const cplx *B, cplx *C, qf_epilogue ep, const qf_guard &guard)
{
    const int N = ctx->N;
    const int tiles_m = (N + BM - 1) / BM, tiles_n = (N + BN - 1) / BN;
    const size_t smem = tile_smem<BM, BN, EXACT && BM == 64 && BN == 64 && WM * WN == 4>::bytes;
    static qf_smem_attr attr;
    QF_TRY(qf_smem_attr_set(attr, (const void *)k_zgemm<BM, BN, WM, WN, EPI, EXACT, FUSED>, ctx->device, smem));
    if (FUSED) {
        ep.ticket = ctx->ticket + 400;
        ep.n_tiles = tiles_m * tiles_n;
        ep.state_rw = ctx->state;
        ep.rec = ctx->host_rec;
        if (ctx->debug_drop == 2) {
            ep.debug_drop = 2;
            ctx->debug_drop = 0;
        }
    }
    dim3 grid(tiles_m * tiles_n), block(WM * WN * 64);
    qf_plan_note(ctx, 0x1000000ull | (unsigned long long)(BM << 8 | EPI << 2 | EXACT << 1 | (FUSED ? 1 : 0)),
                 "{\"kernel\": \"k_zgemm<%d,%d%s>\", \"arithmetic\": \"fp64 3M, v_mfma_f64_16x16x4_f64\", \"tile\": [%d, %d], "
                 "\"tiles\": %d, \"tile_share\": 1.0, \"workgroups\": %d, \"threads\": %d, \"exact_tiling\": %s, \"step_end\": \"%s\"}",
                 BM, BN, EPI ? ",EPI" : "", BM, BN, tiles_m * tiles_n, tiles_m * tiles_n, WM * WN * 64, EXACT ? "true" : "false",
                 !EPI ? "none" : FUSED ? "fused (last tile decides)" : "two-kernel");
    hipLaunchKernelGGL((k_zgemm<BM, BN, WM, WN, EPI, EXACT, FUSED>), grid, block, smem, ctx->stream, N, tiles_m,
                       tiles_n, A, B, C, ep, guard);
    QF_HIP(hipGetLastError());
    return QF_OK;
}

template <int BM, int BN, int WM, int WN, bool EPI, bool EXACT>
int launch2(qf_ctx *ctx, const cplx *A, const cplx *B, cplx *C, const qf_epilogue &ep, const qf_guard &guard)
{
    if (EPI && ep.fused) return launch4<BM, BN, WM, WN, EPI, EXACT, EPI>(ctx, A, B, C, ep, guard);
    return launch4<BM, BN, WM, WN, EPI, EXACT, false>(ctx, A, B, C, ep, guard);
}

template <int BM, int BN, int WM, int WN>
int launch(qf_ctx *ctx, const cplx *A, const cplx *B, cplx *C, const qf_epilogue *ep, const qf_guard &guard)
{
    const int N = ctx->N;
    const bool exact = (N % BM == 0) && (N % BN == 0) && (N % BK == 0);
    qf_epilogue none;
    if (ep) {
        if (exact) return launch2<BM, BN, WM, WN, true, true>(ctx, A, B, C, *ep, guard);
        return launch2<BM, BN, WM, WN, true, false>(ctx, A, B, C, *ep, guard);
    }
    if (exact) return launch2<BM, BN, WM, WN, false, true>(ctx, A, B, C, none, guard);
    return launch2<BM, BN, WM, WN, false, false>(ctx, A, B, C, none, guard);
}

}

int qf_gemm_tiles_n(int N)
{
    gemm_cfg c = pick_gemm(N);
    return (N + c.BN - 1) / c.BN;
}

int qf_launch_zgemm_tri(qf_ctx *ctx, const cplx *A, const cplx *B, const qf_epilogue *ep, qf_guard guard)
{
    const int N = ctx->N;
    if (!ep || N % 64 != 0 || !ctx->sk_partial || ctx->num_cus < 1) {
        qf_set_error("qf_launch_zgemm_tri: not available for this context (N=%d)", N);
        return QF_ERR_STATE;
    }
    static qf_smem_attr attr;
    QF_TRY(qf_smem_attr_set(attr, (const void *)k_zgemm_tri, ctx->device, TRI_SMEM_BYTES));
    const int nt = N / 64;
    int E = ep->fused ? ctx->sk_epi_units_fused : ctx->sk_epi_units;
    if (E < -8) E = -8;
    const long long units = (long long)nt * (nt + 1) / 2 * (N / BK + E);
    if (units > 0x7fffffffLL) {
        qf_set_error("qf_launch_zgemm_tri: N=%d is too large for the stream-K partition", N);
        return QF_ERR_INVALID;
    }
    long long grid_ll = units / (ctx->sk_min_units > 0 ? ctx->sk_min_units : 1);
    if (grid_ll > ctx->num_cus) grid_ll = ctx->num_cus;
    if (grid_ll < 1) grid_ll = 1;
    const int grid = (int)grid_ll;
    qf_streamk sk;
    const int slots = ctx->sk_slots > 0 ? ctx->sk_slots : ctx->num_cus;
    sk.slots = slots;
    sk.partial = ctx->sk_partial;
    sk.flags = ctx->sk_flags;
    sk.epoch = ++ctx->sk_epoch;
    sk.fault = &ctx->host_rec->fault;
    sk.ticket = ctx->sk_flags + slots;
    sk.n_tiles = nt * (nt + 1) / 2;
    sk.state_rw = ctx->state;
    sk.rec = ctx->host_rec;
    if (ctx->debug_drop == 1 || (ctx->debug_drop == 2 && ep->fused)) {
        sk.debug_drop = ctx->debug_drop;
        sk.spin_limit = 1u << 14;
        ctx->debug_drop = 0;
    }
    qf_plan_note(ctx, 0x2000000ull | (unsigned long long)(grid << 8 | (E & 0x3f) << 1 | (ep->fused ? 1 : 0)),
                 "{\"kernel\": \"k_zgemm_tri\", \"arithmetic\": \"fp64 3M, v_mfma_f64_16x16x4_f64\", \"tile\": [64, 64], \"tiles\": %d, "
                 "\"tile_share\": %.6f, \"workgroups\": %d, \"threads\": 256, \"partition\": \"stream-K over (tile, K-tile) units, "
                 "contiguous ranges, epilogue weight E = %d K-tiles\", \"step_end\": \"%s\"}",
                 sk.n_tiles, (double)sk.n_tiles / ((double)nt * nt), grid, E, ep->fused ? "fused (last finisher decides)" : "two-kernel");
    hipLaunchKernelGGL(k_zgemm_tri, dim3(grid), dim3(256), TRI_SMEM_BYTES, ctx->stream, N, nt, (int)units, E, A, B, *ep, guard, sk);
    QF_HIP(hipGetLastError());
    return QF_OK;
}

int qf_launch_zgemm_tri32(qf_ctx *ctx, const cplx *A, const cplx *B, const qf_epilogue *ep, qf_guard guard)
{
    const int N = ctx->N;
    if (!ep || N < 64 || !ctx->t32_partial || !ctx->t32_arrive) {
        qf_set_error("qf_launch_zgemm_tri32: not available for this context (N=%d)", N);
        return QF_ERR_STATE;
    }
    const int nt = (N + 31) / 32;
    qf_tri32 sx;
    sx.partial = ctx->t32_partial;
    sx.arrive = ctx->t32_arrive;
    sx.split = (ctx->tri32_split == 2 || ctx->tri32_split == 4) ? ctx->tri32_split : 1;
    sx.split_diag = (ctx->tri32_split_diag == 2 || ctx->tri32_split_diag == 4) ? ctx->tri32_split_diag : 1;
    while (sx.split > 1 && (N + BK - 1) / BK / sx.split < 2) sx.split >>= 1;
    while (sx.split_diag > 1 && (N + BK - 1) / BK / sx.split_diag < 2) sx.split_diag >>= 1;
    sx.ticket = ctx->ticket + 401;
    sx.n_tiles = nt * (nt + 1) / 2;
    sx.state_rw = ctx->state;
    sx.rec = ctx->host_rec;
    if (ctx->debug_drop == 2 && ep->fused) {
        sx.debug_drop = 2;
        ctx->debug_drop = 0;
    }
    sx.deferred = (ep->fused && ctx->defer && guard.state) ? 1 : 0;
    const int grid = nt * sx.split_diag + nt * (nt - 1) / 2 * sx.split;
    const size_t smem = tile_smem<32, 32, false>::bytes;
    qf_plan_note(ctx, 0x3000000ull | (unsigned long long)(grid << 6 | sx.split << 3 | sx.split_diag << 1 | sx.deferred),
                 "{\"kernel\": \"k_zgemm_tri32<%s>\", \"arithmetic\": \"fp64 3M, v_mfma_f64_16x16x4_f64\", \"tile\": [32, 32], \"tiles\": %d, "
                 "\"tile_share\": %.6f, \"workgroups\": %d, \"threads\": 256, \"partition\": \"K range of an off-diagonal / diagonal tile in "
                 "%d / %d pieces, one workgroup each\", \"step_end\": \"%s\"}",
                 N % 32 == 0 ? "exact" : "guarded edges", sx.n_tiles, (double)sx.n_tiles / ((double)nt * nt), grid, sx.split, sx.split_diag,
                 !ep->fused ? "two-kernel" : sx.deferred ? "deferred (the next solve's workgroups decide)" : "fused (last tile decides)");
    if (N % 32 == 0) hipLaunchKernelGGL(k_zgemm_tri32<true>, dim3(grid), dim3(256), smem, ctx->stream, N, nt, A, B, *ep, guard, sx);
    else hipLaunchKernelGGL(k_zgemm_tri32<false>, dim3(grid), dim3(256), smem, ctx->stream, N, nt, A, B, *ep, guard, sx);
    QF_HIP(hipGetLastError());
    return QF_OK;
}

int qf_launch_zgemm(qf_ctx *ctx, const cplx *A, const cplx *B, cplx *C, const qf_epilogue *ep, qf_guard guard)
{
    if (ep && ctx->gemm_tri) return qf_launch_zgemm_tri(ctx, A, B, ep, guard);
    if (ep && ctx->gemm_tri32) return qf_launch_zgemm_tri32(ctx, A, B, ep, guard);
    gemm_cfg c = pick_gemm(ctx->N);
    if (c.BM == 64) return launch<64, 64, 2, 2>(ctx, A, B, C, ep, guard);
    return launch<32, 32, 2, 2>(ctx, A, B, C, ep, guard);
}
```

### quflow_amd/integrators.py

```python
import contextlib
import ctypes
import operator

import numpy as np

from . import _lib
from . import laplacian as _laplacian
from .context import Context, default_device, get_context, get_stepper_context, ptr
from .geometry import hbar


_SKEW_HERM_ = True


def _device_matmul(A, B):
    from .geometry import _device_matmul as mm
    return mm(A, B)


def _device_commutator(W, P, skewherm):
    from . import _lib
    from .context import as_c128, get_context, ptr, result_array
    Wc = as_c128(W, "W")
    Pc = as_c128(P, "P")
# ... 1092 lines not shown
                int(self.magnetic), ctypes.byref(st))
        out = {}
        if diagnostics and self.magnetic:
            d = (ctypes.c_double * 5)()
            _lib.check(self._lib.qf_states_advance_diag(*args, d))
            out = _mhd_dict(d)
        else:
            _lib.check(self._lib.qf_states_advance(*args))
            if diagnostics:
                out = self.diagnostics()
        out.update({"iterations": st.total_iterations / max(steps, 1),
                    "number_of_maxit": st.number_of_maxit / max(steps, 1),
                    "total_iterations": st.total_iterations, "tol": st.tol_used,
                    "last_resnorm": st.last_resnorm})
        return out

    def diagnostics(self):
        if self.magnetic:
            d = (ctypes.c_double * 5)()
            _lib.check(self._lib.qf_mhd_diagnostics(self.ctx.handle, d))
            return _mhd_dict(d)
        _lib.check(self._lib.qf_states_select(self.ctx.handle, 0))
        e, s = self._member.diagnostics()
        m = (ctypes.c_double * (2 * self.k))()
        _lib.check(self._lib.qf_states_inner(self.ctx.handle, m))
        return {"energy": e, "enstrophy": s, "members": [(m[2 * j], m[2 * j + 1]) for j in range(self.k)]}

    def _select(self, j):
        _lib.check(self._lib.qf_states_select(self.ctx.handle, int(j)))
        return self._member

    def shr(self, j, n_omega=None):
        return self._select(j).shr(n_omega)

    def fun(self, j, n_omega=None, berezin=True):
        return self._select(j).fun(n_omega, berezin)

    def spectrum(self, j):
        return self._select(j).spectrum()

    def rotate(self, xi):
        for j in range(self.k):
            self._select(j).rotate(xi)
            _lib.check(self._lib.qf_states_store(self.ctx.handle, j))
        return self

    def download(self):
        states = np.zeros((self.k, self.N, self.N), dtype=np.complex128)
        _lib.check(self._lib.qf_states_download(self.ctx.handle, ptr(states), self.k))
        return states

    def upload(self, states):
        states = _check_stack(states, self.magnetic, self.N)
        if states.shape[0] != self.k:
            raise ValueError("state must be (%d, %d, %d), got %s" % (self.k, self.N, self.N, states.shape))
        _lib.check(self._lib.qf_states_upload(self.ctx.handle, ptr(states), self.k))

    def sync(self):
        _lib.check(self._lib.qf_sync(self.ctx.handle))


class DeviceMHDTrajectory(DeviceStackTrajectory):

    def __init__(self, state0, device=None):
        super().__init__(state0, magnetic=True, device=device)


class DeviceEnsemble:

    def __init__(self, W0s, device=None, hamiltonian=None):
        self.members = [DeviceTrajectory(W0, device=device, hamiltonian=hamiltonian) for W0 in W0s]
        if not self.members:
            raise ValueError("DeviceEnsemble needs at least one initial condition")
        if len({m.N for m in self.members}) != 1:
            raise ValueError("the members of a DeviceEnsemble share one matrix size")
        if len({m.c64 for m in self.members}) != 1:
            raise ValueError("the members of a DeviceEnsemble share one dtype (complex128 or complex64)")
        self.c64 = self.members[0].c64
        self._lib = self.members[0]._lib

    def __len__(self):
        return len(self.members)

    CONCURRENT = 4

    def advance(self, dt, steps, tol='auto', maxit=10, minit=1):
        assert minit >= 1, "minit must be at least 1."
        assert maxit >= minit, "maxit must be at minit."
        tol_c = -1.0 if isinstance(tol, str) else float(tol)
        for m in self.members:
            _refuse_stochastic(m.forcing, "DeviceEnsemble.advance")
        fn = self._lib.qf_c64_isomp_multi if self.c64 else self._lib.qf_isomp_multi
        out = []
        failed = []
        for g0 in range(0, len(self.members), self.CONCURRENT):
            group = self.members[g0:g0 + self.CONCURRENT]
            k = len(group)
            handles = (ctypes.c_void_p * k)(*[m.ctx.handle for m in group])
            st = (_lib.IsompStats * k)()
            rc = fn(handles, k, float(dt), int(steps), tol_c, int(minit), int(maxit), st)
            if rc != _lib.QF_ERR_NONFINITE:
                _lib.check(rc)
            for r, s in enumerate(st):
                if rc == _lib.QF_ERR_NONFINITE and s.total_iterations < 0:
                    failed.append(g0 + r)
                    out.append({"failed": True, "tol": s.tol_used})
                    continue
                out.append({"iterations": s.total_iterations / max(steps, 1), "number_of_maxit": s.number_of_maxit / max(steps, 1),
                            "total_iterations": s.total_iterations, "tol": s.tol_used, "last_resnorm": s.last_resnorm})
        if failed:
            err = ValueError("array must not contain infs or NaNs (DeviceEnsemble members %s)" % ", ".join(map(str, failed)))
            err.failed = failed
            err.stats = out
            raise err
        return out

    def diagnostics(self):
        return [m.diagnostics() for m in self.members]

    def download(self):
        return [m.download() for m in self.members]

    def sync(self):
        for m in self.members:
            m.sync()

    def close(self):
        for m in self.members:
            m.ctx.close()
```

Measured before the change: 2680.

## Batch ensemble members' isomp iterations into shared multi-member kernel launches

Groups same-sized ensemble members (N up to 768, tri32 path) so that each iteration's solve, first product and triangular second product is launched once for the whole group on a lead stream, using 2D grids indexed by member. Host scheduling moves into a tag queue that is shared by batched and unbatched runs, with events ordering member streams around the group. The Python ensemble now asks the library for its concurrency and splits members into balanced groups. This is meant to cut per-member launch overhead and fill the GPU at small N, at the cost of coupling members' progress and adding more complex host orchestration.

Result: no change. 2669 (-0.4%).

```diff
diff --git a/include/quflow_hip.h b/include/quflow_hip.h
--- a/include/quflow_hip.h
+++ b/include/quflow_hip.h
@@ -74,6 +74,7 @@
 
 int qf_isomp_multi(qf_ctx **ctxs, int k, double dt, int steps, double tol, int minit, int maxit,
                    qf_isomp_stats *stats_out);
+int qf_ensemble_concurrent(const qf_ctx *ctx, int c64);
 int qf_c64_isomp_multi(qf_ctx **ctxs, int k, double dt, int steps, double tol, int minit, int maxit, qf_isomp_stats *stats_out);
 
 #define QF_ERK_EULER 0
diff --git a/quflow_amd/_lib.py b/quflow_amd/_lib.py
--- a/quflow_amd/_lib.py
+++ b/quflow_amd/_lib.py
@@ -104,6 +104,7 @@
                                       ctypes.c_int, ctypes.c_int, ctypes.POINTER(IsompStats)]),
     "qf_c64_isomp_multi": (ctypes.c_int, [ctypes.POINTER(_vp), ctypes.c_int, ctypes.c_double, ctypes.c_int, ctypes.c_double,
                                           ctypes.c_int, ctypes.c_int, ctypes.POINTER(IsompStats)]),
+    "qf_ensemble_concurrent": (ctypes.c_int, [_vp, ctypes.c_int]),
     "qf_erk": (ctypes.c_int, [_vp, ctypes.c_int, ctypes.c_double, ctypes.c_int, ctypes.c_int]),
     "qf_erk_states": (ctypes.c_int, [_vp, _vp, ctypes.c_int, ctypes.c_int, ctypes.c_double, ctypes.c_int, ctypes.c_int]),
     "qf_isomp_simple_hooked": (ctypes.c_int, [_vp, ctypes.c_double, ctypes.c_int, ctypes.POINTER(IsompHooks)]),
diff --git a/quflow_amd/csrc/api_context.hip b/quflow_amd/csrc/api_context.hip
--- a/quflow_amd/csrc/api_context.hip
+++ b/quflow_amd/csrc/api_context.hip
@@ -141,6 +141,8 @@
     if (const char *g = getenv("QUFLOW_HIP_DEFER")) ctx->defer_allowed = !(g[0] == '0');
     if (getenv("QUFLOW_HIP_DEBUG"))
         if (const char *g = getenv("QUFLOW_HIP_DEBUG_DROP_FLAG")) ctx->debug_drop = atoi(g);
+    if (const char *g = getenv("QUFLOW_HIP_BATCH")) ctx->batch_allowed = !(g[0] == '0');
+    if (ctx->debug_drop) ctx->batch_allowed = false;
     if (const char *g = getenv("QUFLOW_HIP_FACTOR_CACHE_MB")) ctx->factor_budget_bytes = (size_t)(atoi(g) > 0 ? atoi(g) : 1) << 20;
     const size_t NN = (size_t)N * N;
     const size_t mbytes = NN * sizeof(cplx);
@@ -258,6 +260,7 @@
     }
     if (ctx->timer_start) (void)hipEventDestroy(ctx->timer_start);
     if (ctx->timer_stop) (void)hipEventDestroy(ctx->timer_stop);
+    if (ctx->batch_event) (void)hipEventDestroy(ctx->batch_event);
     if (ctx->stream) (void)hipStreamDestroy(ctx->stream);
     delete ctx;
     return QF_OK;
diff --git a/quflow_amd/csrc/api_isomp.hip b/quflow_amd/csrc/api_isomp.hip
--- a/quflow_amd/csrc/api_isomp.hip
+++ b/quflow_amd/csrc/api_isomp.hip
@@ -9,12 +9,11 @@
 #include <utility>
 
 #include "qf_api.h"
+#include "qf_tag_queue.h"
 
 namespace {
 
-#ifndef QF_RUN_AHEAD
-#define QF_RUN_AHEAD 3
-#endif
+static_assert(QF_TAG_STEP_ABORTED == QF_STEP_ABORTED, "qf_tag_queue.h and qf_internal.h disagree about the aborted step counter");
 
 template <class S> constexpr bool is_c64 = std::is_same<S, qf_c64>::value;
 
@@ -187,7 +186,7 @@
     return d;
 }
 
-template <class S> int enqueue_iterations_fused(qf_ctx *ctx, int step, int first, int count, double vareps, bool last_step)
+template <class S> int enqueue_iterations_fused(qf_ctx *ctx, int step, int first, int count, double vareps)
 {
     S *w = ws<S>(ctx);
     const bool defer = !is_c64<S> && ctx->defer;
@@ -219,7 +218,6 @@
             }
         }
     }
-    if (defer && last_step && count > 0) QF_TRY(qf_launch_decide(ctx, dec));
     return QF_OK;
 }
 
@@ -308,102 +306,78 @@
 
 template <class S> struct fused_run {
     qf_ctx *ctx = nullptr;
-    int steps = 0, minit = 1, maxit = 1;
+    qf_tag_queue q;
     double vareps = 0.0;
-    int pred = 1, pred0 = 1;
-    std::vector<int> enq_iters;
-    int known = 0, enq = 0;
-    bool first_seen = false;
-    bool aborted = false;
+    bool batched = false;
+    hipStream_t stream = nullptr;
     unsigned long long idle_polls = 0;
 
-    int enqueue(int step, int first, int count)
-    {
-        if constexpr (!is_c64<S>)
-            if (ctx->gemm_i8) return enqueue_iterations_fused_i8(ctx, step, first, count, vareps);
-        return enqueue_iterations_fused<S>(ctx, step, first, count, vareps, step == steps - 1);
-    }
-    bool cold_start = true;
     void begin(qf_ctx *c, int steps_, int minit_, int maxit_, double vareps_)
     {
         ctx = c;
-        cold_start = ws<S>(c)->increment_is_zero;
-        steps = steps_;
-        minit = minit_;
-        maxit = maxit_;
         vareps = vareps_;
-        pred = ctx->pred_iters;
-        if (pred < minit) pred = minit;
-        if (pred > maxit) pred = maxit;
-        pred0 = ctx->pred_first_iters > 0 ? ctx->pred_first_iters : pred + 1;
-        if (pred0 < pred) pred0 = pred;
-        if (pred0 > maxit) pred0 = maxit;
-        enq_iters.assign((size_t)steps + 1, 0);
-        known = enq = 0;
-        first_seen = false;
-        aborted = false;
+        batched = false;
+        stream = c->stream;
         idle_polls = 0;
-    }
-    bool done() const { return known >= steps; }
+        q.begin(steps_, minit_, maxit_, c->pred_iters, c->pred_first_iters, ws<S>(c)->increment_is_zero, !is_c64<S> && c->defer && !c->gemm_i8);
+    }
+    bool done() const { return q.done(); }
+    int drain()
+    {
+        while (!q.pending.empty()) {
+            const qf_tag t = q.pending.front();
+            q.pending.pop_front();
+            if constexpr (!is_c64<S>) {
+                if (t.decide) {
+                    QF_TRY(qf_launch_decide(ctx, deferred_decision(ctx)));
+                    continue;
+                }
+                if (ctx->gemm_i8) {
+                    QF_TRY(enqueue_iterations_fused_i8(ctx, t.step, t.iter, 1, vareps));
+                    continue;
+                }
+            }
+            QF_TRY(enqueue_iterations_fused<S>(ctx, t.step, t.iter, 1, vareps));
+        }
+        return QF_OK;
+    }
+    int look()
+    {
+        if (done()) return QF_OK;
+        volatile qf_host_record *rec = ctx->host_rec;
+        unsigned long long p = __atomic_load_n(&rec->progress, __ATOMIC_ACQUIRE);
+        qf_tag_queue::result r = q.observe(p, rec->last_step_iters);
+        if (r == qf_tag_queue::IDLE) {
+            if (++idle_polls <= (1ull << 22)) return QF_OK;
+            if (batched && !q.pending.empty()) {
+                idle_polls = 0;
+                return QF_OK;
+            }
+            QF_HIP(hipStreamSynchronize(stream));
+            p = __atomic_load_n(&rec->progress, __ATOMIC_ACQUIRE);
+            r = q.observe(p, rec->last_step_iters);
+            if (r == qf_tag_queue::IDLE) {
+                qf_set_error("qf_isomp: device progress stuck at step %d iteration %d (waiting for step %d)", (int)(p >> 32),
+                             (int)(p & 0xffffffffull), q.known);
+                return QF_ERR_STATE;
+            }
+        }
+        idle_polls = 0;
+        if (r == qf_tag_queue::STUCK) {
+            qf_set_error("qf_isomp: step %d did not close after maxit=%d iterations (internal error)", q.known, q.maxit);
+            return QF_ERR_STATE;
+        }
+        if (q.learned_first > 0) ctx->pred_first_iters = q.learned_first;
+        if (r == qf_tag_queue::ADVANCED && done()) ctx->pred_iters = q.pred;
+        if (r == qf_tag_queue::REFILLED && !batched) QF_TRY(drain());
+        return QF_OK;
+    }
     int pump()
     {
         if (done()) return QF_OK;
-        while (enq < steps && enq - known < QF_RUN_AHEAD) {
-            const int n = (enq == 0 && cold_start) ? pred0 : pred;
-            QF_TRY(enqueue(enq, 0, n));
-            enq_iters[enq] = n;
-            ++enq;
-        }
-        volatile qf_host_record *rec = ctx->host_rec;
-        unsigned long long p = __atomic_load_n(&rec->progress, __ATOMIC_ACQUIRE);
-        int ps = (int)(p >> 32), pi = (int)(p & 0xffffffffull);
-        if (ps >= QF_STEP_ABORTED) {
-            aborted = true;
-            known = steps;
-            return QF_OK;
-        }
-        if (!(ps > known || (ps == known && pi >= enq_iters[known]))) {
-            if (++idle_polls > (1ull << 22)) {
-                QF_HIP(hipStreamSynchronize(ctx->stream));
-                p = __atomic_load_n(&rec->progress, __ATOMIC_ACQUIRE);
-                ps = (int)(p >> 32);
-                pi = (int)(p & 0xffffffffull);
-                if (ps >= QF_STEP_ABORTED) {
-                    aborted = true;
-                    known = steps;
-                    return QF_OK;
-                }
-                if (!(ps > known || (ps == known && pi >= enq_iters[known]))) {
-                    qf_set_error("qf_isomp: device progress stuck at step %d iteration %d (waiting for step %d)", ps, pi, known);
-                    return QF_ERR_STATE;
-                }
-            } else {
-                return QF_OK;
-            }
-        }
-        idle_polls = 0;
-        if (ps > known) {
-            const int it = rec->last_step_iters;
-            if (known == 0 && ps == 1 && !first_seen && cold_start) {
-                first_seen = true;
-                if (it >= minit && it <= maxit) ctx->pred_first_iters = it;
-            } else if (it >= minit && it <= maxit) {
-                pred = it;
-            }
-            known = ps < enq ? ps : enq;
-            if (done()) ctx->pred_iters = pred;
-            return QF_OK;
-        }
-        const int have = enq_iters[known];
-        if (have >= maxit) {
-            qf_set_error("qf_isomp: step %d did not close after maxit=%d iterations (internal error)", known, maxit);
-            return QF_ERR_STATE;
-        }
-        QF_TRY(enqueue(known, have, maxit - have));
-        enq_iters[known] = maxit;
-        enq = known + 1;
-        if (pred < maxit) pred += 1;
-        return QF_OK;
+        q.fill();
+        QF_TRY(drain());
+        return look();
     }
 };
 
@@ -435,7 +409,7 @@
         QF_TRY(run.pump());
         poll_relax();
     }
-    ctx->pred_iters = run.pred;
+    ctx->pred_iters = run.q.pred;
     return QF_OK;
 }
 
@@ -488,6 +462,68 @@
         QF_HIP(hipMemsetAsync(ctx->c64->tri_arrive, 0, ctx->c64->tri_arrive_count * sizeof(unsigned), ctx->stream));
     ctx->needs_reset = false;
     return QF_OK;
+}
+
+struct batch_group {
+    std::vector<fused_run<qf_ctx> *> runs;
+    hipStream_t stream = nullptr;
+    double vareps = 0.0;
+
+    int launch()
+    {
+        for (;;) {
+            bool hold = false;
+            for (fused_run<qf_ctx> *run : runs) hold = hold || run->q.expects_tags();
+            if (hold) return QF_OK;
+            qf_ctx *it_ctx[QF_BATCH_MAX], *de_ctx[QF_BATCH_MAX];
+            qf_guard guards[QF_BATCH_MAX];
+            qf_decide decs[QF_BATCH_MAX], lone[QF_BATCH_MAX];
+            qf_epilogue eps[QF_BATCH_MAX];
+            int nb = 0, nd = 0;
+            bool defer = false;
+            for (fused_run<qf_ctx> *run : runs) {
+                if (run->q.pending.empty()) continue;
+                const qf_tag t = run->q.pending.front();
+                run->q.pending.pop_front();
+                qf_ctx *ctx = run->ctx;
+                if (t.decide) {
+                    de_ctx[nd] = ctx;
+                    lone[nd++] = deferred_decision(ctx);
+                    continue;
+                }
+                it_ctx[nb] = ctx;
+                guards[nb].state = ctx->state;
+                guards[nb].step = t.step;
+                guards[nb].iter = t.iter;
+                guards[nb].alt = ctx->Whalf2;
+                defer = ctx->defer;
+                if (defer) decs[nb] = deferred_decision(ctx);
+                eps[nb] = epilogue_of(ctx, true);
+                ++nb;
+            }
+            if (!nb && !nd) return QF_OK;
+            auto role = [&](int id) {
+                for (int r = 0; r < nb; ++r) it_ctx[r]->plan_role = id;
+            };
+            if (nd) QF_TRY(qf_launch_decide_batch(de_ctx, nd, stream, lone));
+            if (!nb) continue;
+            role(QF_KERNEL_POISSON);
+            int rc = qf_launch_solve_batch(it_ctx, nb, stream, vareps, guards, defer ? decs : nullptr);
+            role(QF_KERNEL_GEMM1);
+            if (rc == QF_OK) rc = qf_launch_zgemm_batch(it_ctx, nb, stream, guards);
+            role(QF_KERNEL_GEMM2);
+            for (int r = 0; r < nb; ++r) guards[r].alt = nullptr;
+            if (rc == QF_OK) rc = qf_launch_zgemm_tri32_batch(it_ctx, nb, stream, eps, guards);
+            role(-1);
+            QF_TRY(rc);
+        }
+    }
+};
+
+bool batchable(const qf_ctx *ctx)
+{
+    return ctx->batch_allowed && ctx->fused_allowed && !ctx->gemm_i8 && !ctx->gemm_tri && ctx->gemm_tri32 && ctx->N % 32 == 0 &&
+           ctx->N >= 64 && ctx->N <= 768 && !ctx->ham_offset_on && ctx->profile_mask == 0 && ctx->debug_drop == 0;
 }
 
 template <class S> int fused_enter(qf_ctx *ctx, double dt, double tol, int minit, int maxit, bool carry)
@@ -796,6 +832,7 @@
         return first_rc;
     }
     auto abort_all = [&](int rc) {
+        for (int q = 0; q < k; ++q) (void)hipStreamSynchronize(ctxs[q]->stream);
         for (int q = 0; q < k; ++q) fused_abort(ctxs[q]);
         return rc;
     };
@@ -805,20 +842,92 @@
         if (rc != QF_OK) return abort_all(rc);
         runs[r].begin(ctxs[r], steps, minit, maxit, dt / (2 * qf_hbar(ctxs[r]->N)));
     }
+    std::vector<batch_group> groups;
+    if constexpr (!is_c64<S>) {
+        std::vector<char> taken((size_t)k, 0);
+        for (int r = 0; r < k && steps > 0; ++r) {
+            if (taken[r] || !batchable(ctxs[r])) continue;
+            std::vector<int> like;
+            for (int q = r; q < k; ++q)
+                if (!taken[q] && batchable(ctxs[q]) && ctxs[q]->N == ctxs[r]->N && ctxs[q]->defer == ctxs[r]->defer &&
+                    ctxs[q]->tri32_split == ctxs[r]->tri32_split && ctxs[q]->tri32_split_diag == ctxs[r]->tri32_split_diag) {
+                    like.push_back(q);
+                    taken[q] = 1;
+                }
+            const int n = (int)like.size();
+            if (n < 2) continue;
+            int ng = (n + QF_BATCH_MAX - 1) / QF_BATCH_MAX;
+            if (const char *e = getenv("QF_EXP_GROUPS")) ng = atoi(e) > ng ? (atoi(e) < n ? atoi(e) : n) : ng;
+            int at = 0;
+            for (int g = 0; g < ng; ++g) {
+                const int size = n / ng + (g < n % ng ? 1 : 0);
+                if (size < 2) {
+                    at += size;
+                    continue;
+                }
+                batch_group grp;
+                grp.stream = ctxs[like[at]]->stream;
+                grp.vareps = runs[like[at]].vareps;
+                for (int j = 0; j < size; ++j) {
+                    fused_run<S> &run = runs[like[at + j]];
+                    run.batched = true;
+                    run.stream = grp.stream;
+                    grp.runs.push_back(&run);
+                }
+                at += size;
+                groups.push_back(grp);
+            }
+        }
+    }
+    auto group_event = [&](qf_ctx *ctx) {
+        if (!ctx->batch_event) QF_HIP(hipEventCreateWithFlags(&ctx->batch_event, hipEventDisableTiming));
+        return QF_OK;
+    };
+    for (batch_group &grp : groups)
+        for (size_t j = 1; j < grp.runs.size(); ++j) {
+            qf_ctx *ctx = grp.runs[j]->ctx;
+            int rc = group_event(ctx);
+            if (rc == QF_OK && hipEventRecord(ctx->batch_event, ctx->stream) != hipSuccess) rc = QF_ERR_HIP;
+            if (rc == QF_OK && hipStreamWaitEvent(grp.stream, ctx->batch_event, 0) != hipSuccess) rc = QF_ERR_HIP;
+            if (rc != QF_OK) {
+                qf_set_error("%s: could not order a group's stream behind its members' entries", name);
+                return abort_all(rc);
+            }
+        }
     for (;;) {
         bool all = true;
+        for (batch_group &grp : groups) {
+            for (auto *run : grp.runs) run->q.fill();
+            int rc = grp.launch();
+            for (auto *run : grp.runs)
+                if (rc == QF_OK) rc = run->look();
+            if (rc != QF_OK) return abort_all(rc);
+        }
         for (int r = 0; r < k; ++r) {
             if (runs[r].done()) continue;
-            const int rc = runs[r].pump();
-            if (rc != QF_OK) return abort_all(rc);
+            if (!runs[r].batched) {
+                const int rc = runs[r].pump();
+                if (rc != QF_OK) return abort_all(rc);
+            }
             all = all && runs[r].done();
         }
         if (all) break;
         poll_relax();
     }
+    for (batch_group &grp : groups) {
+        qf_ctx *lead = grp.runs[0]->ctx;
+        int rc = group_event(lead);
+        if (rc == QF_OK && hipEventRecord(lead->batch_event, grp.stream) != hipSuccess) rc = QF_ERR_HIP;
+        for (size_t j = 1; j < grp.runs.size() && rc == QF_OK; ++j)
+            if (hipStreamWaitEvent(grp.runs[j]->ctx->stream, lead->batch_event, 0) != hipSuccess) rc = QF_ERR_HIP;
+        if (rc != QF_OK) {
+            qf_set_error("%s: could not order the members' streams behind their group's", name);
+            return abort_all(rc);
+        }
+    }
     int first_rc = QF_OK;
     for (int r = 0; r < k; ++r) {
-        ctxs[r]->pred_iters = runs[r].pred;
+        ctxs[r]->pred_iters = runs[r].q.pred;
         const int rc = fused_leave<S>(ctxs[r], steps, stats_out ? stats_out + r : nullptr);
         if (rc != QF_OK) {
             mark_failed(r);
@@ -873,6 +982,14 @@
     QF_TRY(qf_launch_inner2(ctx, ctx->W, ctx->stage, ctx->scalars + 2));
     QF_HIP(hipMemcpyAsync(ctx->host_scalars, ctx->scalars + 2, 2 * sizeof(double), hipMemcpyDeviceToHost, ctx->stream));
     return QF_OK;
+}
+
+int qf_ensemble_concurrent(const qf_ctx *ctx, int c64)
+{
+    if (!ctx) return 4;
+    const bool batch = !c64 && ctx->batch_allowed && ctx->fused_allowed && ctx->gemm_tri_allowed && !ctx->gemm_i8_allowed &&
+                       ctx->N % 32 == 0 && ctx->N >= 64 && ctx->N <= 768 && ctx->N < ctx->gemm_tri_min_n;
+    return batch ? QF_BATCH_MAX : 4;
 }
 
 int qf_isomp_multi(qf_ctx **ctxs, int k, double dt, int steps, double tol, int minit, int maxit, qf_isomp_stats *stats_out)
diff --git a/quflow_amd/csrc/poisson.hip b/quflow_amd/csrc/poisson.hip
--- a/quflow_amd/csrc/poisson.hip
+++ b/quflow_amd/csrc/poisson.hip
@@ -232,12 +232,53 @@
 #include "poisson_solve_body.h"
 #undef QF_SOLVE_OFFSET
 
-__global__ __launch_bounds__(256) void k_decide(int N, qf_decide dec)
+struct qf_solve_member {
+    const double2 *W = nullptr;
+    double2 *P = nullptr;
+    const double2 *tab = nullptr;
+    double scale = 0.0;
+    qf_guard guard;
+    qf_decide dec;
+};
+struct qf_solve_batch_args {
+    qf_solve_member m[QF_BATCH_MAX];
+};
+template <int L, int FOLD>
+__global__ __launch_bounds__(L <= 17 ? 512 : 256) void k_solve_batch(int N, int G, int C, int tail_off, qf_solve_batch_args args)
+{
+    typedef double R;
+    constexpr int SKEWH = 1;
+    const qf_solve_member &mb = args.m[blockIdx.y];
+    const double2 *__restrict__ W = mb.W;
+    double2 *__restrict__ P = mb.P;
+    const double2 *__restrict__ tab = mb.tab;
+    const double scale = mb.scale;
+    const qf_guard guard = mb.guard;
+    const qf_decide dec = mb.dec;
+#define QF_SOLVE_OFFSET 0
+#include "poisson_solve_body.h"
+#undef QF_SOLVE_OFFSET
+}
+
+__device__ __forceinline__ void decide_body(int N, const qf_decide &dec)
 {
     __shared__ double scratch[40];
     if (!dec.state_rw->pending) return;
     const qf_new_state ns = qf_decide_compute(N, dec.slots, dec.rowpart, dec.state_rw, scratch);
     if (threadIdx.x == 0) qf_decide_apply(dec.state_rw, dec.rec, dec.ticket, ns);
+}
+
+__global__ __launch_bounds__(256) void k_decide(int N, qf_decide dec)
+{
+    decide_body(N, dec);
+}
+
+struct qf_decide_batch_args {
+    qf_decide m[QF_BATCH_MAX];
+};
+__global__ __launch_bounds__(256) void k_decide_batch(int N, qf_decide_batch_args args)
+{
+    decide_body(N, args.m[blockIdx.y]);
 }
 
 struct solve_cfg {
@@ -413,6 +454,70 @@
     return QF_OK;
 }
 
+int qf_launch_solve_batch(qf_ctx *const *ctxs, int nb, hipStream_t stream, double scale, const qf_guard *guards, const qf_decide *decs)
+{
+    if (!ctxs || nb < 1 || nb > QF_BATCH_MAX || !guards) {
+        qf_set_error("qf_launch_solve_batch: bad arguments (nb=%d)", nb);
+        return QF_ERR_INVALID;
+    }
+    const int N = ctxs[0]->N;
+    solve_cfg c = pick_cfg(N, sizeof(cplx), fold_wanted(N, 1));
+    if (c.G * c.C > 512 || c.smem > 160 * 1024 || !(c.fold ? c.L == 9 : (c.L == 4 || c.L == 8 || c.L == 16))) {
+        qf_set_error("qf_launch_solve_batch: no batched solve for N=%d", N);
+        return QF_ERR_UNSUPPORTED;
+    }
+    const int T = c.fold ? c.T : N;
+    const unsigned blocks = (unsigned)((T + c.G - 1) / c.G);
+    qf_solve_batch_args args;
+    for (int r = 0; r < nb; ++r) {
+        qf_ctx *ctx = ctxs[r];
+        if (ctx->N != N || ctx->ham_offset_on) {
+            qf_set_error("qf_launch_solve_batch: member %d does not fit the batch", r);
+            return QF_ERR_INVALID;
+        }
+        qf_solve_member &m = args.m[r];
+        m.W = ctx->Whalf;
+        m.P = ctx->Phalf;
+        m.tab = (ctx->ham_table ? ctx->ham : ctx->poisson).tab;
+        m.scale = scale;
+        m.guard = guards[r];
+        if (decs) m.dec = decs[r];
+        qf_plan_note(ctx, 0x4000000ull | (unsigned long long)nb << 32 | (unsigned long long)(c.L << 16 | c.G << 8 | c.fold << 2 | 2),
+                     "{\"kernel\": \"k_solve_batch<L=%d, skew-Hermitian%s>\", \"batch\": %d, \"chunk\": %d, \"chunks_per_walk\": %d, "
+                     "\"walks_per_workgroup\": %d, \"workgroups\": %u, \"threads\": %d, \"lds_bytes\": %zu, \"step_end\": \"%s\"}",
+                     c.L, c.fold ? ", folded walk slots" : "", nb, c.L, c.C, c.G, blocks, c.threads, c.smem,
+                     m.dec.state_rw ? "takes the deferred decision of the previous iteration" : "none");
+    }
+    dim3 grid(blocks, (unsigned)nb), block(c.threads);
+    const int tail_off = (int)c.smem - 8 * (int)sizeof(cplx);
+#define QF_SOLVE_B(LL, FO)                                                                          \
+    {                                                                                               \
+        static qf_smem_attr attr;                                                                   \
+        QF_TRY(qf_smem_attr_set(attr, (const void *)k_solve_batch<LL, FO>, ctxs[0]->device, c.smem));  \
+        hipLaunchKernelGGL((k_solve_batch<LL, FO>), grid, block, c.smem, stream, N, c.G, c.C, tail_off, args);  \
+    }
+    if (c.fold) QF_SOLVE_B(9, 1)
+    else if (c.L == 4) QF_SOLVE_B(4, 0)
+    else if (c.L == 8) QF_SOLVE_B(8, 0)
+    else QF_SOLVE_B(16, 0)
+#undef QF_SOLVE_B
+    QF_HIP(hipGetLastError());
+    return QF_OK;
+}
+
+int qf_launch_decide_batch(qf_ctx *const *ctxs, int nb, hipStream_t stream, const qf_decide *decs)
+{
+    if (!ctxs || nb < 1 || nb > QF_BATCH_MAX || !decs) {
+        qf_set_error("qf_launch_decide_batch: bad arguments (nb=%d)", nb);
+        return QF_ERR_INVALID;
+    }
+    qf_decide_batch_args args;
+    for (int r = 0; r < nb; ++r) args.m[r] = decs[r];
+    hipLaunchKernelGGL(k_decide_batch, dim3(1, (unsigned)nb), dim3(256), 0, stream, ctxs[0]->N, args);
+    QF_HIP(hipGetLastError());
+    return QF_OK;
+}
+
 int qf_launch_laplace(qf_ctx *ctx, const cplx *P, cplx *W)
 {
     const int N = ctx->N;
diff --git a/quflow_amd/csrc/qf_internal.h b/quflow_amd/csrc/qf_internal.h
--- a/quflow_amd/csrc/qf_internal.h
+++ b/quflow_amd/csrc/qf_internal.h
@@ -87,6 +87,8 @@
     qf_host_record *rec = nullptr;
     unsigned *ticket = nullptr;
 };
+
+#define QF_BATCH_MAX 8
 
 struct qf_guard {
     const qf_dev_state *state = nullptr;
@@ -380,6 +382,8 @@
     unsigned *t32_arrive = nullptr;
     bool defer_allowed = true;
     bool defer = false;
+    bool batch_allowed = true;
+    hipEvent_t batch_event = nullptr;
     int num_cus = 0;
     cplx *sk_partial = nullptr;
     unsigned *sk_flags = nullptr;
@@ -503,6 +507,10 @@
 int qf_launch_zgemm_tri(qf_ctx *ctx, const cplx *A, const cplx *B, const qf_epilogue *ep, qf_guard guard = qf_guard());
 int qf_launch_zgemm(qf_ctx *ctx, const cplx *A, const cplx *B, cplx *C, const qf_epilogue *ep,
                     qf_guard guard = qf_guard());
+int qf_launch_solve_batch(qf_ctx *const *ctxs, int nb, hipStream_t stream, double scale, const qf_guard *guards, const qf_decide *decs);
+int qf_launch_zgemm_batch(qf_ctx *const *ctxs, int nb, hipStream_t stream, const qf_guard *guards);
+int qf_launch_zgemm_tri32_batch(qf_ctx *const *ctxs, int nb, hipStream_t stream, const qf_epilogue *eps, const qf_guard *guards);
+int qf_launch_decide_batch(qf_ctx *const *ctxs, int nb, hipStream_t stream, const qf_decide *decs);
 
 int qf_launch_basis(qf_ctx *ctx, double *basis_dev);
 __host__ __device__ inline long long qf_slab_prefix(int N, int Nmax, int m)
diff --git a/quflow_amd/csrc/qf_tag_queue.h b/quflow_amd/csrc/qf_tag_queue.h
--- /dev/null
+++ b/quflow_amd/csrc/qf_tag_queue.h
@@ -0,0 +1,109 @@
+#pragma once
+
+#include <deque>
+#include <vector>
+
+#ifndef QF_RUN_AHEAD
+#define QF_RUN_AHEAD 3
+#endif
+
+#define QF_TAG_STEP_ABORTED 0x40000000
+
+struct qf_tag {
+    int step = -1;
+    int iter = 0;
+    int decide = 0;
+};
+
+struct qf_tag_queue {
+    enum result { IDLE = 0, ADVANCED = 1, REFILLED = 2, ABORTED = 3, STUCK = -1 };
+
+    int steps = 0, minit = 1, maxit = 1;
+    int pred = 1, pred0 = 1;
+    bool cold_start = true, defer = false;
+    std::vector<int> enq_iters;
+    int known = 0, enq = 0;
+    bool first_seen = false, aborted = false;
+    int learned_first = 0;
+    std::deque<qf_tag> pending;
+
+    void begin(int steps_, int minit_, int maxit_, int pred_iters, int pred_first_iters, bool cold, bool defer_)
+    {
+        steps = steps_;
+        minit = minit_;
+        maxit = maxit_;
+        cold_start = cold;
+        defer = defer_;
+        pred = pred_iters;
+        if (pred < minit) pred = minit;
+        if (pred > maxit) pred = maxit;
+        pred0 = pred_first_iters > 0 ? pred_first_iters : pred + 1;
+        if (pred0 < pred) pred0 = pred;
+        if (pred0 > maxit) pred0 = maxit;
+        enq_iters.assign((size_t)steps + 1, 0);
+        known = enq = 0;
+        first_seen = false;
+        aborted = false;
+        learned_first = 0;
+        pending.clear();
+    }
+    bool done() const { return known >= steps; }
+    bool expects_tags() const { return !done() && pending.empty() && enq < steps; }
+
+    void push(int step, int first, int count)
+    {
+        for (int i = first; i < first + count; ++i) {
+            qf_tag t;
+            t.step = step;
+            t.iter = i;
+            pending.push_back(t);
+        }
+        if (defer && step == steps - 1 && count > 0) {
+            qf_tag t;
+            t.step = step;
+            t.decide = 1;
+            pending.push_back(t);
+        }
+    }
+    void fill()
+    {
+        if (done()) return;
+        while (enq < steps && enq - known < QF_RUN_AHEAD) {
+            const int n = (enq == 0 && cold_start) ? pred0 : pred;
+            push(enq, 0, n);
+            enq_iters[enq] = n;
+            ++enq;
+        }
+    }
+    result observe(unsigned long long p, int last_step_iters)
+    {
+        if (done()) return IDLE;
+        const int ps = (int)(p >> 32), pi = (int)(p & 0xffffffffull);
+        if (ps >= QF_TAG_STEP_ABORTED) {
+            aborted = true;
+            known = steps;
+            pending.clear();
+            return ABORTED;
+        }
+        if (!(ps > known || (ps == known && pi >= enq_iters[known]))) return IDLE;
+        if (ps > known) {
+            const int it = last_step_iters;
+            if (known == 0 && ps == 1 && !first_seen && cold_start) {
+                first_seen = true;
+                if (it >= minit && it <= maxit) learned_first = it;
+            } else if (it >= minit && it <= maxit) {
+                pred = it;
+            }
+            known = ps < enq ? ps : enq;
+            return ADVANCED;
+        }
+        const int have = enq_iters[known];
+        if (have >= maxit) return STUCK;
+        pending.clear();
+        push(known, have, maxit - have);
+        enq_iters[known] = maxit;
+        enq = known + 1;
+        if (pred < maxit) pred += 1;
+        return REFILLED;
+    }
+};
diff --git a/quflow_amd/csrc/zgemm.hip b/quflow_amd/csrc/zgemm.hip
--- a/quflow_amd/csrc/zgemm.hip
+++ b/quflow_amd/csrc/zgemm.hip
@@ -104,10 +104,10 @@
 }
 
 template <int BM, int BN, int WM, int WN, bool EPI, bool EXACT, bool FUSED = false>
-__global__ __launch_bounds__(WM *WN * 64) void k_zgemm(int N, int tiles_m, int tiles_n,
-                                                        const cplx *__restrict__ A,
-                                                        const cplx *__restrict__ B, cplx *__restrict__ C,
-                                                        qf_epilogue ep, qf_guard guard)
+__device__ __forceinline__ void zgemm_body(int N, int tiles_m, int tiles_n,
+                                           const cplx *__restrict__ A,
+                                           const cplx *__restrict__ B, cplx *__restrict__ C,
+                                           const qf_epilogue &ep, const qf_guard &guard)
 {
     constexpr int T = WM * WN * 64;
     constexpr bool FAST = EXACT && BM == 64 && BN == 64 && T == 256;
@@ -626,6 +626,32 @@
         }
     }
     QF_STAMP_AT(KT + 2)
+}
+
+template <int BM, int BN, int WM, int WN, bool EPI, bool EXACT, bool FUSED = false>
+__global__ __launch_bounds__(WM *WN * 64) void k_zgemm(int N, int tiles_m, int tiles_n,
+                                                        const cplx *__restrict__ A,
+                                                        const cplx *__restrict__ B, cplx *__restrict__ C,
+                                                        qf_epilogue ep, qf_guard guard)
+{
+    zgemm_body<BM, BN, WM, WN, EPI, EXACT, FUSED>(N, tiles_m, tiles_n, A, B, C, ep, guard);
+}
+
+struct qf_zgemm_member {
+    const cplx *A = nullptr;
+    const cplx *B = nullptr;
+    cplx *C = nullptr;
+    qf_guard guard;
+};
+struct qf_zgemm_batch_args {
+    qf_zgemm_member m[QF_BATCH_MAX];
+};
+template <int BM, int BN, int WM, int WN, bool EXACT>
+__global__ __launch_bounds__(WM *WN * 64) void k_zgemm_batch(int N, int tiles_m, int tiles_n, qf_zgemm_batch_args args)
+{
+    const qf_zgemm_member &m = args.m[blockIdx.y];
+    const qf_epilogue none;
+    zgemm_body<BM, BN, WM, WN, false, EXACT, false>(N, tiles_m, tiles_n, m.A, m.B, m.C, none, m.guard);
 }
 
 constexpr size_t TRI_SMEM_BYTES = 2 * 64 * 65 * sizeof(cplx) + 4 * 64 * sizeof(double) + 64;
@@ -1012,8 +1038,8 @@
 }
 
 template <bool EXACT>
-__global__ __launch_bounds__(256) void k_zgemm_tri32(int N, int nt, const cplx *__restrict__ A, const cplx *__restrict__ B,
-                                                      qf_epilogue ep, qf_guard guard, qf_tri32 sx)
+__device__ __forceinline__ void zgemm_tri32_body(int N, int nt, const cplx *__restrict__ A, const cplx *__restrict__ B,
+                                                 const qf_epilogue &ep, const qf_guard &guard, const qf_tri32 &sx)
 {
     if (!qf_guard_iter(guard)) return;
     constexpr int BM = 32, BN = 32, WM = 2, WN = 2;
@@ -1302,6 +1328,30 @@
     }
 }
 
+template <bool EXACT>
+__global__ __launch_bounds__(256) void k_zgemm_tri32(int N, int nt, const cplx *__restrict__ A, const cplx *__restrict__ B,
+                                                      qf_epilogue ep, qf_guard guard, qf_tri32 sx)
+{
+    zgemm_tri32_body<EXACT>(N, nt, A, B, ep, guard, sx);
+}
+
+struct qf_tri32_member {
+    const cplx *A = nullptr;
+    const cplx *B = nullptr;
+    qf_epilogue ep;
+    qf_guard guard;
+    qf_tri32 sx;
+};
+struct qf_tri32_batch_args {
+    qf_tri32_member m[QF_BATCH_MAX];
+};
+template <bool EXACT>
+__global__ __launch_bounds__(256) void k_zgemm_tri32_batch(int N, int nt, qf_tri32_batch_args args)
+{
+    const qf_tri32_member &m = args.m[blockIdx.y];
+    zgemm_tri32_body<EXACT>(N, nt, m.A, m.B, m.ep, m.guard, m.sx);
+}
+
 #undef QF_KTILE_STEADY
 #undef QF_KTILE_TAIL
 #undef QF_KTILE_LAST
@@ -1444,7 +1494,9 @@
     return QF_OK;
 }
 
-int qf_launch_zgemm_tri32(qf_ctx *ctx, const cplx *A, const cplx *B, const qf_epilogue *ep, qf_guard guard)
+namespace {
+
+int tri32_setup(qf_ctx *ctx, const qf_epilogue *ep, const qf_guard &guard, qf_tri32 &sx, int &grid)
 {
     const int N = ctx->N;
     if (!ep || N < 64 || !ctx->t32_partial || !ctx->t32_arrive) {
@@ -1452,7 +1504,6 @@
         return QF_ERR_STATE;
     }
     const int nt = (N + 31) / 32;
-    qf_tri32 sx;
     sx.partial = ctx->t32_partial;
     sx.arrive = ctx->t32_arrive;
     sx.split = (ctx->tri32_split == 2 || ctx->tri32_split == 4) ? ctx->tri32_split : 1;
@@ -1468,16 +1519,108 @@
         ctx->debug_drop = 0;
     }
     sx.deferred = (ep->fused && ctx->defer && guard.state) ? 1 : 0;
-    const int grid = nt * sx.split_diag + nt * (nt - 1) / 2 * sx.split;
+    grid = nt * sx.split_diag + nt * (nt - 1) / 2 * sx.split;
+    return QF_OK;
+}
+
+void tri32_note(qf_ctx *ctx, const qf_epilogue *ep, const qf_tri32 &sx, int grid, int batch)
+{
+    const int N = ctx->N, nt = (N + 31) / 32;
+    char tail[32] = "";
+    if (batch) snprintf(tail, sizeof(tail), ", \"batch\": %d", batch);
+    qf_plan_note(ctx, 0x3000000ull | (unsigned long long)batch << 32 | (unsigned long long)(grid << 6 | sx.split << 3 | sx.split_diag << 1 | sx.deferred),
+                 "{\"kernel\": \"k_zgemm_tri32%s<%s>\", \"arithmetic\": \"fp64 3M, v_mfma_f64_16x16x4_f64\", \"tile\": [32, 32], \"tiles\": %d, "
+                 "\"tile_share\": %.6f, \"workgroups\": %d, \"threads\": 256, \"partition\": \"K range of an off-diagonal / diagonal tile in "
+                 "%d / %d pieces, one workgroup each\", \"step_end\": \"%s\"%s}",
+                 batch ? "_batch" : "", N % 32 == 0 ? "exact" : "guarded edges", sx.n_tiles, (double)sx.n_tiles / ((double)nt * nt), grid, sx.split, sx.split_diag,
+                 !ep->fused ? "two-kernel" : sx.deferred ? "deferred (the next solve's workgroups decide)" : "fused (last tile decides)", tail);
+}
+
+}
+
+int qf_launch_zgemm_tri32(qf_ctx *ctx, const cplx *A, const cplx *B, const qf_epilogue *ep, qf_guard guard)
+{
+    const int N = ctx->N;
+    const int nt = (N + 31) / 32;
+    qf_tri32 sx;
+    int grid = 0;
+    QF_TRY(tri32_setup(ctx, ep, guard, sx, grid));
     const size_t smem = tile_smem<32, 32, false>::bytes;
-    qf_plan_note(ctx, 0x3000000ull | (unsigned long long)(grid << 6 | sx.split << 3 | sx.split_diag << 1 | sx.deferred),
-                 "{\"kernel\": \"k_zgemm_tri32<%s>\", \"arithmetic\": \"fp64 3M, v_mfma_f64_16x16x4_f64\", \"tile\": [32, 32], \"tiles\": %d, "
-                 "\"tile_share\": %.6f, \"workgroups\": %d, \"threads\": 256, \"partition\": \"K range of an off-diagonal / diagonal tile in "
-                 "%d / %d pieces, one workgroup each\", \"step_end\": \"%s\"}",
-                 N % 32 == 0 ? "exact" : "guarded edges", sx.n_tiles, (double)sx.n_tiles / ((double)nt * nt), grid, sx.split, sx.split_diag,
-                 !ep->fused ? "two-kernel" : sx.deferred ? "deferred (the next solve's workgroups decide)" : "fused (last tile decides)");
+    tri32_note(ctx, ep, sx, grid, 0);
     if (N % 32 == 0) hipLaunchKernelGGL(k_zgemm_tri32<true>, dim3(grid), dim3(256), smem, ctx->stream, N, nt, A, B, *ep, guard, sx);
     else hipLaunchKernelGGL(k_zgemm_tri32<false>, dim3(grid), dim3(256), smem, ctx->stream, N, nt, A, B, *ep, guard, sx);
+    QF_HIP(hipGetLastError());
+    return QF_OK;
+}
+
+int qf_launch_zgemm_batch(qf_ctx *const *ctxs, int nb, hipStream_t stream, const qf_guard *guards)
+{
+    if (!ctxs || nb < 1 || nb > QF_BATCH_MAX || !guards) {
+        qf_set_error("qf_launch_zgemm_batch: bad arguments (nb=%d)", nb);
+        return QF_ERR_INVALID;
+    }
+    const int N = ctxs[0]->N;
+    if (N % 32 != 0 || pick_gemm(N).BM != 32) {
+        qf_set_error("qf_launch_zgemm_batch: no batched first product for N=%d", N);
+        return QF_ERR_UNSUPPORTED;
+    }
+    const int tiles = N / 32;
+    const size_t smem = tile_smem<32, 32, false>::bytes;
+    static qf_smem_attr attr;
+    QF_TRY(qf_smem_attr_set(attr, (const void *)k_zgemm_batch<32, 32, 2, 2, true>, ctxs[0]->device, smem));
+    qf_zgemm_batch_args args;
+    for (int r = 0; r < nb; ++r) {
+        qf_ctx *ctx = ctxs[r];
+        if (ctx->N != N) {
+            qf_set_error("qf_launch_zgemm_batch: member %d does not fit the batch", r);
+            return QF_ERR_INVALID;
+        }
+        args.m[r].A = ctx->Phalf;
+        args.m[r].B = ctx->Whalf;
+        args.m[r].C = ctx->PW;
+        args.m[r].guard = guards[r];
+        qf_plan_note(ctx, 0x1000000ull | (unsigned long long)nb << 32 | (unsigned long long)(32 << 8 | 2),
+                     "{\"kernel\": \"k_zgemm_batch<32,32>\", \"arithmetic\": \"fp64 3M, v_mfma_f64_16x16x4_f64\", \"tile\": [32, 32], "
+                     "\"tiles\": %d, \"tile_share\": 1.0, \"workgroups\": %d, \"threads\": 256, \"exact_tiling\": true, \"step_end\": \"none\", "
+                     "\"batch\": %d}", tiles * tiles, tiles * tiles, nb);
+    }
+    hipLaunchKernelGGL((k_zgemm_batch<32, 32, 2, 2, true>), dim3(tiles * tiles, nb), dim3(256), smem, stream, N, tiles, tiles, args);
+    QF_HIP(hipGetLastError());
+    return QF_OK;
+}
+
+int qf_launch_zgemm_tri32_batch(qf_ctx *const *ctxs, int nb, hipStream_t stream, const qf_epilogue *eps, const qf_guard *guards)
+{
+    if (!ctxs || nb < 1 || nb > QF_BATCH_MAX || !eps || !guards) {
+        qf_set_error("qf_launch_zgemm_tri32_batch: bad arguments (nb=%d)", nb);
+        return QF_ERR_INVALID;
+    }
+    const int N = ctxs[0]->N;
+    if (N % 32 != 0) {
+        qf_set_error("qf_launch_zgemm_tri32_batch: no batched second product for N=%d", N);
+        return QF_ERR_UNSUPPORTED;
+    }
+    const int nt = N / 32;
+    const size_t smem = tile_smem<32, 32, false>::bytes;
+    qf_tri32_batch_args args;
+    int grid0 = 0;
+    for (int r = 0; r < nb; ++r) {
+        qf_ctx *ctx = ctxs[r];
+        qf_tri32_member &m = args.m[r];
+        int grid = 0;
+        QF_TRY(tri32_setup(ctx, eps + r, guards[r], m.sx, grid));
+        if (r == 0) grid0 = grid;
+        if (ctx->N != N || grid != grid0) {
+            qf_set_error("qf_launch_zgemm_tri32_batch: member %d does not fit the batch", r);
+            return QF_ERR_INVALID;
+        }
+        m.A = ctx->PW;
+        m.B = ctx->Phalf;
+        m.ep = eps[r];
+        m.guard = guards[r];
+        tri32_note(ctx, eps + r, m.sx, grid, nb);
+    }
+    hipLaunchKernelGGL(k_zgemm_tri32_batch<true>, dim3(grid0, nb), dim3(256), smem, stream, N, nt, args);
     QF_HIP(hipGetLastError());
     return QF_OK;
 }
diff --git a/quflow_amd/integrators.py b/quflow_amd/integrators.py
--- a/quflow_amd/integrators.py
+++ b/quflow_amd/integrators.py
@@ -1198,7 +1198,19 @@
     def __len__(self):
         return len(self.members)
 
-    CONCURRENT = 4
+    @property
+    def CONCURRENT(self):
+        return int(self._lib.qf_ensemble_concurrent(self.members[0].ctx.handle, 1 if self.c64 else 0))
+
+    def _groups(self):
+        k, c = len(self.members), max(1, self.CONCURRENT)
+        ng = (k + c - 1) // c
+        out, g0 = [], 0
+        for g in range(ng):
+            size = k // ng + (1 if g < k % ng else 0)
+            out.append((g0, self.members[g0:g0 + size]))
+            g0 += size
+        return out
 
     def advance(self, dt, steps, tol='auto', maxit=10, minit=1):
         assert minit >= 1, "minit must be at least 1."
@@ -1209,14 +1221,20 @@
         fn = self._lib.qf_c64_isomp_multi if self.c64 else self._lib.qf_isomp_multi
         out = []
         failed = []
-        for g0 in range(0, len(self.members), self.CONCURRENT):
-            group = self.members[g0:g0 + self.CONCURRENT]
+        other = None
+        for g0, group in self._groups():
             k = len(group)
             handles = (ctypes.c_void_p * k)(*[m.ctx.handle for m in group])
             st = (_lib.IsompStats * k)()
             rc = fn(handles, k, float(dt), int(steps), tol_c, int(minit), int(maxit), st)
-            if rc != _lib.QF_ERR_NONFINITE:
-                _lib.check(rc)
+            if rc not in (_lib.QF_OK, _lib.QF_ERR_NONFINITE):
+                try:
+                    _lib.check(rc)
+                except Exception as e:
+                    if other is None:
+                        other = e
+                out.extend([None] * k)
+                continue
             for r, s in enumerate(st):
                 if rc == _lib.QF_ERR_NONFINITE and s.total_iterations < 0:
                     failed.append(g0 + r)
@@ -1224,6 +1242,10 @@
                     continue
                 out.append({"iterations": s.total_iterations / max(steps, 1), "number_of_maxit": s.number_of_maxit / max(steps, 1),
                             "total_iterations": s.total_iterations, "tol": s.tol_used, "last_resnorm": s.last_resnorm})
+        if other is not None:
+            other.failed = failed
+            other.stats = out
+            raise other
         if failed:
             err = ValueError("array must not contain infs or NaNs (DeviceEnsemble members %s)" % ", ".join(map(str, failed)))
             err.failed = failed
```
